# leggedrobotics/traversability_estimation

Hardware: AMD Instinct MI355X
Metric: map cells/s through full filter chain (higher is better)
Workload: dtype f64 moments and eigen-solve, f32 acos and score tail (step filter and combine: f32 compare/add, exact); 1 GPU; 1 x 4096x4096 elevation map per GPU, res 0.05 m, radius 9 cells (normals/roughness/step), slope+roughness+step+normals+combine + traversability_footprint pass; maps_per_gpu=1, map_cells=16777216, footprint=True

## Files before the change

### include/travgpu.h

```cpp
#ifndef TRAVGPU_H
#define TRAVGPU_H

#include <stddef.h>
#include <stdint.h>

#ifdef __cplusplus
extern "C" {
#endif

#define TE_ABI_VERSION 1

typedef enum te_status {
  TE_OK = 0,
  TE_ERR_INVALID_ARG = -1,
  TE_ERR_BAD_PARAM = -2,
  TE_ERR_NOT_READY = -3,
  TE_ERR_HIP = -4,
  TE_ERR_NO_DEVICE = -5,
  TE_ERR_UNSUPPORTED = -6
} te_status;

typedef enum te_layer {
  TE_LAYER_ELEVATION = 0,
  TE_LAYER_SLOPE = 1,
  TE_LAYER_STEP = 2,
  TE_LAYER_ROUGHNESS = 3,
  TE_LAYER_TRAVERSABILITY = 4,
  TE_LAYER_FOOTPRINT = 5,
  TE_LAYER_NORMAL_X = 6,
  TE_LAYER_NORMAL_Y = 7,
  TE_LAYER_NORMAL_Z = 8,
  TE_LAYER_SLOPE_FOOTPRINT = 9,
  TE_LAYER_STEP_FOOTPRINT = 10,
  TE_LAYER_ROUGHNESS_FOOTPRINT = 11,
  TE_LAYER_TRAVERSABILITY_X = 12,
  TE_LAYER_TRAVERSABILITY_ROT = 13,
  TE_LAYER_ROBOT_SLOPE = 14,
  TE_LAYER_COUNT = 15
} te_layer;

#define TE_RUN_KEEP_NORMALS 0x1u
#define TE_RUN_FOOTPRINT    0x2u
#define TE_RUN_FOOTPRINT_MEMO 0x8u
#define TE_RUN_SEQUENTIAL 0x10u
#define TE_RUN_NORMALS_ONLY 0x20u
#define TE_RUN_GENERIC_KERNELS 0x4u

typedef enum te_filter {
  TE_FILTER_SLOPE = 1,
  TE_FILTER_STEP = 2,
  TE_FILTER_ROUGHNESS = 3,
  TE_FILTER_COMBINE = 4,
  TE_FILTER_NORMALS = 5
} te_filter;

typedef struct te_params {
  uint32_t size;
  uint32_t abi_version;
  double normals_radius;
  int32_t normals_axis;
  int32_t _pad0;
  double slope_critical;
  double step_critical;
  double step_radius1;
  double step_radius2;
  int32_t step_ncrit;
  int32_t _pad1;
  double rough_critical;
  double rough_radius;
  float w_scale, w_slope, w_step, w_rough;
  double fp_radius;
  double fp_offset;
  double fp_default;
  double fp_max_gap;
  double fp_critical_step;
  int32_t fp_check_roughness;
  int32_t _pad2;
} te_params;

typedef struct te_ctx te_ctx;

int te_params_default(te_params* p);
int te_params_validate(const te_params* p);

int te_device_count(int* count);
int te_create(int device, te_ctx** out);
int te_destroy(te_ctx* ctx);

int te_set_params(te_ctx* ctx, const te_params* p);
int te_get_params(te_ctx* ctx, te_params* p);
#define TE_OPT_FP_BLOCKED_WALK 1
#define TE_OPT_FP_BLOCKED_BLOCKS_PER_CU 2
#define TE_OPT_GRAPH_REPLAY 4
#define TE_OPT_POLYGON_PER_CELL 3
#define TE_OPT_BCAST_RCCL 5
#define TE_OPT_FP_ANY_REACH 7
#define TE_OPT_NORMALS_RANK_RULE 6
#define TE_OPT_FILTER_ANY_RADIUS 8
#define TE_OPT_FACE_FLAGS 9
int te_set_option(te_ctx* ctx, int option, int value);
int te_download_face_flags(te_ctx* ctx, unsigned char* out, size_t bytes);
int te_set_geometry(te_ctx* ctx, int rows, int cols, int batch, double resolution, double pos_x, double pos_y);

int te_upload_elevation(te_ctx* ctx, const float* host, int map0, int nmaps);
int te_upload_tile(te_ctx* ctx, const float* host_tile, int map, int row0, int col0, int h, int w);
int te_device_ptr(te_ctx* ctx, int layer, void** dptr, size_t* bytes);
int te_set_layer_present(te_ctx* ctx, int layer, int present);

int te_upload_layer(te_ctx* ctx, int layer, const float* host, int map0, int nmaps);
int te_upload_layer_circular(te_ctx* ctx, int layer, const float* host, int map, int start_row, int start_col);
int te_download_layer_circular(te_ctx* ctx, int layer, float* host, int map, int start_row, int start_col);
int te_prefetch_layers(te_ctx* ctx, int n, const int* layers, const float* const* hosts);
int te_wait_prefetch(te_ctx* ctx);
int te_run_filter(te_ctx* ctx, int filter, unsigned flags);
int te_run_chain(te_ctx* ctx, unsigned flags);
int te_run_chain_region(te_ctx* ctx, unsigned flags, int map, int row0, int col0, int h, int w);
int te_download_tile(te_ctx* ctx, int layer, int map, int row0, int col0, int h, int w, float* host_tile);
int te_upload_tile_async(te_ctx* ctx, const float* host_tile, int map, int row0, int col0, int h, int w);
int te_download_tile_async(te_ctx* ctx, int layer, int map, int row0, int col0, int h, int w, float* host_tile);
int te_run_footprint(te_ctx* ctx);
int te_check_footprint_paths(te_ctx* ctx, int map, int n_paths, const int* pose_offset, const double* pose_xy,
                             unsigned char* is_safe, double* traversability, int* status);
typedef struct te_path_check_stats {
  int n_visits, n_discs, n_radius_classes;
} te_path_check_stats;
int te_check_footprint_paths_radius(te_ctx* ctx, int map, int n_paths, const int* pose_offset, const double* pose_xy,
                                    const double* radius, double offset, unsigned char* is_safe, double* traversability,
                                    int* status, te_path_check_stats* stats);
int te_set_check_robot_inclination(te_ctx* ctx, int enabled);
int te_check_inclination(te_ctx* ctx, int map, int n_segments, const double* start_end_xy, unsigned char* ok, int* status);
#define TE_MAX_POLYGON_VERTICES 32
int te_run_polygon_footprint(te_ctx* ctx, int n_points, const double* points_xy, double yaw);
int te_polygons_traversable(te_ctx* ctx, int map, int n_polygons, const int* vertex_offset, const double* vertex_xy,
                            unsigned char* is_traversable, double* traversability);
int te_polygon_untraversable_hull(te_ctx* ctx, int map, int n_vertices, const double* vertex_xy, unsigned char* is_traversable,
                                  double* traversability, int cap_vertices, int* n_hull, double* hull_xy);
int te_check_polygon_footprint_paths(te_ctx* ctx, int map, int n_paths, const int* pose_offset, const double* poses, int n_points,
                                     const double* points_xyz, const unsigned char* conservative, unsigned char* is_safe,
                                     double* traversability, double* area, int* status);
int te_path_polygons(int n_paths, const int* pose_offset, const double* poses, int n_points, const double* points_xyz,
                     const unsigned char* conservative, int cap_polygons, int cap_vertices, int* n_polygons, int* n_vertices,
                     int* polygon_first, int* vertex_offset, double* vertex_xy, double* area);
int te_sync(te_ctx* ctx);

int te_download_layer(te_ctx* ctx, int layer, float* host, int map0, int nmaps);
int te_pin_host(void* host, size_t bytes);
int te_unpin_host(void* host);

int te_shard_range(int batch, int n_shards, int k, int* first, int* count);
int te_bcast_params(te_ctx** ctxs, int n, int root);
int te_run_chain_multi(te_ctx** ctxs, int n, unsigned flags);
int te_sync_multi(te_ctx** ctxs, int n);

int te_time_chain(te_ctx* ctx, unsigned flags, int warmup, int iters, float* ms_per_iter);
int te_time_chain_samples(te_ctx* ctx, unsigned flags, int warmup, int iters, float* ms);

#define TE_MSG_MAX_NAME 64
typedef struct te_msg_info {
  uint32_t seq, stamp_sec, stamp_nsec;
  char frame_id[TE_MSG_MAX_NAME];
  double resolution, length_x, length_y;
  double pose[7];
  int32_t rows, cols;
  int32_t start_row, start_col;
  int32_t n_layers, n_basic_layers;
} te_msg_info;

int te_msg_parse(const void* msg, size_t len, te_msg_info* info);
int te_msg_layer(const void* msg, size_t len, int k, char* name, size_t* data_offset);
int te_msg_write(const te_msg_info* info, int n_layers, const char* const* names, const float* const* layer_data, int n_basic,
                 const char* const* basic_names, void* out, size_t cap, size_t* written);
int te_upload_msg(te_ctx* ctx, const void* msg, size_t len, const char* layer_name, int layer, te_msg_info* info);
int te_download_msg(te_ctx* ctx, const te_msg_info* info, int n_layers, const int* layers, const char* const* names, int n_basic,
                    const char* const* basic_names, void* out, size_t cap, size_t* written);
int te_bag_find_message(const void* bag, size_t len, const char* topic, size_t* msg_offset, size_t* msg_len);
int te_bag_write(const void* msg, size_t msg_len, const char* topic, uint32_t stamp_sec, uint32_t stamp_nsec, void* out,
                 size_t cap, size_t* written);

typedef struct te_image_info {
  uint32_t seq, stamp_sec, stamp_nsec;
  char frame_id[TE_MSG_MAX_NAME];
  int32_t height, width, step;
  int32_t channels, bytes_per_channel;
// ... 64 lines not shown
```

### traversability_estimation_amd/capi.py

```python
import ctypes as C
import os
import struct
import sys

import numpy as np

_HERE = os.path.dirname(os.path.abspath(__file__))
LIB_PATH = os.environ.get("TRAVGPU_LIB") or os.path.join(_HERE, "libtravgpu.so")

TE_OK = 0
TE_ERR_INVALID_ARG, TE_ERR_BAD_PARAM, TE_ERR_NOT_READY, TE_ERR_HIP, TE_ERR_NO_DEVICE, TE_ERR_UNSUPPORTED = \
    -1, -2, -3, -4, -5, -6

LAYERS = dict(elevation=0, traversability_slope=1, traversability_step=2, traversability_roughness=3,
              traversability=4, traversability_footprint=5, surface_normal_x=6, surface_normal_y=7,
              surface_normal_z=8, slope_footprint=9, step_footprint=10, roughness_footprint=11,
              traversability_x=12, traversability_rot=13, robot_slope=14)
FILTERS = dict(slope=1, step=2, roughness=3, combine=4, normals=5)
RUN_KEEP_NORMALS = 0x1
RUN_FOOTPRINT = 0x2
RUN_GENERIC_KERNELS = 0x4
RUN_FOOTPRINT_MEMO = 0x8
RUN_SEQUENTIAL = 0x10
RUN_NORMALS_ONLY = 0x20
OPT_FP_BLOCKED_WALK, OPT_FP_BLOCKED_BLOCKS_PER_CU, OPT_POLYGON_PER_CELL, OPT_GRAPH_REPLAY, OPT_BCAST_RCCL, OPT_NORMALS_RANK_RULE = 1, 2, 3, 4, 5, 6
OPT_FP_ANY_REACH = 7
OPT_FACE_FLAGS = 9
OPT_FILTER_ANY_RADIUS = 8

SYMBOLS = ["te_params_default", "te_params_validate", "te_device_count", "te_create", "te_destroy",
           "te_set_params", "te_get_params", "te_set_option", "te_download_face_flags", "te_set_geometry", "te_upload_elevation", "te_upload_tile", "te_download_tile",
           "te_upload_tile_async", "te_download_tile_async",
           "te_device_ptr", "te_set_layer_present", "te_upload_layer", "te_prefetch_layers", "te_wait_prefetch", "te_upload_layer_circular", "te_download_layer_circular", "te_run_filter", "te_run_chain", "te_run_chain_region", "te_run_footprint", "te_check_footprint_paths", "te_check_footprint_paths_radius",
           "te_sync",
           "te_download_layer", "te_time_chain", "te_time_chain_samples", "te_last_error", "te_version",
           "te_msg_parse", "te_msg_layer", "te_msg_write", "te_upload_msg", "te_download_msg", "te_bag_find_message",
           "te_bag_write", "te_run_polygon_footprint", "te_polygons_traversable",
           "te_check_polygon_footprint_paths", "te_pin_host", "te_unpin_host", "te_path_polygons",
           "te_shard_range", "te_bcast_params", "te_run_chain_multi", "te_sync_multi",
           "te_set_check_robot_inclination", "te_check_inclination", "te_polygon_untraversable_hull",
           "te_image_parse", "te_upload_image", "te_upload_image_msg",
           "te_download_occupancy", "te_download_occupancy_msg", "te_occupancy_msg_write", "te_occupancy_parse",
           "te_download_cloud", "te_download_cloud_msg", "te_cloud_msg_write", "te_cloud_parse", "te_cloud_field", "te_cloud_spans",
           "te_expr_check", "te_run_expression", "te_time_expression_samples"]
MSG_MAX_NAME = 64
OCCUPANCY_MAX_LAYERS = CLOUD_MAX_LAYERS = 16
POINTFIELD_FLOAT32 = 7


def shard_range(batch, n_shards, k):
    first, count = C.c_int(), C.c_int()
    _check(load().te_shard_range(int(batch), int(n_shards), int(k), C.byref(first), C.byref(count)))
    return first.value, count.value


def _handles(ctxs):
    return (C.c_void_p * len(ctxs))(*[c._h for c in ctxs])


def bcast_params(ctxs, root=0):
    _check(load().te_bcast_params(_handles(ctxs), len(ctxs), int(root)))


def run_chain_multi(ctxs, flags=0):
    _check(load().te_run_chain_multi(_handles(ctxs), len(ctxs), int(flags)))


def sync_multi(ctxs):
    _check(load().te_sync_multi(_handles(ctxs), len(ctxs)))


def pack_paths(paths):
    paths = [np.asarray(p, dtype=np.float64).reshape(-1, 2) for p in paths]
    n = len(paths)
    off = np.zeros(n + 1, np.int32)
    if n:
        off[1:] = np.cumsum([len(p) for p in paths])
    xy = np.ascontiguousarray(np.concatenate(paths) if n and off[-1] else np.zeros((1, 2)), dtype=np.float64)
    return off, xy


class TeMsgInfo(C.Structure):
    _fields_ = [("seq", C.c_uint32), ("stamp_sec", C.c_uint32), ("stamp_nsec", C.c_uint32),
                ("frame_id", C.c_char * MSG_MAX_NAME),
                ("resolution", C.c_double), ("length_x", C.c_double), ("length_y", C.c_double),
                ("pose", C.c_double * 7),
                ("rows", C.c_int32), ("cols", C.c_int32), ("start_row", C.c_int32), ("start_col", C.c_int32),
                ("n_layers", C.c_int32), ("n_basic_layers", C.c_int32)]


class TeImageInfo(C.Structure):
    _fields_ = [("seq", C.c_uint32), ("stamp_sec", C.c_uint32), ("stamp_nsec", C.c_uint32),
                ("frame_id", C.c_char * MSG_MAX_NAME),
                ("height", C.c_int32), ("width", C.c_int32), ("step", C.c_int32),
                ("channels", C.c_int32), ("bytes_per_channel", C.c_int32), ("is_bigendian", C.c_int32),
                ("encoding", C.c_char * MSG_MAX_NAME)]


class TeOccupancyInfo(C.Structure):
    _fields_ = [("seq", C.c_uint32), ("stamp_sec", C.c_uint32), ("stamp_nsec", C.c_uint32),
                ("frame_id", C.c_char * MSG_MAX_NAME),
                ("map_load_sec", C.c_uint32), ("map_load_nsec", C.c_uint32),
                ("resolution", C.c_float), ("width", C.c_uint32), ("height", C.c_uint32),
                ("origin", C.c_double * 7)]


class TeCloudInfo(C.Structure):
    _fields_ = [("seq", C.c_uint32), ("stamp_sec", C.c_uint32), ("stamp_nsec", C.c_uint32),
                ("frame_id", C.c_char * MSG_MAX_NAME),
                ("height", C.c_uint32), ("width", C.c_uint32),
                ("n_fields", C.c_uint32), ("point_step", C.c_uint32), ("row_step", C.c_uint32),
                ("is_bigendian", C.c_int32), ("is_dense", C.c_int32)]


IMAGE_ENCODINGS = {"mono8": (1, 1), "8UC1": (1, 1), "mono16": (1, 2), "16UC1": (1, 2),
                   "rgb8": (3, 1), "bgr8": (3, 1), "8UC3": (3, 1), "rgba8": (4, 1), "bgra8": (4, 1), "8UC4": (4, 1),
                   "rgb16": (3, 2), "bgr16": (3, 2), "16UC3": (3, 2), "rgba16": (4, 2), "bgra16": (4, 2), "16UC4": (4, 2)}


class TeExprInfo(C.Structure):
    _fields_ = [("n_instructions", C.c_int32), ("layer_mask", C.c_uint32), ("n_reductions", C.c_int32), ("stack_depth", C.c_int32)]


class TePathCheckStats(C.Structure):
    _fields_ = [("n_visits", C.c_int), ("n_discs", C.c_int), ("n_radius_classes", C.c_int)]


class TeParams(C.Structure):
    _fields_ = [("size", C.c_uint32), ("abi_version", C.c_uint32),
                ("normals_radius", C.c_double), ("normals_axis", C.c_int32), ("_pad0", C.c_int32),
                ("slope_critical", C.c_double),
                ("step_critical", C.c_double), ("step_radius1", C.c_double), ("step_radius2", C.c_double),
                ("step_ncrit", C.c_int32), ("_pad1", C.c_int32),
                ("rough_critical", C.c_double), ("rough_radius", C.c_double),
                ("w_scale", C.c_float), ("w_slope", C.c_float), ("w_step", C.c_float), ("w_rough", C.c_float),
                ("fp_radius", C.c_double), ("fp_offset", C.c_double), ("fp_default", C.c_double),
                ("fp_max_gap", C.c_double), ("fp_critical_step", C.c_double),
                ("fp_check_roughness", C.c_int32), ("_pad2", C.c_int32)]


class TeError(RuntimeError):
    def __init__(self, code, msg):
        super().__init__(f"travgpu error {code}: {msg}")
        self.code = code


_lib = None


def load():
    global _lib
    if _lib is None:
        if not os.path.exists(LIB_PATH):
            raise ImportError(f"{LIB_PATH} is missing: build it with `python -m traversability_estimation_amd.build` "
                              "(hipcc --offload-arch=gfx950); there is no CPU fallback")
        L = C.CDLL(LIB_PATH)
        vp, pp = C.c_void_p, C.POINTER(TeParams)
        fp = C.POINTER(C.c_float)
        L.te_params_default.argtypes = [pp]
        L.te_params_validate.argtypes = [pp]
        L.te_device_count.argtypes = [C.POINTER(C.c_int)]
        L.te_create.argtypes = [C.c_int, C.POINTER(vp)]
        L.te_destroy.argtypes = [vp]
        L.te_set_params.argtypes = [vp, pp]
        L.te_get_params.argtypes = [vp, pp]
        L.te_set_option.argtypes = [vp, C.c_int, C.c_int]
        if "TRAVGPU_LIB" not in os.environ or hasattr(L, "te_download_face_flags"):
            L.te_download_face_flags.argtypes = [vp, C.POINTER(C.c_ubyte), C.c_size_t]
        L.te_set_geometry.argtypes = [vp, C.c_int, C.c_int, C.c_int, C.c_double, C.c_double, C.c_double]
        L.te_upload_elevation.argtypes = [vp, fp, C.c_int, C.c_int]
        L.te_upload_tile.argtypes = [vp, fp, C.c_int, C.c_int, C.c_int, C.c_int, C.c_int]
        L.te_download_tile.argtypes = [vp, C.c_int, C.c_int, C.c_int, C.c_int, C.c_int, C.c_int, fp]
        L.te_upload_tile_async.argtypes = [vp, fp, C.c_int, C.c_int, C.c_int, C.c_int, C.c_int]
        L.te_download_tile_async.argtypes = [vp, C.c_int, C.c_int, C.c_int, C.c_int, C.c_int, C.c_int, fp]
        L.te_device_ptr.argtypes = [vp, C.c_int, C.POINTER(vp), C.POINTER(C.c_size_t)]
        L.te_set_layer_present.argtypes = [vp, C.c_int, C.c_int]
        L.te_upload_layer.argtypes = [vp, C.c_int, fp, C.c_int, C.c_int]
        L.te_upload_layer_circular.argtypes = [vp, C.c_int, fp, C.c_int, C.c_int, C.c_int]
        if "TRAVGPU_LIB" not in os.environ or hasattr(L, "te_prefetch_layers"):
            L.te_prefetch_layers.argtypes = [vp, C.c_int, C.POINTER(C.c_int), C.POINTER(fp)]
            L.te_wait_prefetch.argtypes = [vp]
        L.te_download_layer_circular.argtypes = [vp, C.c_int, fp, C.c_int, C.c_int, C.c_int]
        L.te_run_filter.argtypes = [vp, C.c_int, C.c_uint]
        L.te_run_chain.argtypes = [vp, C.c_uint]
        L.te_run_chain_region.argtypes = [vp, C.c_uint, C.c_int, C.c_int, C.c_int, C.c_int, C.c_int]
        L.te_run_footprint.argtypes = [vp]
        L.te_polygon_untraversable_hull.argtypes = [vp, C.c_int, C.c_int, C.POINTER(C.c_double), C.POINTER(C.c_ubyte),
                                                    C.POINTER(C.c_double), C.c_int, C.POINTER(C.c_int), C.POINTER(C.c_double)]
        L.te_set_check_robot_inclination.argtypes = [vp, C.c_int]
        L.te_check_inclination.argtypes = [vp, C.c_int, C.c_int, C.POINTER(C.c_double), C.POINTER(C.c_ubyte), C.POINTER(C.c_int)]
        L.te_check_footprint_paths.argtypes = [vp, C.c_int, C.c_int, C.POINTER(C.c_int), C.POINTER(C.c_double),
                                               C.POINTER(C.c_ubyte), C.POINTER(C.c_double), C.POINTER(C.c_int)]
        L.te_check_footprint_paths_radius.argtypes = [vp, C.c_int, C.c_int, C.POINTER(C.c_int), C.POINTER(C.c_double),
                                                      C.POINTER(C.c_double), C.c_double, C.POINTER(C.c_ubyte),
                                                      C.POINTER(C.c_double), C.POINTER(C.c_int), C.POINTER(TePathCheckStats)]
        L.te_run_polygon_footprint.argtypes = [vp, C.c_int, C.POINTER(C.c_double), C.c_double]
        L.te_polygons_traversable.argtypes = [vp, C.c_int, C.c_int, C.POINTER(C.c_int), C.POINTER(C.c_double),
                                              C.POINTER(C.c_ubyte), C.POINTER(C.c_double)]
        L.te_check_polygon_footprint_paths.argtypes = [vp, C.c_int, C.c_int, C.POINTER(C.c_int), C.POINTER(C.c_double), C.c_int,
                                                       C.POINTER(C.c_double), C.POINTER(C.c_ubyte), C.POINTER(C.c_ubyte),
                                                       C.POINTER(C.c_double), C.POINTER(C.c_double), C.POINTER(C.c_int)]
        L.te_pin_host.argtypes = [vp, C.c_size_t]
        L.te_unpin_host.argtypes = [vp]
        ip_, dp_ = C.POINTER(C.c_int), C.POINTER(C.c_double)
        L.te_path_polygons.argtypes = [C.c_int, ip_, dp_, C.c_int, dp_, C.POINTER(C.c_ubyte), C.c_int, C.c_int, ip_, ip_, ip_, ip_,
                                       dp_, dp_]
        L.te_sync.argtypes = [vp]
        L.te_download_layer.argtypes = [vp, C.c_int, fp, C.c_int, C.c_int]
        L.te_time_chain.argtypes = [vp, C.c_uint, C.c_int, C.c_int, C.POINTER(C.c_float)]
        L.te_time_chain_samples.argtypes = [vp, C.c_uint, C.c_int, C.c_int, C.POINTER(C.c_float)]
        L.te_shard_range.argtypes = [C.c_int, C.c_int, C.c_int, C.POINTER(C.c_int), C.POINTER(C.c_int)]
        L.te_bcast_params.argtypes = [C.POINTER(vp), C.c_int, C.c_int]
        L.te_run_chain_multi.argtypes = [C.POINTER(vp), C.c_int, C.c_uint]
        L.te_sync_multi.argtypes = [C.POINTER(vp), C.c_int]
        szp, cpp = C.POINTER(C.c_size_t), C.POINTER(C.c_char_p)
        L.te_msg_parse.argtypes = [C.c_char_p, C.c_size_t, C.POINTER(TeMsgInfo)]
        L.te_msg_layer.argtypes = [C.c_char_p, C.c_size_t, C.c_int, C.c_char_p, szp]
        L.te_msg_write.argtypes = [C.POINTER(TeMsgInfo), C.c_int, cpp, C.POINTER(fp), C.c_int, cpp, vp, C.c_size_t, szp]
        L.te_upload_msg.argtypes = [vp, C.c_char_p, C.c_size_t, C.c_char_p, C.c_int, C.POINTER(TeMsgInfo)]
        L.te_download_msg.argtypes = [vp, C.POINTER(TeMsgInfo), C.c_int, C.POINTER(C.c_int), cpp, C.c_int, cpp, vp,
                                      C.c_size_t, szp]
        L.te_bag_find_message.argtypes = [C.c_char_p, C.c_size_t, C.c_char_p, szp, szp]
        L.te_bag_write.argtypes = [C.c_char_p, C.c_size_t, C.c_char_p, C.c_uint32, C.c_uint32, vp, C.c_size_t, szp]
        L.te_image_parse.argtypes = [C.c_char_p, C.c_size_t, C.POINTER(TeImageInfo), szp]
        L.te_upload_image.argtypes = [vp, C.POINTER(TeImageInfo), vp, C.c_int, C.c_int, C.c_float, C.c_float, C.c_double]
        L.te_upload_image_msg.argtypes = [vp, C.c_char_p, C.c_size_t, C.c_int, C.c_float, C.c_float, C.c_double, C.c_double,
                                          C.c_double, C.c_double, C.POINTER(TeImageInfo)]
        ip, i8p, u32p = C.POINTER(C.c_int), C.POINTER(C.c_int8), C.POINTER(C.c_uint32)
        L.te_download_occupancy.argtypes = [vp, C.c_int, C.c_int, ip, fp, fp, vp]
        L.te_download_occupancy_msg.argtypes = [vp, C.POINTER(TeMsgInfo), C.c_int, C.c_float, C.c_float, vp, C.c_size_t, szp]
        L.te_occupancy_msg_write.argtypes = [C.POINTER(TeOccupancyInfo), i8p, vp, C.c_size_t, szp]
        L.te_occupancy_parse.argtypes = [C.c_char_p, C.c_size_t, C.POINTER(TeOccupancyInfo), szp]
        L.te_download_cloud.argtypes = [vp, C.c_int, C.c_int, ip, C.c_int, C.c_int, ip, vp, C.c_size_t, szp]
        L.te_download_cloud_msg.argtypes = [vp, C.POINTER(TeMsgInfo), C.c_int, ip, cpp, C.c_int, C.c_int, ip, vp, C.c_size_t, szp]
        L.te_cloud_msg_write.argtypes = [C.POINTER(TeCloudInfo), C.c_int, cpp, fp, vp, C.c_size_t, szp]
        L.te_cloud_parse.argtypes = [C.c_char_p, C.c_size_t, C.POINTER(TeCloudInfo), szp]
        L.te_cloud_field.argtypes = [C.c_char_p, C.c_size_t, C.c_int, C.c_char_p, u32p, u32p, u32p]
        L.te_cloud_spans.argtypes = [szp]
        L.te_expr_check.argtypes = [C.c_char_p, C.POINTER(TeExprInfo)]
        L.te_run_expression.argtypes = [vp, C.c_char_p, C.c_int]
        L.te_time_expression_samples.argtypes = [vp, C.c_char_p, C.c_int, C.c_int, C.POINTER(C.c_float)]
        L.te_last_error.restype = C.c_char_p
        L.te_version.restype = C.c_char_p
        _lib = L
    return _lib


def _check(rc):
    if rc != TE_OK:
        raise TeError(rc, load().te_last_error().decode())

# ... 155 lines not shown
            struct.pack("<BII", 1 if is_bigendian else 0, step, len(data)) + data)


def pin_host(array):
    _check(load().te_pin_host(array.ctypes.data_as(C.c_void_p), array.nbytes))


def unpin_host(array):
    _check(load().te_unpin_host(array.ctypes.data_as(C.c_void_p)))


def path_polygons(paths, points_xyz, conservative=None):
    paths = [np.asarray(p, dtype=np.float64).reshape(-1, 7) for p in paths]
    n = len(paths)
    off = np.zeros(n + 1, np.int32)
    if n:
        off[1:] = np.cumsum([len(p) for p in paths])
    poses = np.ascontiguousarray(np.concatenate(paths) if n and off[-1] else np.zeros((1, 7)), dtype=np.float64)
    pts = np.ascontiguousarray(points_xyz, dtype=np.float64).reshape(-1, 3)
    cons = None if conservative is None else np.ascontiguousarray(conservative, dtype=np.uint8)
    ip_, dp_ = C.POINTER(C.c_int), C.POINTER(C.c_double)
    args = (n, off.ctypes.data_as(ip_), poses.ctypes.data_as(dp_), len(pts), pts.ctypes.data_as(dp_),
            None if cons is None else cons.ctypes.data_as(C.POINTER(C.c_ubyte)))
    npoly, nvert = C.c_int(), C.c_int()
    L = load()
    L.te_path_polygons(*args, 0, 0, C.byref(npoly), C.byref(nvert), None, None, None, None)
    first = np.zeros(n + 1, np.int32)
    voff = np.zeros(npoly.value + 1, np.int32)
    xy = np.zeros((max(nvert.value, 1), 2), np.float64)
    area = np.zeros(max(npoly.value, 1), np.float64)
    _check(L.te_path_polygons(*args, npoly.value, nvert.value, C.byref(npoly), C.byref(nvert), first.ctypes.data_as(ip_),
                              voff.ctypes.data_as(ip_), xy.ctypes.data_as(dp_), area.ctypes.data_as(dp_)))
    return [[(xy[voff[q]:voff[q + 1]].copy(), float(area[q])) for q in range(first[k], first[k + 1])] for k in range(n)]


def expr_check(text):
    info = TeExprInfo()
    _check(load().te_expr_check(str(text).encode(), C.byref(info)))
    return {"n_instructions": int(info.n_instructions), "layers": [k for k, v in LAYERS.items() if info.layer_mask >> v & 1],
            "n_reductions": int(info.n_reductions), "stack_depth": int(info.stack_depth)}


def device_count():
    n = C.c_int(0)
    rc = load().te_device_count(C.byref(n))
    return n.value if rc == TE_OK else 0


class Context:

    def __init__(self, device=0):
        self._h = C.c_void_p()
        _check(load().te_create(int(device), C.byref(self._h)))
        self.rows = self.cols = self.batch = 0

    def close(self):
        if self._h:
            load().te_destroy(self._h)
            self._h = C.c_void_p()

    def __del__(self):
        try:
            self.close()
        except Exception:
            pass

    def __enter__(self):
        return self

    def __exit__(self, *a):
        self.close()

    def set_params(self, p):
        _check(load().te_set_params(self._h, C.byref(p)))

    def set_option(self, option, value):
        _check(load().te_set_option(self._h, int(option), int(value)))

    def download_face_flags(self):
        out = np.empty((self.batch, (self.cols + 3) // 4, (self.rows + 63) // 64), np.uint8)
        _check(load().te_download_face_flags(self._h, out.ctypes.data_as(C.POINTER(C.c_ubyte)), out.size))
        return out

    def get_params(self):
        p = TeParams()
        _check(load().te_get_params(self._h, C.byref(p)))
        return p

    def set_geometry(self, rows, cols, batch, res, pos=(0.0, 0.0)):
        _check(load().te_set_geometry(self._h, int(rows), int(cols), int(batch), float(res), float(pos[0]), float(pos[1])))
        self.rows, self.cols, self.batch = int(rows), int(cols), int(batch)

    def upload_elevation(self, elev, map0=0):
        a = np.ascontiguousarray(elev, dtype=np.float32).reshape(-1)
        per = self.rows * self.cols
        assert a.size % per == 0, (a.size, per)
        _check(load().te_upload_elevation(self._h, a.ctypes.data_as(C.POINTER(C.c_float)), int(map0), a.size // per))

    def upload_tile(self, tile, map_index, row0, col0):
        t = np.ascontiguousarray(tile, dtype=np.float32)
        w, h = t.shape
        _check(load().te_upload_tile(self._h, t.ctypes.data_as(C.POINTER(C.c_float)), int(map_index), int(row0),
                                     int(col0), int(h), int(w)))

    def download_tile(self, layer, map_index, row0, col0, h, w):
        t = np.empty((int(w), int(h)), np.float32)
        _check(load().te_download_tile(self._h, LAYERS[layer] if isinstance(layer, str) else int(layer), int(map_index), int(row0),
                                       int(col0), int(h), int(w), t.ctypes.data_as(C.POINTER(C.c_float))))
        return t

    def upload_tile_async(self, tile, map_index, row0, col0):
        assert tile.dtype == np.float32 and tile.flags["C_CONTIGUOUS"], "upload_tile_async: float32, C-contiguous (no hidden copy)"
        w, h = tile.shape
        _check(load().te_upload_tile_async(self._h, tile.ctypes.data_as(C.POINTER(C.c_float)), int(map_index), int(row0), int(col0),
                                           int(h), int(w)))

    def download_tile_async(self, layer, map_index, row0, col0, out):
        assert out.dtype == np.float32 and out.flags["C_CONTIGUOUS"]
        w, h = out.shape
        _check(load().te_download_tile_async(self._h, LAYERS[layer] if isinstance(layer, str) else int(layer), int(map_index),
                                             int(row0), int(col0), int(h), int(w), out.ctypes.data_as(C.POINTER(C.c_float))))

    def device_ptr(self, layer):
        p, n = C.c_void_p(), C.c_size_t()
        _check(load().te_device_ptr(self._h, LAYERS[layer] if isinstance(layer, str) else int(layer), C.byref(p),
                                    C.byref(n)))
        return p.value, n.value

    def set_layer_present(self, layer, present):
        _check(load().te_set_layer_present(self._h, LAYERS[layer] if isinstance(layer, str) else int(layer), 1 if present else 0))

    def upload_layer(self, layer, data, map0=0):
        a = np.ascontiguousarray(data, dtype=np.float32).reshape(-1)
        per = self.rows * self.cols
        assert a.size % per == 0, (a.size, per)
        _check(load().te_upload_layer(self._h, LAYERS[layer] if isinstance(layer, str) else int(layer),
                                      a.ctypes.data_as(C.POINTER(C.c_float)), int(map0), a.size // per))

    def prefetch_layers(self, layers):
        names = list(layers)
        arrs = [np.ascontiguousarray(layers[k], dtype=np.float32).reshape(-1) for k in names]
        for a in arrs:
            assert a.size == self.rows * self.cols * self.batch, (a.size, self.rows, self.cols, self.batch)
        ids = (C.c_int * len(names))(*[LAYERS[k] if isinstance(k, str) else int(k) for k in names])
        ptrs = (C.POINTER(C.c_float) * len(names))(*[a.ctypes.data_as(C.POINTER(C.c_float)) for a in arrs])
        self._prefetch_keep = arrs
        _check(load().te_prefetch_layers(self._h, len(names), ids, ptrs))

    def wait_prefetch(self):
        try:
            _check(load().te_wait_prefetch(self._h))
        finally:
            self._prefetch_keep = None

    def upload_layer_circular(self, layer, data, start_index, map_index=0):
        a = np.ascontiguousarray(data, dtype=np.float32).reshape(-1)
        assert a.size == self.rows * self.cols, (a.size, self.rows, self.cols)
        _check(load().te_upload_layer_circular(self._h, LAYERS[layer] if isinstance(layer, str) else int(layer),
                                               a.ctypes.data_as(C.POINTER(C.c_float)), int(map_index),
                                               int(start_index[0]), int(start_index[1])))

    def download_layer_circular(self, layer, start_index, map_index=0):
        out = np.empty((self.cols, self.rows), dtype=np.float32)
        _check(load().te_download_layer_circular(self._h, LAYERS[layer] if isinstance(layer, str) else int(layer),
                                                 out.ctypes.data_as(C.POINTER(C.c_float)), int(map_index),
                                                 int(start_index[0]), int(start_index[1])))
# ... 247 lines not shown
```

### traversability_estimation_amd/csrc/te_ctx.h

```cpp
#pragma once
#include <math.h>
#include <stdarg.h>
#include <stdio.h>
#include <string.h>

#include <algorithm>
#include <condition_variable>
#include <dlfcn.h>
#include <functional>
#include <chrono>
#include <mutex>
#include <new>
#include <thread>
#include <vector>

#include <cstdlib>
#include "te_devbuf.h"
#include "te_disc_table.h"
#include "te_internal.h"
#include "te_msg.h"

struct te_ctx;

namespace te {
namespace shim {
int fail(int code, const char* fmt, ...);
}
}

#define HIP_TRY(expr)                                                                            \
  do {                                                                                           \
    hipError_t e__ = (expr);                                                                     \
    if (e__ != hipSuccess) {                                                                     \
      (void)hipGetLastError();  \
      return ::te::shim::fail(TE_ERR_HIP, "%s: %s", #expr, hipGetErrorString(e__));                          \
    }                                                                                            \
  } while (0)

struct te_ctx {
  std::mutex mu;
  int device = 0;
  hipStream_t stream = nullptr;
  hipEvent_t ev0 = nullptr, ev1 = nullptr;
  hipStream_t aux_stream = nullptr;
  hipEvent_t ev_fork = nullptr, ev_join = nullptr;
  te_params params;
  bool have_params = false, have_geo = false, have_elev = false, chain_done = false, footprint_done = false;
  struct PdTable {
    double radius = 0.0, offset = 0.0, res = 0.0;
    int rows = 0, cols = 0;
    te::DevBuf dev;
    int n_spiral = 0;
    unsigned long long used = 0;
  };
  static constexpr int kPdTables = 16;
  struct LayerMem {
    te::DevBuf slab;
    te::DevBuf poly;
    te::DevBuf poly_stream;
    te::DevBuf robot_slope;
    te::DevBuf tie_scratch;
    te::DevBuf img_stage;
    te::DevBuf occ_out, cloud_counts, cloud_out;
    te::DevBuf expr_scratch;
    struct FpAny {
      te::DevBuf tab, prefix;
    } fpa;
    PdTable pd_tables[kPdTables];
    te::DevBuf pd_scratch;
  } lmem;
  struct CtxMem {
    te::DevBuf spiral;
    te::DevBuf count;
    te::DevBuf hole_queue;
    te::DevBuf clip_table, fp_clip_table;
    te::DevBuf fa_tab;
    te::DevBuf tile_in[2], tile_out[2];
  } cmem;
  float* poly_rot = nullptr;
  bool have_robot_slope = false, check_inclination = false;
  std::vector<unsigned> poly_stream_host;
  te::Geo geo;
  te::ChainParams cp;
  te::FootprintParams fp;
  te::Layers L;
  size_t layer_elems = 0;
  bool mask_done = false;
  unsigned long long pd_clock = 0;
  bool combine_deferred = false;
  bool trav_external = false;
  bool trav_ptr_out = false;
  int opt_fb_walk = 0, opt_fb_blocks_per_cu = 0, opt_polygon_per_cell = 0, opt_graph = 0, opt_bcast_rccl = 0, opt_rank_rule = 0,
      opt_fp_any = 0;
  int opt_filter_any = 0;
  te::DiscTable fa_host[4];
  long long invalid_cells = -1;
  long long invalid_runs = -1;
  uint8_t* face_flags = nullptr;
  double face_crit = __builtin_nan("");
  bool elev_ptr_out = false;
  int opt_face_flags = 1;
  bool tables_ready = false;
  bool fp_tables_ready = false;
  int fp_tables_rc = TE_OK;
  char fp_tables_err[256] = "";
  static constexpr int kGraphs = 4;
  hipGraphExec_t graph_exec[kGraphs] = {nullptr, nullptr, nullptr, nullptr};
  unsigned graph_flags[kGraphs] = {0, 0, 0, 0};
  int graph_next = 0;
  bool graph_ok = true;
  struct TileSlot {
    hipEvent_t ready = nullptr, freed = nullptr;
    bool used = false;
  };
  hipStream_t in_stream = nullptr, out_stream = nullptr;
  TileSlot in_slot[2], out_slot[2];
  int in_next = 0, out_next = 0;
  bool tiles_pending = false;
  te::HostStager stager;
  unsigned layers_written = 0;
  te::HostStager prefetcher;
  hipStream_t prefetch_order = nullptr;
  std::thread prefetch_thread;
  std::mutex pf_mu;
  std::condition_variable pf_cv;
  std::function<void()> pf_job;
  bool pf_quit = false;
  bool prefetch_running = false, prefetch_elev = false;
  unsigned prefetch_mask = 0;
  std::atomic<int> prefetch_rc{TE_OK};
};

namespace te {
namespace shim {
void finish_prefetch_locked(te_ctx* c);
struct CtxLock {
  std::lock_guard<std::mutex> lk;
  explicit CtxLock(te_ctx* c, bool beside_prefetch = false, unsigned touches = 0) : lk(c->mu) {
    if (!beside_prefetch || (touches & c->prefetch_mask)) finish_prefetch_locked(c);
  }
};
constexpr unsigned bit(int layer) { return (layer >= 0 && layer < 32) ? 1u << layer : 0u; }
int count_invalid_elevation(te_ctx* c);
const uint8_t* usable_face_flags(const te_ctx* c);
float* layer_ptr(te_ctx* c, int layer);
int ensure_input_layer(te_ctx* c, int layer);
int rebuild_tables(te_ctx* c);
void rebuild_footprint_tables(te_ctx* c);
int sync_tiles(te_ctx* c);
int run_whole_locked(te_ctx* c, unsigned flags);
}
}
```

### traversability_estimation_amd/csrc/te_face_flags.h

```cpp
#pragma once

#include <stddef.h>
#include <stdint.h>

#if defined(__HIPCC__)
#define TE_FF_HD __host__ __device__ __forceinline__
#else
#define TE_FF_HD inline
#endif

namespace te {

constexpr int kFaceGranI = 64, kFaceGranJ = 4;
constexpr int kFaceDilate = 2;

TE_FF_HD int face_flag_ntx(int rows) { return (rows + kFaceGranI - 1) / kFaceGranI; }
TE_FF_HD int face_flag_nfy(int cols) { return (cols + kFaceGranJ - 1) / kFaceGranJ; }
TE_FF_HD size_t face_flag_bytes(int rows, int cols, int batch) {
  return (size_t)face_flag_ntx(rows) * (size_t)face_flag_nfy(cols) * (size_t)batch;
}
TE_FF_HD size_t face_flag_index(int rows, int cols, int map, int i, int j) {
  return ((size_t)map * (size_t)face_flag_nfy(cols) + (size_t)(j / kFaceGranJ)) * (size_t)face_flag_ntx(rows) + (size_t)(i / kFaceGranI);
}

TE_FF_HD float face_min(float a, float b) { return (b < a || a != a) ? b : a; }
TE_FF_HD bool face_hit(float m, float e, double crit_step) { return (double)m < (double)e - crit_step; }

TE_FF_HD bool face_tile_near_failing_border(int rows, int cols, int edge_fail, int i0, int j0, int tw, int th) {
  return ((edge_fail & 1) && i0 <= 2) || ((edge_fail & 2) && i0 + tw - 1 >= rows - 3) || ((edge_fail & 4) && j0 <= 2) ||
         ((edge_fail & 8) && j0 + th - 1 >= cols - 3);
}

TE_FF_HD bool face_tile_clear(const uint8_t* flags, int rows, int cols, int map, int i0, int j0, int th) {
  const int ntx = face_flag_ntx(rows), nfy = face_flag_nfy(cols);
  const uint8_t* f = flags + ((size_t)map * (size_t)nfy) * (size_t)ntx + (size_t)(i0 / kFaceGranI);
  unsigned any = 0;
  for (int t = 0; t < th / kFaceGranJ; ++t) {
    const int fj = j0 / kFaceGranJ + t;
    if (fj < nfy) any |= f[(size_t)fj * (size_t)ntx];
  }
  return any == 0;
}

#if !defined(__HIP_DEVICE_COMPILE__)
inline void face_flags_host(const float* elev, int rows, int cols, int batch, double crit_step, uint8_t* flags, uint8_t* hit = nullptr) {
  const size_t nflags = face_flag_bytes(rows, cols, batch);
  for (size_t k = 0; k < nflags; ++k) flags[k] = 0;
  const float nan = __builtin_nanf("");
  for (int m = 0; m < batch; ++m) {
    const float* e = elev + (size_t)m * rows * cols;
    for (int j = 0; j < cols; ++j)
      for (int i = 0; i < rows; ++i) {
        float mn = nan;
        for (int dj = -1; dj <= 1; ++dj)
          for (int di = -1; di <= 1; ++di) {
            const int a = i + di, b = j + dj;
            if (a >= 0 && a < rows && b >= 0 && b < cols) mn = face_min(mn, e[(size_t)b * rows + a]);
          }
        const bool h = face_hit(mn, e[(size_t)j * rows + i], crit_step);
        if (hit) hit[(size_t)m * rows * cols + (size_t)j * rows + i] = h ? 1 : 0;
        if (!h) continue;
        const int a0 = i - kFaceDilate < 0 ? 0 : i - kFaceDilate, a1 = i + kFaceDilate > rows - 1 ? rows - 1 : i + kFaceDilate;
        const int b0 = j - kFaceDilate < 0 ? 0 : j - kFaceDilate, b1 = j + kFaceDilate > cols - 1 ? cols - 1 : j + kFaceDilate;
        for (int gj = b0 / kFaceGranJ; gj <= b1 / kFaceGranJ; ++gj)
          for (int gi = a0 / kFaceGranI; gi <= a1 / kFaceGranI; ++gi) flags[face_flag_index(rows, cols, m, gi * kFaceGranI, gj * kFaceGranJ)] = 1;
      }
  }
}
#endif

}
```

### traversability_estimation_amd/csrc/te_footprint.hip

```cpp
#include "te_internal.h"

#include <cstdlib>
#include "te_geom.h"
#include "te_march.h"

namespace te {

namespace {

constexpr int kLanes = 64;

__device__ __forceinline__ float qnanf() { return __builtin_nanf(""); }
inline int submap_edge_failures(const Geo& g) {
  auto bound = [](double position, double len, double mappos) {
    double shifted = position - mappos + 0.5 * len;
    double eps = 10.0 * 2.220446049250313e-16;
    if (fabs(position) > 1.0) eps *= fabs(position);
    if (shifted <= 0)
      shifted = eps;
    else if (shifted >= len)
      shifted = len - eps;
    return shifted + mappos - 0.5 * len;
  };
  auto ok = [](double x, double len, double mappos, double res, int n) {
// ... 189 lines not shown
    const double lowest = height - crit_step;
    const double tcx = cx - cell_x(g, ii), tcy = cy - cell_y(g, ij);
    for (int lin = 0; lin < sm.sr * sm.sc; ++lin) {
      const int a = lin % sm.sr, b = lin / sm.sr;
      if (!(step.at(sm.ti + a, sm.tj + b) == 0.0f && (double)elev.at(sm.ti + a, sm.tj + b) < lowest)) continue;
      double vx, vy;
      pair_vector(g, ii, ij, sm, a, b, vx, vy);
      if (sqrt(vx * vx + vy * vy) < 0.025) continue;
      if (sqrt(tcx * tcx + tcy * tcy) > 0.025) {
        if (tcx * vx + tcy * vy < 0.0) continue;
      }
      if (pair_blocks(g, elev, ii, ij, vx, vy, height, crit_step, max_gap)) return false;
    }
  }
  return true;
}

__device__ bool pair_bit(const Geo& g, const TileView& elev, const float* __restrict__ t_elev, const float* __restrict__ t_key, int idx,
                         int ii, int ij, int lin, double crit_step, double max_gap) {
  const Submap sm = submap_of(g, ii, ij);
  if (lin >= sm.sr * sm.sc) return false;
  const double height = (double)t_elev[idx];
  const double lowest = height - crit_step;
  const int a = lin % sm.sr, b = lin / sm.sr;
  const int m = idx + (sm.tj + b - ij) * MTW + (sm.ti + a - ii);
  const float km = t_key[m];
  if (!((double)km < lowest)) return false;
  double vx, vy;
  pair_vector(g, ii, ij, sm, a, b, vx, vy);
  if (sqrt(vx * vx + vy * vy) < 0.025) return false;
  return pair_blocks(g, elev, ii, ij, vx, vy, height, crit_step, max_gap);
}
__device__ bool check_step_memo(const Geo& g, const float* __restrict__ t_elev, const float* __restrict__ t_key,
                                const unsigned short* __restrict__ fmask, int ctr, int ci, int cj, double crit_step, int edge_fail) {
  const double cx = cell_x(g, ci), cy = cell_y(g, cj);
  const double thr = crit_step + (double)t_elev[ctr];
  int ncand = 0;
  for (int dj = -2; dj <= 2; ++dj) {
    const int hw = (dj == -2 || dj == 2) ? 1 : 2;
    for (int di = -hw; di <= hw; ++di) {
      const int idx = ctr + dj * MTW + di;
      if (!((double)t_key[idx] > thr)) continue;
      ++ncand;
      const int ii = ci + di, ij = cj + dj;
      if (submap_fails(g, edge_fail, ii, ij)) return false;
      unsigned f = fmask[idx];
      if (f == 0u) continue;
      const Submap sm = submap_of(g, ii, ij);
      const double tcx = cx - cell_x(g, ii), tcy = cy - cell_y(g, ij);
      const bool filter = sqrt(tcx * tcx + tcy * tcy) > 0.025;
      while (f) {
        const int lin = __ffs((int)f) - 1;
        f &= f - 1u;
        if (filter) {
          double vx, vy;
          pair_vector(g, ii, ij, sm, lin % sm.sr, lin / sm.sr, vx, vy);
          if (tcx * vx + tcy * vy < 0.0) continue;
        }
        return false;
      }
    }
  }
  if (ncand == 0) {
    if (submap_fails(g, edge_fail, ci, cj)) return false;
    if (fmask[ctr] != 0) return false;
  }
  return true;
}

struct MaskArgs {
  Disc slope_disc;
  Disc step_disc;
  int ncrit_slope, ncrit_rough, check_rough, write_memo;
  double crit_step, max_gap;
  int edge_fail;
  int combine;
  float w_scale, w_slope, w_step, w_rough;
  int ti0, tj0, map;
  unsigned* blocked_count;
  uint8_t* untrav_flags;
  int flag_ntx, flag_nfy;
  const uint8_t* face_flags;
  int whatif;
};

template <int MY>
__global__ __launch_bounds__(MX* MBY) __attribute__((amdgpu_waves_per_eu(4, 4))) void k_fp_mask(Geo g, MaskArgs a, const float* __restrict__ elev,
                                                     const float* __restrict__ slope, const float* __restrict__ step,
                                                     const float* __restrict__ rough, uint8_t* __restrict__ untrav,
                                                     float* __restrict__ slope_fp, float* __restrict__ step_fp,
                                                     float* __restrict__ rough_fp, float* __restrict__ trav) {
  constexpr int MTH = MY + 2 * MH;
  __shared__ float t_elev[MTW * MTH], t_key[MTW * MTH], t_kl[MTW * MTH];
  __shared__ int ntodo, arrived, members, compacted, nkl;
  if (threadIdx.x == 0 && threadIdx.y == 0) ntodo = arrived = members = compacted = nkl = 0;
  const size_t mo = (size_t)(a.map >= 0 ? a.map : (int)blockIdx.z) * g.rows * g.cols;
  const int i0 = ((int)blockIdx.x + a.ti0) * MX, j0 = ((int)blockIdx.y + a.tj0) * MY;
  if (a.blocked_count && threadIdx.x == 0 && threadIdx.y == 0 && blockIdx.x == 0 && blockIdx.y == 0 && blockIdx.z == 0)
    a.blocked_count[0] = a.blocked_count[1] = a.blocked_count[4] = 0u;
  const bool q5 = a.step_disc.Q == 5 && a.step_disc.n_ties == 0;
  bool flat = false;
  if (a.face_flags != nullptr && q5 && a.whatif == 0)
    flat = face_tile_clear(a.face_flags, g.rows, g.cols, a.map >= 0 ? a.map : (int)blockIdx.z, i0, j0, MY) &&
           !(a.edge_fail != 0 && face_tile_near_failing_border(g.rows, g.cols, a.edge_fail, i0, j0, MX, MY));
  flat = __builtin_amdgcn_readfirstlane(flat ? 1 : 0) != 0;
  uint8_t* const my_flags = a.untrav_flags + ((size_t)(a.map >= 0 ? a.map : (int)blockIdx.z) * a.flag_nfy) * a.flag_ntx + (i0 >> 6);
  {
    constexpr int NF = MY / 4;
    const int t = threadIdx.y * MX + threadIdx.x;
    if (t < NF && (j0 >> 2) + t < a.flag_nfy) my_flags[(size_t)((j0 >> 2) + t) * a.flag_ntx] = 0;
  }
  constexpr int NC = MY / MBY;
  const int i = i0 + threadIdx.x;
  const int ic = i < g.rows ? i : g.rows - 1;
  const int jb = threadIdx.y * NC;
  float s_slope[NC], s_step[NC], s_rough[NC];
  fast::static_for<NC>([&](auto cc) __attribute__((always_inline)) {
    constexpr int c = decltype(cc)::value;
    int j = j0 + jb + c;
    j = j < g.cols ? j : g.cols - 1;
    const size_t o = mo + (size_t)j * g.rows + ic;
    s_slope[c] = slope[o];
    s_step[c] = step[o];
    s_rough[c] = (a.check_rough || a.combine) ? rough[o] : 1.0f;
  });
  if (!flat) {
    constexpr int KM = (MTH + MBY - 1) / MBY;
    const int tid = threadIdx.y * MX + threadIdx.x;
    const int ac = i0 + (int)threadIdx.x;
    const bool col_in = ac < g.rows;
    const float* const pe = elev + mo + (col_in ? ac : g.rows - 1);
    const float* const ps = step + mo + (col_in ? ac : g.rows - 1);
    float le[KM], ls[KM];
#pragma unroll
    for (int k = 0; k < KM; ++k) {
      int bb = j0 - MH + (int)threadIdx.y + k * MBY;
      bb = bb < 0 ? 0 : (bb >= g.cols ? g.cols - 1 : bb);
      const size_t o = (size_t)bb * g.rows;
      le[k] = pe[o];
      ls[k] = ps[o];
    }
    constexpr int NH = 2 * MH * MTH;
    static_assert(NH <= MX * MBY, "one halo cell per thread");
    const int hj = tid / (2 * MH), hc = tid - hj * (2 * MH);
    const int hti = hc < MH ? hc : MX + hc;
    const int ha = i0 - MH + hti, hb = j0 - MH + hj;
    float he = 0.0f, hs = 0.0f;
    if (tid < NH) {
      const int aa = ha < 0 ? 0 : (ha >= g.rows ? g.rows - 1 : ha), bb = hb < 0 ? 0 : (hb >= g.cols ? g.cols - 1 : hb);
      const size_t o = mo + (size_t)bb * g.rows + aa;
      he = elev[o];
      hs = step[o];
    }
#pragma unroll
    for (int k = 0; k < KM; ++k) {
      const int tj = (int)threadIdx.y + k * MBY, bb = j0 - MH + tj;
      const bool in = col_in && bb >= 0 && bb < g.cols;
      if (tj < MTH) {
        const int idx = tj * MTW + (int)threadIdx.x + MH;
        t_elev[idx] = in ? le[k] : qnanf();
        t_key[idx] = (in && ls[k] == 0.0f) ? le[k] : qnanf();
      }
    }
    if (tid < NH) {
      const bool in = ha >= 0 && ha < g.rows && hb >= 0 && hb < g.cols;
      const int idx = hj * MTW + hti;
      t_elev[idx] = in ? he : qnanf();
      t_key[idx] = (in && hs == 0.0f) ? he : qnanf();
    }
  }
  __syncthreads();
  bool any_kl = false;
  if (!flat) {
    static_assert((MTH - 2) % MBY == 0, "row segments");
    constexpr int SEG = (MTH - 2) / MBY;
    const int la = threadIdx.x + 2, r0 = 1 + threadIdx.y * SEG;
    float rm[3];
    auto row_min = [&](int r) {
      const float* k = t_key + r * MTW + la;
      return fast::vmin3(k[-1], k[0], k[1]);
    };
    rm[0] = row_min(r0 - 1);
    rm[1] = row_min(r0);
    fast::static_for<SEG>([&](auto rc) __attribute__((always_inline)) {
      constexpr int q = decltype(rc)::value;
      const int r = r0 + q;
      const float next = row_min(r + 1);
      const float m = fast::vmin3(rm[q % 3], rm[(q + 1) % 3], next);
      rm[(q + 2) % 3] = next;
      const int idx = r * MTW + la;
      const bool hit = (double)m < (double)t_elev[idx] - a.crit_step;
      t_kl[idx] = hit ? t_key[idx] : qnanf();
      any_kl |= hit;
    });
    const int tid = threadIdx.y * MX + threadIdx.x;
    if (tid < 4 * (MTH - 2)) {
      const int col = (tid & 3) == 0 ? 1 : MTW - 5 + (tid & 3);
      const int idx = (1 + (tid >> 2)) * MTW + col;
      const float* k = t_key + idx;
      const float m = fast::vmin3(fast::vmin3(k[-MTW - 1], k[-MTW], k[-MTW + 1]), fast::vmin3(k[-1], k[0], k[1]),
                                  fast::vmin3(k[MTW - 1], k[MTW], k[MTW + 1]));
      const bool hit = (double)m < (double)t_elev[idx] - a.crit_step;
      t_kl[idx] = hit ? t_key[idx] : qnanf();
      any_kl |= hit;
    }
  }
  const bool tile_has_kl = flat ? false : __syncthreads_or(any_kl ? 1 : 0) != 0;
  const TileView ve = {t_elev, elev + mo, i0, j0, g.rows, MTH}, vs = {nullptr, step + mo, i0, j0, g.rows, MTH},
                 vl = {nullptr, slope + mo, i0, j0, g.rows, MTH}, vr = {nullptr, rough + mo, i0, j0, g.rows, MTH};
  const bool in_map = i < g.rows;
  float h1k[5], h2k[5], h1l[5], h2l[5];
  auto reduce_row = [&](int row, int slot) {
    const int base = (jb + row + MH) * MTW + (threadIdx.x + MH);
    const float* k = t_key + base;
    const float* l = t_kl + base;
    h1k[slot] = fast::vmax3(k[-1], k[0], k[1]);
    h2k[slot] = fast::vmax3(h1k[slot], k[-2], k[2]);
    h1l[slot] = fast::vmax3(l[-1], l[0], l[1]);
    h2l[slot] = fast::vmax3(h1l[slot], l[-2], l[2]);
  };
  unsigned screen_mask = 0;
  if (q5 && in_map && !tile_has_kl) screen_mask = (1u << NC) - 1u;
  if (q5 && in_map && tile_has_kl) {
    fast::static_for<4>([&](auto rc) __attribute__((always_inline)) {
      constexpr int r = decltype(rc)::value;
      reduce_row(r - 2, r);
    });
    fast::static_for<NC>([&](auto cc) __attribute__((always_inline)) {
      constexpr int c = decltype(cc)::value;
      constexpr int s2 = (c + 4) % 5;
      reduce_row(c + 2, s2);
      constexpr int sm2 = c % 5, sm1 = (c + 1) % 5, s0 = (c + 2) % 5, s1 = (c + 3) % 5;
      const float mk = fast::vmax3(fast::vmax3(h1k[sm2], h2k[sm1], h2k[s0]), h2k[s1], h1k[s2]);
      const float ml = fast::vmax3(fast::vmax3(h1l[sm2], h2l[sm1], h2l[s0]), h2l[s1], h1l[s2]);
      const int ctr = (jb + c + MH) * MTW + (threadIdx.x + MH);
      const double thr = a.crit_step + (double)t_elev[ctr];
      const float lc = t_kl[ctr];
      const bool hit = ((double)mk > thr) ? ((double)ml > thr) : (lc == lc);
      screen_mask |= hit ? 0u : (1u << c);
    });
  }
  unsigned slow_mask = 0;
  fast::static_for<NC>([&](auto cc) __attribute__((always_inline)) {
    constexpr int c = decltype(cc)::value;
    const int j = j0 + jb + c;
    const float c_slope = s_slope[c], c_step = s_step[c], c_rough = s_rough[c];
    bool near_bad_edge = false;
    if (__builtin_expect(a.edge_fail != 0, 0))
      near_bad_edge = ((a.edge_fail & 1) && i <= 2) || ((a.edge_fail & 2) && i >= g.rows - 3) || ((a.edge_fail & 4) && j <= 2) ||
                      ((a.edge_fail & 8) && j >= g.cols - 3);
    const bool step_fast = !(c_step == 0.0f) || (q5 && ((screen_mask >> c) & 1u) != 0 && !near_bad_edge);
    const bool slow = (c_slope == 0.0f) || !step_fast || (a.check_rough && c_rough == 0.0f);
    slow_mask |= (slow && j < g.cols && in_map) ? (1u << c) : 0u;
    if (j < g.cols && in_map) {
      const size_t o = mo + (size_t)j * g.rows + i;
      if (!slow) untrav[o] = 0;
      if (a.combine) {
        const float ta = a.w_slope * c_slope, tb = a.w_step * c_step, tc = a.w_rough * c_rough;
        const float tab = ta + tb;
        const float tabc = tab + tc;
        trav[o] = a.w_scale * tabc;
      }
      if (a.write_memo && !slow) {
        slope_fp[o] = qnanf();
        step_fp[o] = (c_step == 0.0f) ? 1.0f : qnanf();
        rough_fp[o] = qnanf();
      }
    }
  });
  static_assert(sizeof(t_kl) >= MX * MY * sizeof(unsigned short), "the list fits the tile it replaces");
  unsigned short* const todo = reinterpret_cast<unsigned short*>(t_kl);
  if (!q5) {
#pragma unroll 1
    while (slow_mask) {
      const int c = __ffs((int)slow_mask) - 1;
      slow_mask &= slow_mask - 1;
      const int j = j0 + jb + c;
      const size_t o = mo + (size_t)j * g.rows + i;
      const float c_slope = slope[o], c_step = step[o], c_rough = (a.check_rough || a.combine) ? rough[o] : 1.0f;
      float m_slope = qnanf(), m_step = qnanf(), m_rough = qnanf();
      bool ok = true;
      const int ctr = (jb + c + MH) * MTW + (threadIdx.x + MH);
      if (c_slope == 0.0f) {
        ok = count_zero_ok(g, a.slope_disc, vl, i, j, a.ncrit_slope);
        m_slope = ok ? 1.0f : 0.0f;
      }
      if (ok && c_step == 0.0f) {
        const bool screen_ok = check_step_screen(a.step_disc, t_elev, t_key, t_kl, ctr, a.crit_step);
        const bool near_bad_edge = a.edge_fail && (((a.edge_fail & 1) && i <= 2) || ((a.edge_fail & 2) && i >= g.rows - 3) ||
                                                    ((a.edge_fail & 4) && j <= 2) || ((a.edge_fail & 8) && j >= g.cols - 3));
        ok = (screen_ok && !near_bad_edge) || check_step(g, a.step_disc, ve, vs, i, j, a.crit_step, a.max_gap, a.edge_fail);
        m_step = ok ? 1.0f : 0.0f;
      }
      if (ok && a.check_rough && c_rough == 0.0f) {
        ok = count_zero_ok(g, a.slope_disc, vr, i, j, a.ncrit_rough);
        m_rough = ok ? 1.0f : 0.0f;
      }
      untrav[o] = ok ? 0 : 1;
      if (!ok) my_flags[(size_t)(j >> 2) * a.flag_ntx] = 1;
      if (a.write_memo) {
        slope_fp[o] = m_slope;
        step_fp[o] = m_step;
        rough_fp[o] = m_rough;
      }
    }
    return;
  }
  if (tile_has_kl) {
    constexpr int NCELL = MTW * MTH;
    static_assert(sizeof(t_kl) >= 2 * NCELL * sizeof(unsigned short), "candidate list + pair masks fit the tile they replace");
    static_assert(NCELL % 2 == 0, "pair masks are cleared word by word");
    unsigned short* const klist = reinterpret_cast<unsigned short*>(t_kl);
    unsigned short* const fmask = klist + NCELL;
    const int tid = threadIdx.y * MX + threadIdx.x;
    constexpr int SEG = (MTH - 2) / MBY;
    unsigned klbits = 0;
    {
      const int la = threadIdx.x + 2, r0 = 1 + threadIdx.y * SEG;
#pragma unroll
      for (int q = 0; q < SEG; ++q) {
        const float v = t_kl[(r0 + q) * MTW + la];
        klbits |= (v == v) ? (1u << q) : 0u;
      }
      if (tid < 4 * (MTH - 2)) {
        const int col = (tid & 3) == 0 ? 1 : MTW - 5 + (tid & 3);
        const float v = t_kl[(1 + (tid >> 2)) * MTW + col];
        klbits |= (v == v) ? 0x80000000u : 0u;
      }
    }
    __syncthreads();
    for (int k = tid; k < NCELL / 2; k += MX * MBY) reinterpret_cast<unsigned*>(fmask)[k] = 0u;
    if (klbits != 0u) {
      int at = atomicAdd(&nkl, __popc(klbits));
      const int la = threadIdx.x + 2, r0 = 1 + threadIdx.y * SEG;
      unsigned bits = klbits & 0x7fffffffu;
      while (bits) {
        const int q = __ffs((int)bits) - 1;
        bits &= bits - 1u;
        klist[at++] = (unsigned short)((r0 + q) * MTW + la);
      }
      if (klbits & 0x80000000u) klist[at++] = (unsigned short)((1 + (tid >> 2)) * MTW + ((tid & 3) == 0 ? 1 : MTW - 5 + (tid & 3)));
    }
    __syncthreads();
    {
      const int n_jobs = (a.whatif & 1) ? 0 : nkl * 9;
#pragma unroll 1
      for (int k = tid; k < n_jobs; k += MX * MBY) {
        const int idx = klist[k / 9], lin = k - (k / 9) * 9;
// ... 12 lines not shown
        int base = 0;
        if (threadIdx.x == 0) base = atomicAdd(&ntodo, __popcll(bm));
        base = __shfl(base, 0);
        if (need)
          todo2[base + __popcll(bm & ((1ull << threadIdx.x) - 1ull))] =
              (unsigned short)(((jb + c) << 7) | ((((screen_mask >> c) & 1u) != 0 ? 1 : 0) << 6) | (int)threadIdx.x);
      }
    });
    __syncthreads();
    const int n_todo2 = (a.whatif & 2) ? 0 : ntodo;
#pragma unroll 1
    for (int k = tid; k < n_todo2; k += MX * MBY) {
      const int e = todo2[k];
      const int li = e & 63, lj = e >> 7;
      const bool screened = ((e >> 6) & 1) != 0;
      const int ci = i0 + li, j = j0 + lj;
      const size_t o = mo + (size_t)j * g.rows + ci;
      const float c_slope = slope[o], c_step = step[o], c_rough = (a.check_rough || a.combine) ? rough[o] : 1.0f;
      float m_slope = qnanf(), m_step = qnanf(), m_rough = qnanf();
      bool ok = true;
      if (c_slope == 0.0f) {
        ok = count_zero_ok(g, a.slope_disc, vl, ci, j, a.ncrit_slope);
        m_slope = ok ? 1.0f : 0.0f;
      }
      if (ok && c_step == 0.0f) {
        const bool near_bad_edge = a.edge_fail && (((a.edge_fail & 1) && ci <= 2) || ((a.edge_fail & 2) && ci >= g.rows - 3) ||
                                                    ((a.edge_fail & 4) && j <= 2) || ((a.edge_fail & 8) && j >= g.cols - 3));
        ok = (screened && !near_bad_edge) ||
             check_step_memo(g, t_elev, t_key, fmask, (lj + MH) * MTW + (li + MH), ci, j, a.crit_step, a.edge_fail);
        m_step = ok ? 1.0f : 0.0f;
      }
      if (ok && a.check_rough && c_rough == 0.0f) {
        ok = count_zero_ok(g, a.slope_disc, vr, ci, j, a.ncrit_rough);
        m_rough = ok ? 1.0f : 0.0f;
      }
      untrav[o] = ok ? 0 : 1;
      if (!ok) my_flags[(size_t)(j >> 2) * a.flag_ntx] = 1;
      if (a.write_memo) {
        slope_fp[o] = m_slope;
        step_fp[o] = m_step;
        rough_fp[o] = m_rough;
      }
    }
    return;
  }
  const bool mine = __ballot(slow_mask != 0u) != 0ull;
  int rank = 0;
  __builtin_amdgcn_fence(__ATOMIC_RELEASE, "workgroup");
  if (threadIdx.x == 0) {
    if (mine) rank = atomicAdd(&members, 1);
    atomicAdd(&arrived, 1);
  }
  if (!mine) return;
  rank = __builtin_amdgcn_readfirstlane(rank);
  while (*(volatile int*)&arrived < MBY) __builtin_amdgcn_s_sleep(1);
  __builtin_amdgcn_fence(__ATOMIC_ACQUIRE, "workgroup");
  const int n_members = *(volatile int*)&members;
  fast::static_for<NC>([&](auto cc) __attribute__((always_inline)) {
    constexpr int c = decltype(cc)::value;
    const bool need = ((slow_mask >> c) & 1u) != 0;
    const unsigned long long bm = __ballot(need);
    if (bm != 0ull) {
      int base = 0;
      if (threadIdx.x == 0) base = atomicAdd(&ntodo, __popcll(bm));
      base = __shfl(base, 0);
      if (need)
        todo[base + __popcll(bm & ((1ull << threadIdx.x) - 1ull))] =
            (unsigned short)(((jb + c) << 7) | ((((screen_mask >> c) & 1u) != 0 ? 1 : 0) << 6) | (int)threadIdx.x);
    }
  });
  __builtin_amdgcn_fence(__ATOMIC_RELEASE, "workgroup");
  if (threadIdx.x == 0) atomicAdd(&compacted, 1);
  while (*(volatile int*)&compacted < n_members) __builtin_amdgcn_s_sleep(1);
  __builtin_amdgcn_fence(__ATOMIC_ACQUIRE, "workgroup");
  const int n_todo = *(volatile int*)&ntodo;
#pragma unroll 1
  for (int k = rank * MX + (int)threadIdx.x; k < n_todo; k += n_members * MX) {
    const int e = todo[k];
    const int li = e & 63, lj = e >> 7;
    const bool screened = ((e >> 6) & 1) != 0;
    const int ci = i0 + li, j = j0 + lj;
    const size_t o = mo + (size_t)j * g.rows + ci;
    const float c_slope = slope[o], c_step = step[o], c_rough = (a.check_rough || a.combine) ? rough[o] : 1.0f;
    float m_slope = qnanf(), m_step = qnanf(), m_rough = qnanf();
    bool ok = true;
    if (c_slope == 0.0f) {
      ok = count_zero_ok(g, a.slope_disc, vl, ci, j, a.ncrit_slope);
      m_slope = ok ? 1.0f : 0.0f;
    }
    if (ok && c_step == 0.0f) {
      const bool screen_ok = screened;
      const bool near_bad_edge = a.edge_fail && (((a.edge_fail & 1) && ci <= 2) || ((a.edge_fail & 2) && ci >= g.rows - 3) ||
                                                  ((a.edge_fail & 4) && j <= 2) || ((a.edge_fail & 8) && j >= g.cols - 3));
      ok = flat || (screen_ok && !near_bad_edge) || check_step(g, a.step_disc, ve, vs, ci, j, a.crit_step, a.max_gap, a.edge_fail);
      m_step = ok ? 1.0f : 0.0f;
    }
    if (ok && a.check_rough && c_rough == 0.0f) {
      ok = count_zero_ok(g, a.slope_disc, vr, ci, j, a.ncrit_rough);
      m_rough = ok ? 1.0f : 0.0f;
    }
    untrav[o] = ok ? 0 : 1;
    if (!ok) my_flags[(size_t)(j >> 2) * a.flag_ntx] = 1;
    if (a.write_memo) {
      slope_fp[o] = m_slope;
      step_fp[o] = m_step;
      rough_fp[o] = m_rough;
    }
  }
}

struct SpiralArgs {
  int h[kMaxRadiusCells + 1];
  int n_ties;
  int8_t tie_di[kMaxTies], tie_dj[kMaxTies];
  double r2;
  int n_spiral;
  const unsigned* ptab;
  const int* gtab;
  double rmin, rmax, def;
  int out_rows;
  int inner_q;
  int map0;
};

constexpr double kUOff = 4096.0;
constexpr int kFpHead = 24;
constexpr int kFpWaves = 2;

template <int R>
__global__ __launch_bounds__(kLanes, kFpWaves) void k_fp_slide(Geo g, SpiralArgs a, const float* __restrict__ trav,
                                                     const uint8_t* __restrict__ untrav,
                                                     float* __restrict__ footprint) {
  constexpr int W = kLanes + 2 * R;
  constexpr int NR = 2 * R + 3;
  constexpr int NX = (W + kLanes - 1) / kLanes;
  constexpr int kAhead = 4;
  constexpr bool kPipe = R <= 10;
  __shared__ double ring[NR * W];
  const int lane = threadIdx.x;
  const size_t mo = (size_t)(a.map0 + (int)blockIdx.z) * g.rows * g.cols;
  const int i0 = blockIdx.x * kLanes;
  const int js = blockIdx.y * a.out_rows;
  const int jend = js + a.out_rows < g.cols ? js + a.out_rows : g.cols;
  const int i = i0 + lane;
  const int c = lane + R;
  const int kx = (i >= g.rows) ? 0 : (i < R) ? (R - i) : ((g.rows - 1 - i < R) ? -(R - (g.rows - 1 - i)) : 0);

  for (int idx = lane; idx < NR * W; idx += kLanes) ring[idx] = 0.0;
  __syncthreads();
  auto load_row = [&](int r, float (&pt)[NX], int (&pu)[NX]) {
    const int rc = r < 0 ? 0 : (r >= g.cols ? g.cols - 1 : r);
    const size_t base = mo + (size_t)rc * g.rows;
#pragma unroll
    for (int x = 0; x < NX; ++x) {
      int ci = i0 - R + lane + x * kLanes;
      ci = ci < 0 ? 0 : (ci >= g.rows ? g.rows - 1 : ci);
      pt[x] = trav[base + ci];
      pu[x] = untrav[base + ci];
    }
  };
  auto store_row = [&](int r, int slot, const float (&pt)[NX], const int (&pu)[NX]) {
    const bool rin = r >= 0 && r < g.cols;
    double* dst = ring + slot * W;
    double v0 = 0.0;
#pragma unroll
    for (int x = 0; x < NX; ++x) {
      const int cc = lane + x * kLanes;
      const int ci = i0 - R + cc;
      const bool inmap = rin && cc < W && ci >= 0 && ci < g.rows;
      const double t = __builtin_isfinite(pt[x]) ? (double)pt[x] : a.def;
      const double v = inmap ? t + (pu[x] ? kUOff : 0.0) : 0.0;
      if (x == 0) v0 = v;
      dst[cc < W ? cc : lane] = cc < W ? v : v0;
    }
  };

  constexpr bool kRegTab = R <= 16;
  constexpr int NTAB = kRegTab ? (int)(3.2 * (R + 1) * (R + 1) / kLanes) + 1 : 1;
  unsigned tabreg[NTAB];
  if (kRegTab) {
    const unsigned* __restrict__ ptab0 = a.ptab;
#pragma unroll
    for (int ch = 0; ch < NTAB; ++ch) tabreg[ch] = ch * kLanes + lane < a.n_spiral ? ptab0[ch * kLanes + lane] : 0u;
  }

  double S = 0.0;
  const int jstart = js;
  int slot_j = 0;
  int lead[R + 1], trail[R + 1];
// ... 219 lines not shown
            done = true;
            if (a.rmin == 0.0 || (double)ring_first * g.res <= a.rmin) {
              oc = 0.0f;
              return;
            }
            const bool before = in && lane < first;
            acc += before ? v : 0.0;
            cnt += __popcll(__ballot(before));
#pragma unroll
            for (int d = 32; d >= 1; d >>= 1) acc += __shfl_xor(acc, d);
            oc = value_at(ring_first, acc, cnt);
            return;
          }
          acc += in ? v : 0.0;
          cnt += __popcll(__ballot(in));
        };
        if (kRegTab && a.n_spiral <= NTAB * kLanes) {
          fast::static_for<NTAB>([&](auto chc) __attribute__((always_inline)) {
            constexpr int ch = decltype(chc)::value;
            if (done || ch * kLanes >= a.n_spiral) return;
            chunk(tabreg[ch], ch * kLanes);
          });
        } else {
          for (int k0 = 0; k0 < a.n_spiral && !done; k0 += kLanes) chunk(ptab[k0 + lane < a.n_spiral ? k0 + lane : 0], k0);
        }
        if (lane == l) out = oc;
      }
    }
    if (qs % 2 == 0)
      advance(j, ptq[qs], puq[qs], vb, va);
    else
      advance(j, ptq[qs], puq[qs], va, vb);
    if (i < g.rows) footprint[mo + (size_t)j * g.rows + i] = out;
  });
  }
}

bool footprint_slide_general(const Geo& g, const FootprintParams& p, const Layers& L, const unsigned* ptab, const int* clip_table,
                             hipStream_t stream, const Region* region) {
  SpiralArgs a;
  const Disc& d = p.fp_disc;
  for (int k = 0; k <= kMaxRadiusCells; ++k) a.h[k] = (k <= d.R) ? d.hw[k] : -1;
  a.n_ties = d.n_ties;
  for (int t = 0; t < kMaxTies; ++t) {
    a.tie_di[t] = d.tie_di[t];
    a.tie_dj[t] = d.tie_dj[t];
  }
  a.r2 = d.r2;
  a.n_spiral = p.n_spiral;
  a.ptab = ptab;
  a.gtab = clip_table;
  a.rmin = p.rmin;
  a.rmax = p.rmax;
  a.def = p.def;
  a.inner_q = fast::footprint_inner_q(g.res, p.rmin, p.rmax);
  {
    const int nbx = (g.rows + kLanes - 1) / kLanes;
    const int Rk = p.reach;
    const long ring_bytes = (long)(2 * Rk + 3) * (kLanes + 2 * Rk) * 8;
    long per_cu = 160 * 1024 / ring_bytes;
    if (per_cu > kFpWaves * 4) per_cu = kFpWaves * 4;
    int strips = (int)((per_cu * 256) / (nbx * (region ? 1 : (g.batch > 0 ? g.batch : 1))));
    strips = strips < 1 ? 1 : strips;
    int rows_per = (g.cols + strips - 1) / strips;
    static const int min_rows = lab_int("TE_FP_MIN_STRIP", 1);
    a.out_rows = rows_per < min_rows ? min_rows : (rows_per > 512 ? 512 : rows_per);
    a.out_rows = a.out_rows < 1 ? 1 : a.out_rows;
  }
  a.map0 = region ? region->map : 0;
  const dim3 grid((unsigned)((g.rows + kLanes - 1) / kLanes), (unsigned)((g.cols + a.out_rows - 1) / a.out_rows),
                  (unsigned)(region ? 1 : g.batch));
  switch (p.reach) {
#define X(q) \
  case q:    \
    hipLaunchKernelGGL((k_fp_slide<q>), grid, dim3(kLanes), 0, stream, g, a, L.trav, L.untrav, L.footprint); \
    return true;
    X(1) X(2) X(3) X(4) X(5) X(6) X(7) X(8) X(9) X(10) X(11) X(12) X(13) X(14) X(15) X(16) X(17) X(18) X(19) X(20)
#undef X
    default:
      return false;
  }
}

void launch_mask_pass(const Geo& g, const FootprintParams& p, const Layers& L, const uint8_t* face_flags, bool write_memo, const ChainParams* combine,
                      hipStream_t stream, const Region* region, Region* rf_out) {
  MaskArgs m;
  m.slope_disc = p.slope_disc;
  m.step_disc = p.step_disc;
  m.ncrit_slope = p.ncrit_slope;
  m.ncrit_rough = p.ncrit_rough;
  m.check_rough = p.check_rough;
  m.write_memo = write_memo ? 1 : 0;
  m.crit_step = p.crit_step;
  m.max_gap = p.max_gap;
  m.combine = combine ? 1 : 0;
  m.edge_fail = submap_edge_failures(g);
  m.w_scale = combine ? combine->w_scale : 0.0f;
  m.w_slope = combine ? combine->w_slope : 0.0f;
  m.w_step = combine ? combine->w_step : 0.0f;
  m.w_rough = combine ? combine->w_rough : 0.0f;
  m.ti0 = m.tj0 = 0;
  m.map = -1;
  m.blocked_count = L.fp_blocked_count;
  m.untrav_flags = L.untrav_flags;
  m.face_flags = face_flags;
  m.flag_ntx = untrav_flag_ntx(g.rows);
  m.flag_nfy = untrav_flag_nfy(g.cols);
  static const int mask_whatif = lab_int("TE_MASK_WHATIF", 0);
  m.whatif = mask_whatif;
  Region rm = {-1, 0, 0, g.rows, g.cols}, rf = rm;
  if (region) {
    auto grow = [&](const Region& r, int k) {
      Region o = r;
      o.i0 = r.i0 - k < 0 ? 0 : r.i0 - k;
      o.j0 = r.j0 - k < 0 ? 0 : r.j0 - k;
      o.i1 = r.i1 + k > g.rows ? g.rows : r.i1 + k;
      o.j1 = r.j1 + k > g.cols ? g.cols : r.j1 + k;
      return o;
    };
    rm = grow(*region, MH);
    rf = grow(rm, p.reach);
    m.map = region->map;
  }
  const long tiles32 = (long)((rm.i1 - rm.i0 + MX - 1) / MX) * ((rm.j1 - rm.j0 + 31) / 32) * (region ? 1 : (g.batch > 0 ? g.batch : 1));
  static const int small_env = lab_int("TE_MASK_SMALL_TILES", -1);
  const bool small = small_env >= 0 ? small_env != 0 : tiles32 < 1024;
  static const int tile_env = lab_int("TE_MASK_TILE", 0);
  const int my = (small && tiles32 < 128 && small_env != 8) ? 4 : (small ? 8 : (tile_env == 16 ? 16 : 32));
  auto launch_mask = [&](int t0, int t1, hipStream_t st) {
    if (t1 <= t0) return;
    m.ti0 = rm.i0 / MX;
    m.tj0 = t0;
    const dim3 grid((unsigned)((rm.i1 - 1) / MX - m.ti0 + 1), (unsigned)(t1 - t0), (unsigned)(region ? 1 : g.batch));
    if (my == 4)
      hipLaunchKernelGGL(k_fp_mask<4>, grid, dim3(MX, MBY), 0, st, g, m, L.elev, L.slope, L.step, L.rough, L.untrav, L.slope_fp, L.step_fp, L.rough_fp, L.trav);
    else if (my == 8)
      hipLaunchKernelGGL(k_fp_mask<8>, grid, dim3(MX, MBY), 0, st, g, m, L.elev, L.slope, L.step, L.rough, L.untrav, L.slope_fp, L.step_fp, L.rough_fp, L.trav);
#ifdef TE_LAB
    else if (my == 16)
      hipLaunchKernelGGL(k_fp_mask<16>, grid, dim3(MX, MBY), 0, st, g, m, L.elev, L.slope, L.step, L.rough, L.untrav, L.slope_fp, L.step_fp, L.rough_fp, L.trav);
#endif
    else
      hipLaunchKernelGGL(k_fp_mask<32>, grid, dim3(MX, MBY), 0, st, g, m, L.elev, L.slope, L.step, L.rough, L.untrav, L.slope_fp, L.step_fp, L.rough_fp, L.trav);
  };
  const int t_lo = rm.j0 / my, t_hi = (rm.j1 - 1) / my + 1;
  {
    TraceRange tr(combine ? "footprint: isTraversableForFilters mask + weighted combine" : "footprint: isTraversableForFilters mask");
    launch_mask(t_lo, t_hi, stream);
  }
  *rf_out = rf;
}

}

hipError_t launch_footprint_mask(const Geo& g, const FootprintParams& p, const Layers& L, const uint8_t* face_flags, const ChainParams* combine,
                                 hipStream_t stream) {
  Region rf;
  launch_mask_pass(g, p, L, face_flags, false, combine, stream, nullptr, &rf);
  return hipGetLastError();
}

hipError_t launch_footprint(const Geo& g, const FootprintParams& p, const Layers& L, const uint8_t* face_flags, const unsigned* ptab,
                            const int* clip_table, bool write_memo, const ChainParams* combine, double trav_cap, hipStream_t stream,
                            const Region* region) {
  Region rf;
  launch_mask_pass(g, p, L, face_flags, write_memo, combine, stream, region, &rf);
  TraceRange tr_sum("footprint: disc sums (+ blocked discs)");
  const Region* rfp = region ? &rf : nullptr;
  const Disc& d = p.fp_disc;
  fast::FpRouteIn in;
  in.R = d.R;
  in.Q = d.Q;
  in.npoints = d.npoints;
  in.n_ties = d.n_ties;
  in.ties_on_circle = true;
  in.n_gen = 0;
  for (int t = 0; t < d.n_ties; ++t) {
    in.ties_on_circle = in.ties_on_circle && (int)d.tie_di[t] * d.tie_di[t] + (int)d.tie_dj[t] * d.tie_dj[t] == p.reach * p.reach;
    in.n_gen += (d.tie_di[t] != 0 && d.tie_dj[t] != 0) ? 1 : 0;
  }
  in.reach = p.reach;
  in.n_spiral = p.n_spiral;
  in.rmin = p.rmin;
  in.def = p.def;
  in.tcap = trav_cap;
  in.rows = g.rows;
  in.cols = g.cols;
  in.batch = g.batch;
  in.region = rfp != nullptr;
  in.i0 = rf.i0;
  in.i1 = rf.i1;
  in.j0 = rf.j0;
  in.j1 = rf.j1;
  in.guard_rows = layer_has_guard_rows(L.trav, g, sizeof(float)) && layer_has_guard_rows(L.untrav, g, sizeof(uint8_t));
  in.has_list = L.fp_blocked && L.fp_blocked_count;
  in.has_scratch = L.fp_scratch != nullptr;
  in.list_cap = L.fp_blocked_cap;
  in.cus = device_cus();
  in.any = p.any != 0;
  in.no_f3 = lab_flag("TE_NO_F3");
  in.no_f4 = lab_flag("TE_NO_F4");
  in.no_f5 = lab_flag("TE_NO_F5");
  in.f4_no_ties = lab_flag("TE_F4_NO_TIES");
  in.f5_waves = lab_int("TE_F5_WAVES", 0);
  in.f5_max_strip = lab_int("TE_F5_MAX_STRIP", 512);
  in.f4_blocks_per_cu = lab_int("TE_F4_BLOCKS_PER_CU", 0);
  in.f4_min_strip = lab_int("TE_F4_MIN_STRIP", 1);
  const fast::FpRoute r = fast::plan_fp_route(in);
  bool launched = true;
  switch (r.route) {
    case fast::kFpAny:
      return launch_footprint_any(g, p, L, rfp, stream);
    case fast::kFpSlide5:
      launched = fast::footprint_slide5(g, p, L, clip_table, r, stream, rfp);
      break;
    case fast::kFpSlide4:
      launched = fast::footprint_slide4(g, p, L, clip_table, r, stream, rfp);
      break;
    case fast::kFpSlide3:
      launched = fast::footprint_slide3(g, p, L, ptab, clip_table, stream, rfp);
      break;
    case fast::kFpGeneral:
      launched = footprint_slide_general(g, p, L, ptab, clip_table, stream, region);
      break;
  }
  if (!launched) return hipErrorNoBinaryForGpu;
  if (r.blocked) fast::footprint_blocked4(g, p, L, ptab, stream);
  return hipGetLastError();
}

}
```

### traversability_estimation_amd/csrc/te_internal.h

```cpp
#pragma once
#include <atomic>
#include <hip/hip_runtime.h>
#include <math.h>
#include <stdint.h>
#include <stdlib.h>

#include <vector>

#include "te_face_flags.h"
#include "te_fp_route.h"
#include "te_slab.h"
#include "travgpu.h"

namespace te {

#ifdef TE_LAB
inline int lab_int(const char* name, int dflt) {
  const char* v = getenv(name);
  return v ? atoi(v) : dflt;
}
inline bool lab_flag(const char* name) { return getenv(name) != nullptr; }
#else
constexpr int lab_int(const char*, int dflt) { return dflt; }
constexpr bool lab_flag(const char*) { return false; }
// ... 147 lines not shown
struct PathPolygons {
  std::vector<int> vertex_offset;
  std::vector<double> vertex_xy;
  std::vector<double> area;
  std::vector<double> area_previous;
  std::vector<int> first, count, status;
};
void build_path_polygons(int n_paths, const int* pose_offset, const double* poses, int n_points, const double* points_xyz,
                         const unsigned char* conservative, PathPolygons& out);

constexpr int kFixTiles = 8;
inline int fix_groups(int ntiles) { return ntiles <= 2048 ? ntiles : (ntiles + kFixTiles - 1) / kFixTiles; }

struct FastGrid {
  int ntx, nty, nbz;
  int frame;
};

struct HostStager {
  static constexpr size_t kChunk = (size_t)8 << 20, kMinBytes = (size_t)4 << 20;
  static constexpr int kSlots = 4;
  char* slot[kSlots] = {nullptr, nullptr, nullptr, nullptr};
  hipEvent_t ev[kSlots] = {nullptr, nullptr, nullptr, nullptr};
  hipEvent_t ev_order = nullptr;
  hipStream_t stream = nullptr;
  int pool = 0;
  ~HostStager();
  void release();
  hipError_t ensure();
  hipError_t upload(void* dev, const void* host, size_t bytes, hipStream_t compute);
  hipError_t download(void* host, const void* dev, size_t bytes, hipStream_t compute);
};

inline std::atomic<unsigned>& guard_cache_generation() {
  static std::atomic<unsigned> g{0};
  return g;
}
inline bool layer_has_guard_rows(const void* p, const Geo& g, size_t elem_bytes) {
  struct Entry {
    const void* p;
    int rows, cols, batch;
    unsigned gen;
    bool ok;
  };
  static thread_local Entry cache[8] = {};
  static thread_local int next = 0;
  const unsigned gen = guard_cache_generation().load(std::memory_order_acquire);
  for (const Entry& e : cache)
    if (e.p == p && e.rows == g.rows && e.cols == g.cols && e.batch == g.batch && e.gen == gen && p) return e.ok;
  bool ok = false;
  hipDeviceptr_t base = nullptr;
  size_t size = 0;
  if (p && hipMemGetAddressRange(&base, &size, (hipDeviceptr_t)p) == hipSuccess) {
    const size_t guard = (size_t)kSlabGuardRows * (size_t)g.rows * elem_bytes;
    const size_t layer = (size_t)g.rows * (size_t)g.cols * (size_t)(g.batch > 0 ? g.batch : 1) * elem_bytes;
    const char* lo = (const char*)base;
    const char* hi = lo + size;
    ok = (size_t)((const char*)p - lo) >= guard && (const char*)p + layer <= hi && (size_t)(hi - ((const char*)p + layer)) >= guard;
  } else {
    (void)hipGetLastError();
  }
  cache[next] = Entry{p, g.rows, g.cols, g.batch, gen, ok};
  next = (next + 1) & 7;
  return ok;
}

inline int device_cus() {
  static std::atomic<int> cache[64];
  int dev = 0, cus = 256;
  if (hipGetDevice(&dev) != hipSuccess) return cus;
  if (dev >= 0 && dev < 64) {
    const int v = cache[dev].load(std::memory_order_relaxed);
    if (v > 0) return v;
  }
  if (hipDeviceGetAttribute(&cus, hipDeviceAttributeMultiprocessorCount, dev) != hipSuccess || cus <= 0) cus = 256;
  if (dev >= 0 && dev < 64) cache[dev].store(cus, std::memory_order_relaxed);
  return cus;
}

hipError_t launch_filter(const Geo& g, const ChainParams& p, const Layers& L, int filter, unsigned flags,
                         hipStream_t stream);
hipError_t launch_chain(const Geo& g, const ChainParams& p, const Layers& L, const Region& r, unsigned flags,
                        hipStream_t stream);
hipError_t launch_footprint(const Geo& g, const FootprintParams& p, const Layers& L, const uint8_t* face_flags, const unsigned* ptab,
                            const int* clip_table, bool write_memo, const ChainParams* combine, double trav_cap, hipStream_t stream,
                            const Region* region = nullptr);
hipError_t launch_footprint_any(const Geo& g, const FootprintParams& p, const Layers& L, const Region* rf, hipStream_t s);
int chain_max_reach(const ChainParams& p);
inline int untrav_flag_ntx(int rows) { return (rows + 63) / 64; }
inline int untrav_flag_nfy(int cols) { return (cols + 3) / 4; }
inline size_t untrav_flag_bytes(int rows, int cols, int batch) { return (size_t)untrav_flag_ntx(rows) * (size_t)untrav_flag_nfy(cols) * (size_t)batch; }
hipError_t launch_check_circular_paths(const Geo& g, const float* footprint, double fp_default, const float* robot_slope,
                                       int n_paths, const int* pose_offset, const double* pose_xy, unsigned char* is_safe,
                                       double* traversability, int* status, hipStream_t stream);
hipError_t launch_check_inclination(const Geo& g, const float* robot_slope, int n, const double* start_end_xy,
                                    unsigned char* ok, int* status, hipStream_t stream);

struct PathDiscClass {
  const int4* spiral;
  int n_spiral, pad;
  double rmin, rmax, r2;
};
enum { kPdDiscs = 0, kPdOverflow = 1, kPdVisits = 2, kPdCounters = 4 };
struct PathDiscScratch {
  uint64_t* keys;
  float* vals;
  unsigned* list;
  unsigned* counters;
  uint64_t mask;
  unsigned list_cap;
};
hipError_t launch_path_discs(const Geo& g, const PathDiscScratch& s, const PathDiscClass* classes, const float* trav, const uint8_t* untrav,
                             double fp_default, const float* robot_slope, int n_paths, const int* pose_offset, const double* pose_xy,
                             const int* path_class, unsigned char* is_safe, double* traversability, int* status, hipStream_t stream);
hipError_t launch_footprint_mask(const Geo& g, const FootprintParams& p, const Layers& L, const uint8_t* face_flags, const ChainParams* combine,
                                 hipStream_t stream);

namespace any {
struct NormalsJob {
  Disc dn, dr;
  int same_disc, axis, rank_rule;
  int combine;
  int given_normals;
  double slope_crit, rough_crit;
  float w_scale, w_slope, w_step, w_rough;
};
hipError_t step_height(const Geo& g, const Disc& d, const float* elev, float* sh, const Region& r, hipStream_t s);
hipError_t step_score(const Geo& g, const Disc& d, double crit, int ncrit, const float* sh, float* out, const Region& r, hipStream_t s);
hipError_t normals(const Geo& g, const NormalsJob& a, const Layers& L, float* nx, float* ny, float* nz, const Region& r, hipStream_t s);
}

namespace fast {
bool step_height_fast(int Q, const Geo& g, const float* elev, float* sh, const Region& r, hipStream_t s);
bool step_score_fast(int Q, const Geo& g, double crit, int ncrit, const float* sh, float* out, const Region& r,
                     hipStream_t s);
bool step_height5(int Q, const Geo& g, const float* elev, float* sh, float* sh_min, const Region& r, hipStream_t s);
bool step_score5(int Q, const Geo& g, double crit, int ncrit, const float* sh, float* out, float* out_count, const Region& r, hipStream_t s);
bool step_height_ties(const Disc& d, const Geo& g, const float* elev, float* sh, float* scratch, const Region& r, hipStream_t s);
bool step_score_ties(const Disc& d, const Geo& g, double crit, int ncrit, const float* sh, float* out, float* scratch, const Region& r,
                     hipStream_t s);
bool normals_fast(const Geo& g, const ChainParams& p, const Layers& L, bool keep_normals, bool combine,
                  const Region& r, int* block_flags, const int* clip_table, FastGrid* fg, hipStream_t s, bool* combined);
bool roughness_given_fast(const Geo& g, const ChainParams& p, const Layers& L, const Region& r, int* block_flags, FastGrid* fg, hipStream_t s);
int footprint_inner_q(double res, double rmin, double rmax);
bool normals_fast3(const Geo& g, const ChainParams& p, const Layers& L, bool keep_normals, const Region& r, int* block_flags,
                   FastGrid* fg, hipStream_t s);
bool normals_small(const Geo& g, const ChainParams& p, const Layers& L, bool keep_normals, const Region& r, int* block_flags, FastGrid* fg,
                   hipStream_t s, bool write_step = false, bool combine = false);
bool chain_window(const Geo& g, const ChainParams& p, const Layers& L, bool keep_normals, const Region& r, bool combine, hipStream_t s);
int normals_fast_max_blocks(const Geo& g);
size_t normals_hole_queue_bytes();
bool footprint_slide5(const Geo& g, const FootprintParams& p, const Layers& L, const int* clip_table, const FpRoute& r, hipStream_t s,
                      const Region* region);
bool footprint_slide4(const Geo& g, const FootprintParams& p, const Layers& L, const int* clip_table, const FpRoute& r, hipStream_t s,
                      const Region* region);
bool footprint_slide3(const Geo& g, const FootprintParams& p, const Layers& L, const unsigned* ptab, const int* clip_table, hipStream_t s,
                      const Region* region);
constexpr int kClipInts = 6 * (2 * kMaxRadiusCells + 1) * (2 * kMaxRadiusCells + 1);
constexpr int kFpClipInts = 6 * 41 * 41;
void footprint_blocked4(const Geo& g, const FootprintParams& p, const Layers& L, const unsigned* ptab, hipStream_t s);
void build_clip_table(const Disc& d, int Rk, int* out);
}

}
```

### traversability_estimation_amd/csrc/te_paths_api.hip

```cpp
#include "te_ctx.h"
#include "te_fp_table.h"
#include "te_path_visit.h"

using namespace te;
using namespace te::shim;

namespace {
int path_disc_table(te_ctx* c, double radius, double offset, unsigned long long first_clock, std::vector<DevBuf>& temps,
                    PathDiscClass* out) {
  const Geo& g = c->geo;
  out->rmin = radius;
  out->rmax = radius + offset;
  out->r2 = out->rmax * out->rmax;
  out->pad = 0;
  te_ctx::PdTable* victim = nullptr;
  for (te_ctx::PdTable& t : c->lmem.pd_tables) {
    if (t.dev.p && t.radius == radius && t.offset == offset && t.res == g.res && t.rows == g.rows && t.cols == g.cols) {
      t.used = ++c->pd_clock;
      out->spiral = t.dev.as<const int4>();
      out->n_spiral = t.n_spiral;
      return TE_OK;
    }
    if ((!t.dev.p || t.used <= first_clock) && (!victim || (victim->dev.p && (!t.dev.p || t.used < victim->used)))) victim = &t;
  }
// ... 27 lines not shown
}
}

extern "C" {

int te_check_footprint_paths_radius(te_ctx* c, int map, int n_paths, const int* pose_offset, const double* pose_xy, const double* radius,
                                    double offset, unsigned char* is_safe, double* traversability, int* status,
                                    te_path_check_stats* stats) {
  if (!c || n_paths < 0 || (n_paths > 0 && (!pose_offset || !pose_xy || !radius || !is_safe || !traversability || !status)))
    return fail(TE_ERR_INVALID_ARG, "te_check_footprint_paths_radius: NULL argument");
  if (!isfinite(offset) || offset < 0.0) return fail(TE_ERR_INVALID_ARG, "te_check_footprint_paths_radius: offset %g", offset);
  for (int k = 0; k < n_paths; ++k)
    if (!isfinite(radius[k]) || radius[k] < 0.0)
      return fail(TE_ERR_INVALID_ARG, "te_check_footprint_paths_radius: radius[%d] = %g (a footprint radius is finite and not negative)", k, radius[k]);
  CtxLock lk(c);
  if (!c->have_geo || !c->chain_done || !c->tables_ready)
    return fail(TE_ERR_NOT_READY, "te_check_footprint_paths_radius: run the filter chain first (it produces the layers the discs read)");
  if (map < 0 || map >= c->geo.batch) return fail(TE_ERR_INVALID_ARG, "te_check_footprint_paths_radius: map %d of %d", map, c->geo.batch);
  if (c->check_inclination && !c->have_robot_slope)
    return fail(TE_ERR_NOT_READY, "te_check_footprint_paths_radius: check_robot_inclination is set but the layer robot_slope was never uploaded");
  if (stats) stats->n_visits = stats->n_discs = stats->n_radius_classes = 0;
  if (n_paths == 0) return TE_OK;
  const int n_poses = pose_offset[n_paths];
  if (pose_offset[0] != 0 || n_poses < 0) return fail(TE_ERR_INVALID_ARG, "te_check_footprint_paths_radius: bad pose offsets");
  for (int k = 0; k < n_paths; ++k)
    if (pose_offset[k + 1] < pose_offset[k]) return fail(TE_ERR_INVALID_ARG, "te_check_footprint_paths_radius: bad pose offsets");
  if (!c->fp_tables_ready) return fail(c->fp_tables_rc ? c->fp_tables_rc : TE_ERR_NOT_READY, "%s", c->fp_tables_err);
  const Geo& g = c->geo;
  std::vector<double> uniq;
  std::vector<int> cls;
  pv::class_radii(n_paths, radius, &uniq, &cls);
  if (uniq.size() > (size_t)pv::kMaxClasses)
    return fail(TE_ERR_UNSUPPORTED, "te_check_footprint_paths_radius: %zu distinct radii in one call (at most %d)", uniq.size(), pv::kMaxClasses);
  const pv::Geom hg = {g.rows, g.cols, g.res, g.len_x, g.len_y, g.pos_x, g.pos_y};
  unsigned long long n_visits = 0;
  for (int k = 0; k < n_paths; ++k)
    n_visits += (unsigned long long)pv::count_path_visits(hg, pose_offset[k + 1] - pose_offset[k], pose_xy + 2 * (size_t)pose_offset[k]);
  const uint64_t entries = pv::table_entries(n_visits);
  if (entries > ((uint64_t)1 << 31)) return fail(TE_ERR_UNSUPPORTED, "te_check_footprint_paths_radius: %llu centres in one call", n_visits);
  HIP_TRY(hipSetDevice(c->device));
  const unsigned long long first_clock = c->pd_clock;
  std::vector<PathDiscClass> classes(uniq.size());
  std::vector<DevBuf> temps;
  for (size_t q = 0; q < uniq.size(); ++q)
    if (const int rc = path_disc_table(c, uniq[q], offset, first_clock, temps, &classes[q])) return rc;
  const size_t list_cap = n_visits > 0 ? (size_t)n_visits : 1;
  Carve cv;
  const auto p_keys = cv.add<uint64_t>((size_t)entries);
  const auto p_xy = cv.add<double>((size_t)2 * (n_poses > 0 ? n_poses : 1));
  const auto p_trav = cv.add<double>(n_paths);
  const auto p_classes = cv.add<PathDiscClass>(classes.size());
  const auto p_off = cv.add<int>((size_t)n_paths + 1);
  const auto p_cls = cv.add<int>(n_paths);
  const auto p_st = cv.add<int>(n_paths);
  const auto p_vals = cv.add<float>((size_t)entries);
  const auto p_list = cv.add<unsigned>(list_cap);
  const auto p_cnt = cv.add<unsigned>(kPdCounters);
  const auto p_safe = cv.add<unsigned char>(n_paths);
  DevBuf& scratch = c->lmem.pd_scratch;
  if (const hipError_t e = scratch.reserve(cv.total, c->stream))
    return fail(TE_ERR_HIP, "te_check_footprint_paths_radius: hipMalloc(%zu bytes) for %llu centres: %s", cv.total, n_visits, hipGetErrorString(e));
  PathDiscScratch s;
  s.keys = p_keys.in(scratch);
  double* d_xy = p_xy.in(scratch);
  double* d_trav = p_trav.in(scratch);
  PathDiscClass* d_classes = p_classes.in(scratch);
  int* d_off = p_off.in(scratch);
  int* d_cls = p_cls.in(scratch);
  int* d_st = p_st.in(scratch);
  s.vals = p_vals.in(scratch);
  s.list = p_list.in(scratch);
  s.counters = p_cnt.in(scratch);
  unsigned char* d_safe = p_safe.in(scratch);
  s.mask = entries - 1;
  s.list_cap = (unsigned)list_cap;
  unsigned counters[kPdCounters] = {0, 0, 0, 0};
  hipError_t e = hipMemcpyAsync(d_off, pose_offset, p_off.bytes(), hipMemcpyHostToDevice, c->stream);
  if (e == hipSuccess && n_poses > 0) e = hipMemcpyAsync(d_xy, pose_xy, (size_t)2 * n_poses * sizeof(double), hipMemcpyHostToDevice, c->stream);
  if (e == hipSuccess) e = hipMemcpyAsync(d_cls, cls.data(), p_cls.bytes(), hipMemcpyHostToDevice, c->stream);
  if (e == hipSuccess) e = hipMemcpyAsync(d_classes, classes.data(), p_classes.bytes(), hipMemcpyHostToDevice, c->stream);
  if (e == hipSuccess) e = hipMemsetAsync(s.keys, 0xFF, p_keys.bytes(), c->stream);
  if (e == hipSuccess) e = hipMemsetAsync(s.counters, 0, p_cnt.bytes(), c->stream);
  if (e == hipSuccess && !c->mask_done) {
    e = launch_footprint_mask(g, c->fp, c->L, usable_face_flags(c), c->combine_deferred ? &c->cp : nullptr, c->stream);
    if (e == hipSuccess) {
      c->combine_deferred = false;
      c->mask_done = true;
    }
  }
  const size_t per = (size_t)g.rows * g.cols;
  if (e == hipSuccess)
    e = launch_path_discs(g, s, d_classes, c->L.trav + per * map, c->L.untrav + per * map, c->params.fp_default,
                          c->check_inclination ? c->lmem.robot_slope.as<float>() + per * map : nullptr, n_paths, d_off, d_xy, d_cls, d_safe, d_trav, d_st,
                          c->stream);
  if (e == hipSuccess) e = hipMemcpyAsync(is_safe, d_safe, p_safe.bytes(), hipMemcpyDeviceToHost, c->stream);
  if (e == hipSuccess) e = hipMemcpyAsync(traversability, d_trav, p_trav.bytes(), hipMemcpyDeviceToHost, c->stream);
  if (e == hipSuccess) e = hipMemcpyAsync(status, d_st, p_st.bytes(), hipMemcpyDeviceToHost, c->stream);
  if (e == hipSuccess) e = hipMemcpyAsync(counters, s.counters, p_cnt.bytes(), hipMemcpyDeviceToHost, c->stream);
  const hipError_t e_sync = hipStreamSynchronize(c->stream);
  if (e == hipSuccess) e = e_sync;
  if (e != hipSuccess) {
    (void)hipGetLastError();
    return fail(TE_ERR_HIP, "te_check_footprint_paths_radius: %s", hipGetErrorString(e));
  }
  if (counters[kPdOverflow])
    return fail(TE_ERR_UNSUPPORTED, "te_check_footprint_paths_radius: internal error: the memo of %llu entries (work list %zu) overflowed", (unsigned long long)entries, list_cap);
  if (counters[kPdVisits] != n_visits)
    return fail(TE_ERR_UNSUPPORTED, "te_check_footprint_paths_radius: internal error: the kernels visited %u centres, the plan counted %llu", counters[kPdVisits], n_visits);
  if (stats) {
    stats->n_visits = (int)counters[kPdVisits];
    stats->n_discs = (int)counters[kPdDiscs];
    stats->n_radius_classes = (int)uniq.size();
  }
  return TE_OK;
}

int te_check_footprint_paths(te_ctx* c, int map, int n_paths, const int* pose_offset, const double* pose_xy,
                             unsigned char* is_safe, double* traversability, int* status) {
  if (!c || n_paths < 0 || (n_paths > 0 && (!pose_offset || !pose_xy || !is_safe || !traversability || !status)))
    return fail(TE_ERR_INVALID_ARG, "te_check_footprint_paths: NULL argument");
  CtxLock lk(c);
  if (!c->have_geo || !c->footprint_done)
    return fail(TE_ERR_NOT_READY, "te_check_footprint_paths: run the chain with the footprint pass first");
  if (map < 0 || map >= c->geo.batch) return fail(TE_ERR_INVALID_ARG, "te_check_footprint_paths: map %d of %d", map, c->geo.batch);
  if (c->check_inclination && !c->have_robot_slope)
    return fail(TE_ERR_NOT_READY, "te_check_footprint_paths: check_robot_inclination is set but the layer robot_slope was never uploaded");
  if (n_paths == 0) return TE_OK;
  const int n_poses = pose_offset[n_paths];
  if (pose_offset[0] != 0 || n_poses < 0) return fail(TE_ERR_INVALID_ARG, "te_check_footprint_paths: bad pose offsets");
  for (int k = 0; k < n_paths; ++k)
    if (pose_offset[k + 1] < pose_offset[k]) return fail(TE_ERR_INVALID_ARG, "te_check_footprint_paths: bad pose offsets");
  HIP_TRY(hipSetDevice(c->device));
  Carve cv;
  const auto p_off = cv.add<int>((size_t)n_paths + 1);
  const auto p_xy = cv.add<double>((size_t)2 * (n_poses > 0 ? n_poses : 1));
  const auto p_trav = cv.add<double>(n_paths);
  const auto p_st = cv.add<int>(n_paths);
  const auto p_safe = cv.add<unsigned char>(n_paths);
  DevBuf tmp;
  HIP_TRY(tmp.once(cv.total));
  int* d_off = p_off.in(tmp);
  double* d_xy = p_xy.in(tmp);
  double* d_trav = p_trav.in(tmp);
  int* d_st = p_st.in(tmp);
  unsigned char* d_safe = p_safe.in(tmp);
  hipError_t e = hipMemcpyAsync(d_off, pose_offset, p_off.bytes(), hipMemcpyHostToDevice, c->stream);
  if (e == hipSuccess && n_poses > 0) e = hipMemcpyAsync(d_xy, pose_xy, (size_t)2 * n_poses * sizeof(double), hipMemcpyHostToDevice, c->stream);
  const size_t per = (size_t)c->geo.rows * c->geo.cols;
  if (e == hipSuccess)
    e = launch_check_circular_paths(c->geo, c->L.footprint + per * map, c->params.fp_default,
                                    c->check_inclination ? c->lmem.robot_slope.as<float>() + per * map : nullptr, n_paths, d_off, d_xy, d_safe,
                                    d_trav, d_st, c->stream);
  if (e == hipSuccess) e = hipMemcpyAsync(is_safe, d_safe, p_safe.bytes(), hipMemcpyDeviceToHost, c->stream);
  if (e == hipSuccess) e = hipMemcpyAsync(traversability, d_trav, p_trav.bytes(), hipMemcpyDeviceToHost, c->stream);
  if (e == hipSuccess) e = hipMemcpyAsync(status, d_st, p_st.bytes(), hipMemcpyDeviceToHost, c->stream);
  if (e == hipSuccess) e = hipStreamSynchronize(c->stream);
  if (e != hipSuccess) return fail(TE_ERR_HIP, "te_check_footprint_paths: %s", hipGetErrorString(e));
  return TE_OK;
}

int te_set_check_robot_inclination(te_ctx* c, int enabled) {
  if (!c) return fail(TE_ERR_INVALID_ARG, "te_set_check_robot_inclination: NULL");
  CtxLock lk(c);
  c->check_inclination = enabled != 0;
  return TE_OK;
}

// ... 303 lines not shown
```

### traversability_estimation_amd/csrc/te_shim.hip

```cpp
#include "te_ctx.h"
#include "te_fp_table.h"
#include "te_hole_routing.h"

using namespace te;
using namespace te::shim;

namespace te {
namespace shim {

thread_local char g_err[512] = "";

int fail(int code, const char* fmt, ...) {
  va_list ap;
  va_start(ap, fmt);
  vsnprintf(g_err, sizeof(g_err), fmt, ap);
  va_end(ap);
  return code;
}

int build_disc(double radius, double res, Disc* d, const char* what) {
  memset(d, 0, sizeof(*d));
  d->r2 = radius * radius;
  const double q = (radius / res) * (radius / res);
  const double tol = 1e-9 * (q > 1.0 ? q : 1.0);
// ... 30 lines not shown
      d->R = b;
      d->npoints += (b == 0 ? 1 : 2) * (2 * hw + 1);
    }
  }
  if (d->R > d->reach) d->reach = d->R;
  if (d->hw[0] > d->reach) d->reach = d->hw[0];
  d->Q = -1;
  if (d->n_ties == 0) {
    int best = -1;
    for (int a = 0; a <= lim; ++a)
      for (int b = 0; b <= lim; ++b) {
        const int m = a * a + b * b;
        if ((double)m < q && m > best) best = m;
      }
    d->Q = best;
  }
  return TE_OK;
}

int filter_disc(te_ctx* c, double radius, Disc* d, DiscTable* t, const char* what) {
  *t = DiscTable();
  if (c->opt_filter_any != 2) {
    char before[sizeof(g_err)];
    memcpy(before, g_err, sizeof(before));
    const int rc = build_disc(radius, c->geo.res, d, what);
    if (rc == TE_OK || c->opt_filter_any == 0) return rc;
    memcpy(g_err, before, sizeof(before));
  }
  build_disc_table(radius, c->geo.res, t);
  memset(d, 0, sizeof(*d));
  d->R = t->R;
  for (int b = 0; b <= kMaxRadiusCells; ++b) d->hw[b] = -1;
  d->n_ties = t->n_ties();
  d->r2 = t->r2;
  d->reach = t->reach;
  d->npoints = t->npoints < 0x7fffffff ? (int)t->npoints : 0x7fffffff;
  d->Q = -1;
  d->any = 1;
  d->any_hw0 = t->R >= 0 ? t->hw[0] : -1;
  d->tab = nullptr;
  return TE_OK;
}

int upload_any_discs(te_ctx* c) {
  Disc* ds[4] = {&c->cp.normals, &c->cp.rough, &c->cp.step1, &c->cp.step2};
  std::vector<int32_t> ints;
  size_t off[4] = {0, 0, 0, 0};
  for (int k = 0; k < 4; ++k) {
    if (!ds[k]->any) continue;
    off[k] = ints.size();
    ints.insert(ints.end(), c->fa_host[k].hw.begin(), c->fa_host[k].hw.end());
    ints.insert(ints.end(), c->fa_host[k].ties.begin(), c->fa_host[k].ties.end());
    ints.push_back(0);
  }
  if (ints.empty()) return TE_OK;
  const size_t bytes = ints.size() * sizeof(int32_t);
  HIP_TRY(hipSetDevice(c->device));
  if (c->cmem.fa_tab.reserve(bytes, c->stream) != hipSuccess)
    return fail(TE_ERR_UNSUPPORTED, "filter discs of any radius: their tables (%zu bytes) do not fit in device memory", bytes);
  HIP_TRY(hipMemcpyAsync(c->cmem.fa_tab.p, ints.data(), bytes, hipMemcpyHostToDevice, c->stream));
  HIP_TRY(hipStreamSynchronize(c->stream));
  for (int k = 0; k < 4; ++k)
    if (ds[k]->any) ds[k]->tab = c->cmem.fa_tab.as<const int>() + off[k];
  return TE_OK;
}

bool same_disc(const Disc& a, const Disc& b) {
  if (a.R != b.R || a.n_ties != b.n_ties) return false;
  for (int k = 0; k <= kMaxRadiusCells; ++k)
    if (a.hw[k] != b.hw[k]) return false;
  if (a.n_ties && a.r2 != b.r2) return false;
  return true;
}

}
}


namespace {
constexpr int kCfX = 64, kCfY = 32, kCfH = te::kFaceDilate + 1, kCfT = kCfY + 2 * kCfH, kCfWaves = 4, kCfG = 10;
static_assert(kCfX == te::kFaceGranI && kCfY % te::kFaceGranJ == 0 && kCfT <= 64 && kCfY / te::kFaceGranJ <= 64, "k_count_invalid: tile shape");
}
__global__ __launch_bounds__(64 * kCfWaves) void k_count_invalid(const float* __restrict__ v, int rows, int cols, double crit_step,
                                                                 uint8_t* __restrict__ flags, unsigned long long* __restrict__ out) {
  const int lane = threadIdx.x & 63, wave = threadIdx.x >> 6;
  const int ti = (int)blockIdx.x * kCfWaves + wave;
  if (ti >= te::face_flag_ntx(rows)) return;
  const int map = blockIdx.z, i0 = ti * kCfX, j0 = (int)blockIdx.y * kCfY;
  const size_t mo = (size_t)map * (size_t)rows * (size_t)cols;
  const float nan = __builtin_nanf("");
  const int i = i0 + lane, ic = i < rows ? i : rows - 1;
  const bool own = i < rows, has_up = i > 0;
  const int o_prev = ic - 1, o_prev0 = ic > 0 ? ic - 1 : 0, o_next = ic + 1 < rows ? ic + 1 : ic;
  const int xl = lane & 3;
  const int ix = xl < te::kFaceDilate ? i0 - te::kFaceDilate + xl : i0 + kCfX + xl - te::kFaceDilate;
  const bool xin = ix >= 0 && ix < rows;
  const int ixc = ix < 0 ? 0 : (ix < rows ? ix : rows - 1);
  const int ox_prev = ixc > 0 ? ixc - 1 : 0, ox_next = ixc + 1 < rows ? ixc + 1 : ixc;
  auto mn = [](float a, float b) { return __builtin_fminf(a, b); };
  unsigned cnt = 0, runs = 0;
  unsigned long long step_any = 0ull;
  float a0 = nan, a1 = nan, e1 = nan, x0 = nan, x1 = nan, ex1 = nan;
#pragma unroll
  for (int rb = 0; rb < kCfT; rb += kCfG) {
    float prev[kCfG], mid[kCfG], next[kCfG], xprev[kCfG], xmid[kCfG], xnext[kCfG];
#pragma unroll
    for (int q = 0; q < kCfG; ++q) {
      if (rb + q >= kCfT) continue;
      const int j = j0 - kCfH + rb + q;
      const size_t col = mo + (size_t)(j < 0 ? 0 : (j < cols ? j : cols - 1)) * rows;
      const float* __restrict__ cp = v + col;
      prev[q] = cp[col == 0 ? o_prev0 : o_prev], mid[q] = cp[ic], next[q] = cp[o_next];
      xprev[q] = cp[ox_prev], xmid[q] = cp[ixc], xnext[q] = cp[ox_next];
    }
#pragma unroll
    for (int q = 0; q < kCfG; ++q) {
      const int r = rb + q;
      if (r >= kCfT) continue;
      const int j = j0 - kCfH + r;
      const bool jin = j >= 0 && j < cols;
      const bool in = jin && own, inx = jin && xin;
      const float e2 = in ? mid[q] : nan, ex2 = inx ? xmid[q] : nan;
      const float a2 = in ? mn(mn(has_up ? prev[q] : mid[q], mid[q]), next[q]) : nan;
      const float x2 = inx ? mn(mn(xprev[q], xmid[q]), xnext[q]) : nan;
      if (r >= kCfH && r < kCfH + kCfY) {
        const bool bad = in && !__builtin_isfinite(mid[q]);
        const bool first = map == 0 && j == 0 && i == 0;
        cnt += bad ? 1u : 0u;
        runs += (bad && (first || __builtin_isfinite(prev[q]))) ? 1u : 0u;
      }
      if (r >= 2) {
        const bool hit = te::face_hit(mn(mn(a0, a1), a2), e1, crit_step) || te::face_hit(mn(mn(x0, x1), x2), ex1, crit_step);
        if (__ballot(hit) != 0ull) step_any |= 1ull << (r - 1);
      }
      a0 = a1, a1 = a2, e1 = e2;
      x0 = x1, x1 = x2, ex1 = ex2;
    }
  }
  for (int d = 32; d >= 1; d >>= 1) {
    cnt += __shfl_xor((int)cnt, d);
    runs += __shfl_xor((int)runs, d);
  }
  if (lane == 0 && cnt) {
    atomicAdd(out, (unsigned long long)cnt);
    if (runs) atomicAdd(out + 1, (unsigned long long)runs);
  }
  if (flags != nullptr && lane < kCfY / te::kFaceGranJ) {
    const int fj = j0 / te::kFaceGranJ + lane;
    if (fj < te::face_flag_nfy(cols)) {
      const unsigned long long span = (1ull << (te::kFaceGranJ + 2 * te::kFaceDilate)) - 1ull;
      const bool any = ((step_any >> (kCfH - te::kFaceDilate + te::kFaceGranJ * lane)) & span) != 0ull;
      flags[((size_t)map * (size_t)te::face_flag_nfy(cols) + (size_t)fj) * (size_t)te::face_flag_ntx(rows) + (size_t)ti] = any ? 1 : 0;
    }
  }
}


namespace te {
namespace shim {
void finish_prefetch_locked(te_ctx* c) {
  {
    std::unique_lock<std::mutex> pl(c->pf_mu);
    if (!c->prefetch_running && !c->prefetch_mask) return;
    c->pf_cv.wait(pl, [c] { return !c->prefetch_running; });
  }
  const unsigned mask = c->prefetch_mask;
  c->prefetch_mask = 0;
  c->prefetch_elev = false;
  const bool ok = c->prefetch_rc.load() == TE_OK;
  if (mask & (1u << TE_LAYER_ELEVATION)) {
    c->chain_done = false;
    c->footprint_done = false;
    c->mask_done = false;
    c->invalid_cells = -1;
    c->invalid_runs = -1;
    c->face_crit = __builtin_nan("");
    if (ok) {
      c->have_elev = true;
      if (hipSetDevice(c->device) != hipSuccess || count_invalid_elevation(c) != TE_OK) {
        (void)hipGetLastError();
        c->invalid_cells = -1;
        c->face_crit = __builtin_nan("");
      }
    } else {
      c->have_elev = false;
    }
  }
  if (ok) {
    if (mask & (1u << TE_LAYER_ROBOT_SLOPE)) c->have_robot_slope = true;
    if (mask & (1u << TE_LAYER_TRAVERSABILITY)) c->trav_external = c->trav_ptr_out = true;
  }
  if (mask & (bit(TE_LAYER_SLOPE) | bit(TE_LAYER_STEP) | bit(TE_LAYER_ROUGHNESS))) c->mask_done = false;
}
unsigned filter_layers(int filter) {
  const unsigned normals = bit(TE_LAYER_NORMAL_X) | bit(TE_LAYER_NORMAL_Y) | bit(TE_LAYER_NORMAL_Z);
  switch (filter) {
    case TE_FILTER_SLOPE: return bit(TE_LAYER_NORMAL_Z) | bit(TE_LAYER_SLOPE);
    case TE_FILTER_STEP: return bit(TE_LAYER_ELEVATION) | bit(TE_LAYER_STEP);
    case TE_FILTER_ROUGHNESS: return bit(TE_LAYER_ELEVATION) | normals | bit(TE_LAYER_ROUGHNESS);
    case TE_FILTER_COMBINE: return bit(TE_LAYER_SLOPE) | bit(TE_LAYER_STEP) | bit(TE_LAYER_ROUGHNESS) | bit(TE_LAYER_TRAVERSABILITY);
    case TE_FILTER_NORMALS: return bit(TE_LAYER_ELEVATION) | normals | bit(TE_LAYER_SLOPE) | bit(TE_LAYER_ROUGHNESS);
    default: return ~0u;
  }
}
}
}

namespace te {
namespace shim {

int count_invalid_elevation(te_ctx* c) {
  c->invalid_cells = -1;
  c->face_crit = __builtin_nan("");
  HIP_TRY(c->cmem.count.once(2 * sizeof(unsigned long long)));
  unsigned long long* const d_count = c->cmem.count.as<unsigned long long>();
  HIP_TRY(hipMemsetAsync(d_count, 0, 2 * sizeof(unsigned long long), c->stream));
  const bool with_flags = c->face_flags != nullptr;
  const double crit = c->params.fp_critical_step;
  const dim3 grid((unsigned)((face_flag_ntx(c->geo.rows) + kCfWaves - 1) / kCfWaves), (unsigned)((c->geo.cols + kCfY - 1) / kCfY), (unsigned)c->geo.batch);
  if (grid.y > 65535u || grid.z > 65535u) return fail(TE_ERR_UNSUPPORTED, "elevation layer of %d columns x %d maps: too many for one pass", c->geo.cols, c->geo.batch);
  hipLaunchKernelGGL(k_count_invalid, grid, dim3(64 * kCfWaves), 0, c->stream, c->L.elev, c->geo.rows, c->geo.cols, crit, c->face_flags, d_count);
  HIP_TRY(hipGetLastError());
  unsigned long long h[2] = {0, 0};
  HIP_TRY(hipMemcpyAsync(h, d_count, sizeof(h), hipMemcpyDeviceToHost, c->stream));
  HIP_TRY(hipStreamSynchronize(c->stream));
  c->invalid_cells = (long long)h[0];
  c->invalid_runs = (long long)h[1];
  if (with_flags) c->face_crit = crit;
  return TE_OK;
}

const uint8_t* usable_face_flags(const te_ctx* c) {
  return (c->opt_face_flags && c->face_flags && !c->elev_ptr_out && c->face_crit == c->fp.crit_step && c->face_crit == c->params.fp_critical_step)
             ? c->face_flags
             : nullptr;
}

HoleCounts hole_counts(const te_ctx* c) { return HoleCounts{(long long)c->layer_elems, c->invalid_cells, c->invalid_runs}; }
bool clustered_holes(const te_ctx* c) { return holes_clustered(hole_counts(c)); }
bool sparse_holes(const te_ctx* c) {
  static const int force = lab_int("TE_N3_HOLES", 0);
  if (force == 1 || force == 2) return force == 1;
  return holes_sparse(hole_counts(c));
}
bool skip_clean_march(const te_ctx* c) {
#ifdef TE_NO_SKIP_CLEAN
  return false;
#endif
  return sparse_holes(c) && holes_skip_clean_march(hole_counts(c));
}
bool short_strips(const te_ctx* c) {
  static const int force = lab_int("TE_N3_SHORT_STRIPS", -1);
  if (force >= 0) return force == 1 && c->invalid_cells > 0 && !sparse_holes(c);
  return clustered_holes(c) && !sparse_holes(c);
}

bool ensure_hole_queue(te_ctx* c) {
  if (c->cmem.hole_queue.p) return true;
  return hipSetDevice(c->device) == hipSuccess && c->cmem.hole_queue.once(fast::normals_hole_queue_bytes()) == hipSuccess;
}

void ensure_tie_scratch(te_ctx* c) {
  if (c->lmem.tie_scratch.p || !c->tables_ready || c->layer_elems == 0) return;
  if ((c->cp.step1.n_ties == 0 || c->cp.step1.any) && (c->cp.step2.n_ties == 0 || c->cp.step2.any)) return;
  if (hipSetDevice(c->device) == hipSuccess) (void)c->lmem.tie_scratch.once(c->layer_elems * sizeof(float));
}

void set_launch_hints(te_ctx* c) {
  c->L.sparse_holes = sparse_holes(c) && ensure_hole_queue(c) ? 1 : 0;
  c->L.no_holes = c->invalid_cells == 0 ? 1 : 0;
  c->L.skip_clean = c->L.sparse_holes && skip_clean_march(c) ? 1 : 0;
  c->L.short_strips = short_strips(c) ? 1 : 0;
  c->L.hole_queue = c->cmem.hole_queue.as<char>();
  ensure_tie_scratch(c);
  c->L.tie_scratch = c->lmem.tie_scratch.as<float>();
  c->cp.rank_rule = c->opt_rank_rule;
}

int refuse_rank_rule(te_ctx* c) {
  if (c->opt_rank_rule && c->cp.normals.any)
    return fail(TE_ERR_UNSUPPORTED, "TE_OPT_NORMALS_RANK_RULE is not supported with a normals disc of the route of any radius (%d cells)",
                c->cp.normals.R);
  return TE_OK;
}

void drop_graph(te_ctx* c) {
  for (int k = 0; k < te_ctx::kGraphs; ++k) {
    if (c->graph_exec[k]) (void)hipGraphExecDestroy(c->graph_exec[k]);
    c->graph_exec[k] = nullptr;
  }
}

void clear_fp_any_ptrs(te_ctx* c) {
  c->fp.any_spiral = nullptr;
  c->fp.any_ints = nullptr;
  c->fp.any_psum = nullptr;
  c->fp.any_pcnt = nullptr;
}
void release_fp_any(te_ctx* c) {
  c->lmem.fpa = te_ctx::LayerMem::FpAny();
  clear_fp_any_ptrs(c);
}

static int fp_any_alloc(te_ctx* c, DevBuf& buf, size_t bytes, const char* what) {
  if (buf.reserve(bytes, c->stream) == hipSuccess) return TE_OK;
  return fail(TE_ERR_UNSUPPORTED, "footprint radius %.3g m is %d cells: its %s (%zu bytes) do not fit in device memory", c->fp.rmax,
              c->fp.reach, what, bytes);
}

int build_fp_any_tables(te_ctx* c, const FpTable& t) {
  FootprintParams& f = c->fp;
  const Geo& g = c->geo;
  std::vector<int32_t> ints(t.hw.begin(), t.hw.end());
  f.any_R = t.R;
  f.any_inner_R = -1;
  f.any_k_inner = 0;
  const int inner_q = fast::footprint_inner_q(g.res, f.rmin, f.rmax);
  if (inner_q >= 0) {
// ... 110 lines not shown

void rebuild_footprint_tables(te_ctx* c) {
  c->fp_tables_ready = false;
  const int rc = rebuild_footprint_tables_impl(c);
  c->fp_tables_rc = rc;
  if (rc) {
    snprintf(c->fp_tables_err, sizeof(c->fp_tables_err), "%s", g_err);
    (void)hipGetLastError();
  } else {
    c->fp_tables_ready = true;
  }
}

int rebuild_tables(te_ctx* c) {
  c->tables_ready = false;
  c->fp_tables_ready = false;
  drop_graph(c);
  if (!c->have_params || !c->have_geo) return TE_OK;
  const te_params& p = c->params;
  const double res = c->geo.res;
  int rc;
  if ((rc = filter_disc(c, p.normals_radius, &c->cp.normals, &c->fa_host[0], "normals"))) return rc;
  if ((rc = filter_disc(c, p.rough_radius, &c->cp.rough, &c->fa_host[1], "roughness estimation"))) return rc;
  if ((rc = filter_disc(c, p.step_radius1, &c->cp.step1, &c->fa_host[2], "step first window"))) return rc;
  if ((rc = filter_disc(c, p.step_radius2, &c->cp.step2, &c->fa_host[3], "step second window"))) return rc;
  if ((rc = upload_any_discs(c))) return rc;
  if (c->cp.normals.any || c->cp.rough.any)
    c->cp.same_rough_disc = c->cp.normals.any && c->cp.rough.any && same_disc_table(c->fa_host[0], c->fa_host[1]) ? 1 : 0;
  else
    c->cp.same_rough_disc = same_disc(c->cp.normals, c->cp.rough) ? 1 : 0;
  c->cp.axis = p.normals_axis;
  c->cp.slope_crit = p.slope_critical;
  c->cp.step_crit = p.step_critical;
  c->cp.rough_crit = p.rough_critical;
  c->cp.step_ncrit = p.step_ncrit;
  c->cp.w_scale = p.w_scale;
  c->cp.w_slope = p.w_slope;
  c->cp.w_step = p.w_step;
  c->cp.w_rough = p.w_rough;
  if (!c->cp.normals.any && (c->cp.normals.R >= 1 || c->cp.normals.n_ties != 0)) {
    const Disc& dn = c->cp.normals;
    HIP_TRY(hipSetDevice(c->device));
    HIP_TRY(c->cmem.clip_table.once(sizeof(int) * (2 * fast::kClipInts + kMaxTies)));
    int* const clip_table = c->cmem.clip_table.as<int>();
    std::vector<int> tab, tab_full;
    int gen_tab[kMaxTies];
    if (dn.n_ties == 0) {
      const int R = dn.R;
      tab.resize((size_t)(2 * R + 1) * (2 * R + 1) * 6);
      fast::build_clip_table(dn, R, tab.data());
      HIP_TRY(hipMemcpyAsync(clip_table, tab.data(), tab.size() * sizeof(int), hipMemcpyHostToDevice, c->stream));
    } else {
      Disc full = dn;
      int n_gen = 0;
      for (int t = 0; t < dn.n_ties; ++t) {
        const int ai = abs((int)dn.tie_di[t]), aj = abs((int)dn.tie_dj[t]);
        if (full.hw[aj] < ai) full.hw[aj] = ai;
        if (full.R < aj) full.R = aj;
        if (dn.tie_di[t] != 0 && dn.tie_dj[t] != 0) gen_tab[n_gen++] = ((int)dn.tie_di[t] & 0xff) | (((int)dn.tie_dj[t] & 0xff) << 8);
      }
      const int R = dn.reach;
      tab_full.resize((size_t)(2 * R + 1) * (2 * R + 1) * 6);
      fast::build_clip_table(full, R, tab_full.data());
      HIP_TRY(hipMemcpyAsync(clip_table + fast::kClipInts, tab_full.data(), tab_full.size() * sizeof(int), hipMemcpyHostToDevice, c->stream));
      if (n_gen) HIP_TRY(hipMemcpyAsync(clip_table + 2 * fast::kClipInts, gen_tab, n_gen * sizeof(int), hipMemcpyHostToDevice, c->stream));
    }
    HIP_TRY(hipStreamSynchronize(c->stream));
  }
  c->L.clip_table = c->cmem.clip_table.as<int>();

  c->tables_ready = true;
  rebuild_footprint_tables(c);
  return TE_OK;
}

void free_layers(te_ctx* c) {
  drop_graph(c);
  c->lmem = te_ctx::LayerMem();
  memset(&c->L, 0, sizeof(c->L));
  c->face_flags = nullptr;
  c->poly_rot = nullptr;
  clear_fp_any_ptrs(c);
  c->face_crit = __builtin_nan("");
  c->elev_ptr_out = false;
  guard_cache_generation().fetch_add(1, std::memory_order_acq_rel);
  c->layers_written = 0;
  c->have_robot_slope = false;
  c->layer_elems = 0;
  c->trav_ptr_out = false;
  c->have_elev = false;
  c->chain_done = false;
  c->footprint_done = false;
  c->mask_done = false;
}

float* layer_ptr(te_ctx* c, int layer) {
  switch (layer) {
    case TE_LAYER_ELEVATION: return c->L.elev;
    case TE_LAYER_SLOPE: return c->L.slope;
    case TE_LAYER_STEP: return c->L.step;
    case TE_LAYER_ROUGHNESS: return c->L.rough;
    case TE_LAYER_TRAVERSABILITY: return c->L.trav;
    case TE_LAYER_FOOTPRINT: return c->L.footprint;
    case TE_LAYER_NORMAL_X: return c->L.nx;
    case TE_LAYER_NORMAL_Y: return c->L.ny;
    case TE_LAYER_NORMAL_Z: return c->L.nz;
    case TE_LAYER_SLOPE_FOOTPRINT: return c->L.slope_fp;
    case TE_LAYER_STEP_FOOTPRINT: return c->L.step_fp;
    case TE_LAYER_ROUGHNESS_FOOTPRINT: return c->L.rough_fp;
    case TE_LAYER_TRAVERSABILITY_X: return c->lmem.poly.as<float>();
    case TE_LAYER_TRAVERSABILITY_ROT: return c->poly_rot;
    case TE_LAYER_ROBOT_SLOPE: return c->lmem.robot_slope.as<float>();
    default: return nullptr;
  }
}

int ensure_input_layer(te_ctx* c, int layer) {
  c->layers_written |= bit(layer);
  DevBuf& rs = c->lmem.robot_slope;
  if (layer != TE_LAYER_ROBOT_SLOPE || rs.p) return TE_OK;
  HIP_TRY(hipSetDevice(c->device));
  HIP_TRY(rs.once(c->layer_elems * sizeof(float)));
  const hipError_t e = hipMemsetD32Async((hipDeviceptr_t)rs.p, 0x7fc00000, c->layer_elems, c->stream);
  if (e != hipSuccess) {
    rs.release();
    return fail(TE_ERR_HIP, "robot_slope layer: %s", hipGetErrorString(e));
  }
  return TE_OK;
}

constexpr unsigned kNormalLayers = bit(TE_LAYER_NORMAL_X) | bit(TE_LAYER_NORMAL_Y) | bit(TE_LAYER_NORMAL_Z);
constexpr unsigned kMemoLayers = bit(TE_LAYER_SLOPE_FOOTPRINT) | bit(TE_LAYER_STEP_FOOTPRINT) | bit(TE_LAYER_ROUGHNESS_FOOTPRINT);
static void note_normals_kept(te_ctx* c, unsigned flags) {
  if (flags & (TE_RUN_KEEP_NORMALS | TE_RUN_NORMALS_ONLY))
    c->layers_written |= kNormalLayers;
  else
    c->layers_written &= ~kNormalLayers;
}

int run_chain_locked(te_ctx* c, unsigned flags, const Region& r) {
  if (!c->have_params || !c->have_geo) return fail(TE_ERR_NOT_READY, "te_run_chain: set params and geometry first");
  if (!c->tables_ready) {
    int rc = rebuild_tables(c);
    if (rc) return rc;
  }
  if (!c->have_elev) return fail(TE_ERR_NOT_READY, "te_run_chain: no elevation uploaded");
  if (int rc = refuse_rank_rule(c)) return rc;
  HIP_TRY(hipSetDevice(c->device));
  static const bool force_two = lab_flag("TE_TWO_STREAMS");
  const bool small = !force_two && (size_t)c->geo.rows * c->geo.cols * c->geo.batch < ((size_t)1 << 21);
  c->L.aux_stream = ((flags & TE_RUN_SEQUENTIAL) || small) ? nullptr : c->aux_stream;
  if (flags & TE_RUN_NORMALS_ONLY) flags &= ~(TE_RUN_FOOTPRINT | TE_RUN_FOOTPRINT_MEMO);
  if ((flags & TE_RUN_FOOTPRINT) && !c->fp_tables_ready)
    return fail(c->fp_tables_rc ? c->fp_tables_rc : TE_ERR_NOT_READY, "%s", c->fp_tables_err[0] ? c->fp_tables_err : "footprint tables not built");
  c->combine_deferred = (r.map < 0) && !(flags & TE_RUN_SEQUENTIAL) && (flags & TE_RUN_FOOTPRINT);
  if (c->combine_deferred) flags |= kDeferCombine;
  c->L.ev_fork = c->ev_fork;
  c->L.ev_join = c->ev_join;
  c->L.fb_walk = c->opt_fb_walk;
  c->L.fb_blocks_per_cu = c->opt_fb_blocks_per_cu;
  set_launch_hints(c);
  if (c->opt_rank_rule) flags |= TE_RUN_GENERIC_KERNELS;
  HIP_TRY(launch_chain(c->geo, c->cp, c->L, r, flags, c->stream));
  c->chain_done = true;
  c->footprint_done = false;
  c->mask_done = false;
  if (r.map < 0) c->trav_external = false;
  if (r.map < 0) note_normals_kept(c, flags);
  return TE_OK;
}

int run_footprint_locked(te_ctx* c, unsigned flags, bool fresh = false) {
  if (!c->chain_done || !c->tables_ready)
    return fail(TE_ERR_NOT_READY, "te_run_footprint: run the filter chain first (it produces the layers the footprint reads)");
  if (!c->fp_tables_ready) return fail(c->fp_tables_rc ? c->fp_tables_rc : TE_ERR_NOT_READY, "%s", c->fp_tables_err);
  HIP_TRY(hipSetDevice(c->device));
  const ChainParams& q = c->cp;
  const bool bounded = !c->trav_external && (fresh || !c->trav_ptr_out) && q.w_scale >= 0.0f && q.w_slope >= 0.0f && q.w_step >= 0.0f && q.w_rough >= 0.0f;
  const double trav_cap = bounded ? (double)q.w_scale * ((double)q.w_slope + (double)q.w_step + (double)q.w_rough) : -1.0;
  HIP_TRY(launch_footprint(c->geo, c->fp, c->L, usable_face_flags(c), c->cmem.spiral.as<unsigned>(), c->cmem.fp_clip_table.as<int>(), (flags & TE_RUN_FOOTPRINT_MEMO) != 0,
                           c->combine_deferred ? &c->cp : nullptr, trav_cap, c->stream));
  c->combine_deferred = false;
  c->footprint_done = true;
  c->mask_done = true;
  if (flags & TE_RUN_FOOTPRINT_MEMO) c->layers_written |= kMemoLayers;
  return TE_OK;
}

int run_whole_locked(te_ctx* c, unsigned flags) {
  const Region r = {-1, 0, 0, c->geo.rows, c->geo.cols};
  static const bool no_graph = lab_flag("TE_NO_GRAPH");
  const bool large = c->opt_graph == 1 || (c->opt_graph == 0 && (size_t)c->geo.rows * c->geo.cols * c->geo.batch >= ((size_t)1 << 22));
  flags &= TE_RUN_KEEP_NORMALS | TE_RUN_FOOTPRINT | TE_RUN_GENERIC_KERNELS | TE_RUN_FOOTPRINT_MEMO | TE_RUN_SEQUENTIAL | TE_RUN_NORMALS_ONLY;
  if (c->opt_rank_rule) flags |= TE_RUN_GENERIC_KERNELS;
  if (flags & TE_RUN_NORMALS_ONLY) flags &= ~(TE_RUN_FOOTPRINT | TE_RUN_FOOTPRINT_MEMO);
  if (!no_graph && large && !(flags & TE_RUN_NORMALS_ONLY) && c->graph_ok && c->have_params && c->have_geo && c->have_elev) {
    if (!c->tables_ready) {
      int rc = rebuild_tables(c);
      if (rc) return rc;
    }
    if (int rc = refuse_rank_rule(c)) return rc;
    HIP_TRY(hipSetDevice(c->device));
    int slot = -1;
    ensure_tie_scratch(c);
    const unsigned key = flags | (((flags & TE_RUN_FOOTPRINT) && usable_face_flags(c)) ? 0x08000000u : 0u) | (sparse_holes(c) && ensure_hole_queue(c) ? 0x80000000u : 0u) | (c->invalid_cells == 0 ? 0x40000000u : 0u) | (skip_clean_march(c) ? 0x20000000u : 0u) | (short_strips(c) ? 0x10000000u : 0u);
    for (int k = 0; k < te_ctx::kGraphs; ++k)
      if (c->graph_exec[k] && c->graph_flags[k] == key) slot = k;
    if (slot < 0) {
      slot = c->graph_next;
      c->graph_next = (c->graph_next + 1) % te_ctx::kGraphs;
      if (c->graph_exec[slot]) (void)hipGraphExecDestroy(c->graph_exec[slot]);
      c->graph_exec[slot] = nullptr;
      hipGraph_t graph = nullptr;
      int rc = TE_OK;
      hipError_t e = hipStreamBeginCapture(c->stream, hipStreamCaptureModeRelaxed);
      if (e == hipSuccess) {
        rc = run_chain_locked(c, flags, r);
        if (!rc && (flags & TE_RUN_FOOTPRINT)) rc = run_footprint_locked(c, flags, true);
        e = hipStreamEndCapture(c->stream, &graph);
      }
      if (e == hipSuccess && rc == TE_OK && graph) e = hipGraphInstantiate(&c->graph_exec[slot], graph, nullptr, nullptr, 0);
      if (graph) (void)hipGraphDestroy(graph);
      if (e != hipSuccess || rc != TE_OK || !c->graph_exec[slot]) {
        (void)hipGetLastError();
        drop_graph(c);
        c->graph_ok = false;
        slot = -1;
      } else {
        c->graph_flags[slot] = key;
      }
    }
    if (slot >= 0) {
      TraceRange tr("te_run_chain: graph replay (chain + footprint kernels)");
      HIP_TRY(hipGraphLaunch(c->graph_exec[slot], c->stream));
      c->trav_external = false;
      c->chain_done = true;
      c->footprint_done = (flags & TE_RUN_FOOTPRINT) != 0;
      c->mask_done = c->footprint_done;
      c->combine_deferred = false;
      note_normals_kept(c, flags);
      if ((flags & TE_RUN_FOOTPRINT) && (flags & TE_RUN_FOOTPRINT_MEMO)) c->layers_written |= kMemoLayers;
      return TE_OK;
    }
  }
  int rc = run_chain_locked(c, flags, r);
  if (!rc && (flags & TE_RUN_FOOTPRINT)) rc = run_footprint_locked(c, flags, true);
  return rc;
}

int sync_tiles(te_ctx* c) {
  if (!c->tiles_pending) return TE_OK;
  if (c->in_stream) HIP_TRY(hipStreamSynchronize(c->in_stream));
  if (c->out_stream) HIP_TRY(hipStreamSynchronize(c->out_stream));
  c->tiles_pending = false;
  return TE_OK;
}

}
}

extern "C" {

const char* te_last_error(void) { return g_err; }
const char* te_version(void) { return "travgpu 0.1 (gfx950)"; }

int te_params_default(te_params* p) {
  if (!p) return fail(TE_ERR_INVALID_ARG, "te_params_default: NULL");
  memset(p, 0, sizeof(*p));
  p->size = (uint32_t)sizeof(te_params);
  p->abi_version = TE_ABI_VERSION;
  p->normals_radius = 0.05;
  p->normals_axis = 2;
  p->slope_critical = 1.0;
  p->step_critical = 0.12;
  p->step_radius1 = 0.04;
  p->step_radius2 = 0.04;
  p->step_ncrit = 4;
  p->rough_critical = 0.05;
  p->rough_radius = 0.05;
  p->w_scale = 1.0f / 3.0f;
  p->w_slope = p->w_step = p->w_rough = 1.0f;
  p->fp_radius = 0.30;
  p->fp_offset = 0.15;
  p->fp_default = 0.3;
  p->fp_max_gap = 0.3;
  p->fp_critical_step = 0.12;
  p->fp_check_roughness = 0;
  return TE_OK;
}

int te_params_validate(const te_params* p) {
  if (!p) return fail(TE_ERR_INVALID_ARG, "te_params: NULL");
  if (p->size != sizeof(te_params) || p->abi_version != TE_ABI_VERSION)
    return fail(TE_ERR_INVALID_ARG, "te_params: size/abi mismatch (got %u/%u, want %zu/%d)", p->size, p->abi_version,
                sizeof(te_params), TE_ABI_VERSION);
  if (!(p->slope_critical <= M_PI_2 && p->slope_critical >= 0.0))
    return fail(TE_ERR_BAD_PARAM, "Critical slope must be in the interval [0, PI/2]");
  if (!(p->step_critical >= 0.0))
    return fail(TE_ERR_BAD_PARAM, "Critical step height must be greater than zero.");
  if (!(p->step_radius1 >= 0.0))
    return fail(TE_ERR_BAD_PARAM, "'first_window_radius' must be greater than zero.");
  if (!(p->step_radius2 >= 0.0))
    return fail(TE_ERR_BAD_PARAM, "'second_window_radius' must be greater than zero.");
  if (p->step_ncrit <= 0)
    return fail(TE_ERR_BAD_PARAM, "'critical_cell_number' must be greater than zero.");
  if (!(p->rough_critical >= 0.0))
    return fail(TE_ERR_BAD_PARAM, "Critical roughness must be greater than zero");
  if (!(p->rough_radius >= 0.0))
    return fail(TE_ERR_BAD_PARAM, "Roughness estimation radius must be greater than zero");
  if (!(p->normals_radius >= 0.0)) return fail(TE_ERR_BAD_PARAM, "normals radius must not be negative");
  if (p->normals_axis < 0 || p->normals_axis > 2)
    return fail(TE_ERR_BAD_PARAM, "normal_vector_positive_axis must be x, y or z");
// ... 90 lines not shown
      if (sl->freed) (void)hipEventDestroy(sl->freed);
    }
    if (c->stream) (void)hipStreamDestroy(c->stream);
  }
  delete c;
  return TE_OK;
}

int te_set_params(te_ctx* c, const te_params* p) {
  if (!c) return fail(TE_ERR_INVALID_ARG, "te_set_params: NULL ctx");
  int rc = te_params_validate(p);
  if (rc) return rc;
  CtxLock lk(c,  true);
  te_params old = c->params;
  c->params = *p;
  c->have_params = true;
  rc = rebuild_tables(c);
  if (rc) {
    c->params = old;
    (void)rebuild_tables(c);
    return rc;
  }
  if (memcmp(&old, p, offsetof(te_params, fp_radius)) != 0) c->chain_done = false;
  c->mask_done = c->mask_done && c->chain_done && old.fp_max_gap == p->fp_max_gap &&
                      old.fp_critical_step == p->fp_critical_step && old.fp_check_roughness == p->fp_check_roughness;
  c->footprint_done = false;
  if (!(old.fp_critical_step == p->fp_critical_step)) c->face_crit = __builtin_nan("");
  return TE_OK;
}

int te_set_option(te_ctx* c, int option, int value) {
  if (!c) return fail(TE_ERR_INVALID_ARG, "te_set_option: NULL ctx");
  CtxLock lk(c);
  switch (option) {
    case TE_OPT_FP_BLOCKED_WALK:
      if (value < 0 || value > 2) return fail(TE_ERR_INVALID_ARG, "te_set_option: TE_OPT_FP_BLOCKED_WALK takes 0 (by list length), 1 (per wavefront), 2 (per lane)");
      c->opt_fb_walk = value;
      break;
    case TE_OPT_FP_BLOCKED_BLOCKS_PER_CU:
      if (value < 0 || value > 32) return fail(TE_ERR_INVALID_ARG, "te_set_option: TE_OPT_FP_BLOCKED_BLOCKS_PER_CU takes 0 (default) .. 32");
      c->opt_fb_blocks_per_cu = value;
      break;
    case TE_OPT_POLYGON_PER_CELL:
      c->opt_polygon_per_cell = value != 0;
      break;
    case TE_OPT_GRAPH_REPLAY:
      if (value < 0 || value > 2) return fail(TE_ERR_INVALID_ARG, "te_set_option: TE_OPT_GRAPH_REPLAY takes 0 (by size), 1 (always), 2 (never)");
      c->opt_graph = value;
      break;
    case TE_OPT_BCAST_RCCL:
      c->opt_bcast_rccl = value != 0;
      return TE_OK;
    case TE_OPT_FP_ANY_REACH:
      if (value < 0 || value > 1) return fail(TE_ERR_INVALID_ARG, "te_set_option: TE_OPT_FP_ANY_REACH takes 0 (by reach) or 1 (every reach)");
      if (c->opt_fp_any != value) {
        c->opt_fp_any = value;
        c->footprint_done = false;
        if (c->tables_ready) rebuild_footprint_tables(c);
      }
      break;
    case TE_OPT_FILTER_ANY_RADIUS:
      if (value < 0 || value > 2)
        return fail(TE_ERR_INVALID_ARG, "te_set_option: TE_OPT_FILTER_ANY_RADIUS takes 0 (up to 32 cells), 1 (any radius), 2 (the route of any radius for every disc)");
      if (c->opt_filter_any != value) {
        const int old = c->opt_filter_any;
        c->opt_filter_any = value;
        if (c->have_params && c->have_geo) {
          const int rc = rebuild_tables(c);
          if (rc) {
            c->opt_filter_any = old;
            (void)rebuild_tables(c);
            return rc;
          }
        }
        c->chain_done = false;
        c->footprint_done = false;
        c->mask_done = false;
      }
      break;
    case TE_OPT_FACE_FLAGS:
      if (value < 0 || value > 1) return fail(TE_ERR_INVALID_ARG, "te_set_option: TE_OPT_FACE_FLAGS takes 0 (never passed to the mask kernel) or 1 (passed when known)");
      c->opt_face_flags = value;
      break;
    case TE_OPT_NORMALS_RANK_RULE:
      c->opt_rank_rule = value != 0;
      c->chain_done = false;
      c->footprint_done = false;
      c->mask_done = false;
      break;
    default:
      return fail(TE_ERR_INVALID_ARG, "te_set_option: unknown option %d", option);
  }
  drop_graph(c);
  return TE_OK;
}

int te_download_face_flags(te_ctx* c, unsigned char* out, size_t bytes) {
  if (!c || !out) return fail(TE_ERR_INVALID_ARG, "te_download_face_flags: NULL");
  CtxLock lk(c);
  const uint8_t* f = c->have_geo && c->have_elev ? usable_face_flags(c) : nullptr;
  if (!f) return fail(TE_ERR_NOT_READY, "te_download_face_flags: the face flags of the elevation layer are unknown or switched off");
  const size_t n = face_flag_bytes(c->geo.rows, c->geo.cols, c->geo.batch);
  if (bytes != n) return fail(TE_ERR_INVALID_ARG, "te_download_face_flags: %zu bytes given, the flags are %zu", bytes, n);
  HIP_TRY(hipSetDevice(c->device));
  HIP_TRY(hipMemcpyAsync(out, f, n, hipMemcpyDeviceToHost, c->stream));
  HIP_TRY(hipStreamSynchronize(c->stream));
  return TE_OK;
}

int te_get_params(te_ctx* c, te_params* p) {
  if (!c || !p) return fail(TE_ERR_INVALID_ARG, "te_get_params: NULL");
  CtxLock lk(c,  true);
  *p = c->params;
  return TE_OK;
}

int te_set_geometry(te_ctx* c, int rows, int cols, int batch, double res, double pos_x, double pos_y) {
  if (!c) return fail(TE_ERR_INVALID_ARG, "te_set_geometry: NULL ctx");
  if (rows <= 0 || cols <= 0 || batch <= 0 || !(res > 0.0) || !isfinite(res) || !isfinite(pos_x) || !isfinite(pos_y))
    return fail(TE_ERR_INVALID_ARG, "te_set_geometry: rows=%d cols=%d batch=%d res=%g", rows, cols, batch, res);
  CtxLock lk(c);
  HIP_TRY(hipSetDevice(c->device));
  HIP_TRY(hipStreamSynchronize(c->stream));
  const size_t elems = (size_t)rows * cols * batch;
  if (elems != c->layer_elems || rows != c->geo.rows || cols != c->geo.cols || batch != c->geo.batch) {
    free_layers(c);
    Geo gtmp;
    gtmp.rows = rows;
    gtmp.cols = cols;
    gtmp.batch = batch;
    const SlabPlan sp = plan_slab(rows, cols, batch, (size_t)fast::normals_fast_max_blocks(gtmp), fast::fp_list_slack(rows, cols, batch, device_cus()),
                                  untrav_flag_bytes(rows, cols, batch), face_flag_bytes(rows, cols, batch));
    const hipError_t e = c->lmem.slab.once(sp.total);
    if (e != hipSuccess) return fail(TE_ERR_HIP, "te_set_geometry: hipMalloc(%zu bytes): %s", sp.total, hipGetErrorString(e));
    char* const slab = c->lmem.slab.as<char>();
    float** ptrs[kSlabFloatLayers] = {&c->L.elev, &c->L.slope, &c->L.step,     &c->L.rough,   &c->L.trav,     &c->L.footprint, &c->L.nx,
                                      &c->L.ny,   &c->L.nz,    &c->L.slope_fp, &c->L.step_fp, &c->L.rough_fp, &c->L.step_height};
    for (int k = 0; k < kSlabFloatLayers; ++k) *ptrs[k] = (float*)(slab + sp.layer_off(k));
    const bool have_list = sp.list_cap < ((size_t)1 << 32);
    c->L.untrav = (uint8_t*)(slab + sp.mask.off);
    c->L.block_flags = (int*)(slab + sp.fix_flags.off);
    c->L.fp_blocked = have_list ? (unsigned*)(slab + sp.list.off) : nullptr;
    c->L.fp_blocked_count = (unsigned*)(slab + sp.list_count.off);
    c->L.fp_blocked_cap = sp.list_cap;
    c->L.untrav_flags = (uint8_t*)(slab + sp.untrav_flags.off);
    c->L.fp_scratch = have_list ? (unsigned*)(slab + sp.sum_scratch.off) : nullptr;
    c->face_flags = (uint8_t*)(slab + sp.face_flags.off);
    c->face_crit = __builtin_nan("");
    c->layer_elems = elems;
    HIP_TRY(hipMemsetAsync(slab, 0xFF, sp.list.off, c->stream));
    HIP_TRY(hipMemsetAsync(slab + sp.back_guard.off, 0xFF, sp.back_guard.bytes, c->stream));
    HIP_TRY(hipMemsetAsync(c->face_flags, 0x01, sp.face_flags.bytes, c->stream));
    HIP_TRY(hipMemsetAsync(c->L.untrav_flags, 0x01, sp.untrav_flags.bytes, c->stream));
    HIP_TRY(hipMemsetAsync(c->L.untrav, 0x01, sp.mask.bytes, c->stream));
    HIP_TRY(hipMemsetAsync(c->L.fp_blocked_count, 0, sp.list_count.bytes, c->stream));
    HIP_TRY(hipMemsetAsync(c->L.block_flags, 0, sp.fix_flags.bytes, c->stream));
  }
  c->geo.rows = rows;
  c->geo.cols = cols;
  c->geo.batch = batch;
  c->geo.res = res;
  c->geo.len_x = (double)rows * res;
  c->geo.len_y = (double)cols * res;
  c->geo.pos_x = pos_x;
  c->geo.pos_y = pos_y;
  c->geo.ax = pos_x + (0.5 * c->geo.len_x - 0.5 * res);
  c->geo.ay = pos_y + (0.5 * c->geo.len_y - 0.5 * res);
  c->have_geo = true;
  c->chain_done = false;
  c->footprint_done = false;
  c->mask_done = false;
  return rebuild_tables(c);
}

int te_run_filter(te_ctx* c, int filter, unsigned flags) {
  if (!c) return fail(TE_ERR_INVALID_ARG, "te_run_filter: NULL ctx");
  static const char* const kFilterRange[] = {"te_run_filter", "te_run_filter: slope", "te_run_filter: step", "te_run_filter: roughness",
                                             "te_run_filter: combine", "te_run_filter: normals"};
  TraceRange tr(kFilterRange[(filter >= 0 && filter < 6) ? filter : 0]);
  CtxLock lk(c,  true, filter_layers(filter));
  if (!c->have_geo || !c->have_params) return fail(TE_ERR_NOT_READY, "te_run_filter: set params and geometry first");
  if (!c->tables_ready) {
    int rc = rebuild_tables(c);
    if (rc) return rc;
  }
  if (filter < TE_FILTER_SLOPE || filter > TE_FILTER_NORMALS) return fail(TE_ERR_INVALID_ARG, "te_run_filter: bad filter %d", filter);
  if ((filter == TE_FILTER_STEP || filter == TE_FILTER_ROUGHNESS || filter == TE_FILTER_NORMALS) && !c->have_elev)
    return fail(TE_ERR_NOT_READY, "te_run_filter: no elevation uploaded");
  if (filter == TE_FILTER_NORMALS)
    if (int rc = refuse_rank_rule(c)) return rc;
  HIP_TRY(hipSetDevice(c->device));
  set_launch_hints(c);
  if (c->opt_rank_rule) flags |= TE_RUN_GENERIC_KERNELS;
  HIP_TRY(launch_filter(c->geo, c->cp, c->L, filter, flags, c->stream));
  c->chain_done = false;
  c->footprint_done = false;
  c->mask_done = false;
  c->trav_external = true;
  if (filter == TE_FILTER_NORMALS) c->layers_written |= kNormalLayers;
  return TE_OK;
}

int te_run_chain(te_ctx* c, unsigned flags) {
  if (!c) return fail(TE_ERR_INVALID_ARG, "te_run_chain: NULL ctx");
  TraceRange tr("te_run_chain");
  CtxLock lk(c);
  if (!c->have_geo) return fail(TE_ERR_NOT_READY, "te_run_chain: geometry not set");
  return run_whole_locked(c, flags);
}

int te_run_chain_region(te_ctx* c, unsigned flags, int map, int row0, int col0, int h, int w) {
  if (!c) return fail(TE_ERR_INVALID_ARG, "te_run_chain_region: NULL ctx");
  TraceRange tr("te_run_chain_region");
  CtxLock lk(c);
  if (!c->have_geo) return fail(TE_ERR_NOT_READY, "te_run_chain_region: geometry not set");
  if (map < 0 || map >= c->geo.batch || row0 < 0 || col0 < 0 || h <= 0 || w <= 0 || row0 + h > c->geo.rows ||
      col0 + w > c->geo.cols)
    return fail(TE_ERR_INVALID_ARG, "te_run_chain_region: rectangle outside the map");
  if (!c->chain_done) return fail(TE_ERR_NOT_READY, "te_run_chain_region: run the full chain once first");
  const Region r = {map, row0, col0, row0 + h, col0 + w};
  const bool want_fp = (flags & (TE_RUN_FOOTPRINT | TE_RUN_FOOTPRINT_MEMO)) != 0;
  const bool fp_was_done = c->footprint_done, mask_was_done = c->mask_done;
  if (want_fp && !fp_was_done)
    return fail(TE_ERR_NOT_READY, "te_run_chain_region: the footprint flag refreshes a complete traversability_footprint layer; run the "
                                  "whole-map footprint pass once first (te_run_chain with TE_RUN_FOOTPRINT, or te_run_footprint)");
  int rc = run_chain_locked(c, flags & ~(TE_RUN_FOOTPRINT | TE_RUN_FOOTPRINT_MEMO), r);
  if (rc || !want_fp) return rc;
  const int gap_cells = (int)ceil(c->params.fp_max_gap / c->geo.res) + 5;
  const int reach = chain_max_reach(c->cp);
  const int grow = reach > gap_cells - 3 ? reach : gap_cells - 3;
  Region changed = r;
  changed.i0 = r.i0 - grow < 0 ? 0 : r.i0 - grow;
  changed.j0 = r.j0 - grow < 0 ? 0 : r.j0 - grow;
  changed.i1 = r.i1 + grow > c->geo.rows ? c->geo.rows : r.i1 + grow;
  changed.j1 = r.j1 + grow > c->geo.cols ? c->geo.cols : r.j1 + grow;
  const ChainParams& q = c->cp;
  const bool bounded = !c->trav_external && !c->trav_ptr_out && q.w_scale >= 0.0f && q.w_slope >= 0.0f && q.w_step >= 0.0f && q.w_rough >= 0.0f;
  const double trav_cap = bounded ? (double)q.w_scale * ((double)q.w_slope + (double)q.w_step + (double)q.w_rough) : -1.0;
  HIP_TRY(launch_footprint(c->geo, c->fp, c->L, usable_face_flags(c), c->cmem.spiral.as<unsigned>(), c->cmem.fp_clip_table.as<int>(), (flags & TE_RUN_FOOTPRINT_MEMO) != 0, nullptr, trav_cap,
                           c->stream, &changed));
  c->footprint_done = true;
  c->mask_done = mask_was_done;
  return TE_OK;
}

int te_run_footprint(te_ctx* c) {
  if (!c) return fail(TE_ERR_INVALID_ARG, "te_run_footprint: NULL ctx");
  TraceRange tr("te_run_footprint");
  CtxLock lk(c);
  return run_footprint_locked(c, TE_RUN_FOOTPRINT_MEMO);
}

int te_sync(te_ctx* c) {
  if (!c) return fail(TE_ERR_INVALID_ARG, "te_sync: NULL ctx");
  CtxLock lk(c);
  HIP_TRY(hipSetDevice(c->device));
  static const long spin_us = lab_int("TE_SYNC_SPIN_US", 2000);
  if (spin_us > 0) {
    const auto t0 = std::chrono::steady_clock::now();
    for (;;) {
      const hipError_t e = hipStreamQuery(c->stream);
      if (e == hipSuccess) return sync_tiles(c);
      if (e != hipErrorNotReady) return fail(TE_ERR_HIP, "te_sync: %s", hipGetErrorString(e));
      if (std::chrono::duration_cast<std::chrono::microseconds>(std::chrono::steady_clock::now() - t0).count() > spin_us) break;
    }
  }
  HIP_TRY(hipStreamSynchronize(c->stream));
  return sync_tiles(c);
}

int te_time_chain(te_ctx* c, unsigned flags, int warmup, int iters, float* ms_per_iter) {
  if (!c || !ms_per_iter || iters <= 0 || warmup < 0) return fail(TE_ERR_INVALID_ARG, "te_time_chain: bad argument");
  CtxLock lk(c);
  if (!c->have_geo) return fail(TE_ERR_NOT_READY, "te_time_chain: geometry not set");
  for (int k = 0; k < warmup; ++k) {
    int rc = run_whole_locked(c, flags);
    if (rc) return rc;
  }
  HIP_TRY(hipEventRecord(c->ev0, c->stream));
  for (int k = 0; k < iters; ++k) {
    int rc = run_whole_locked(c, flags);
    if (rc) return rc;
  }
  HIP_TRY(hipEventRecord(c->ev1, c->stream));
  HIP_TRY(hipEventSynchronize(c->ev1));
  float ms = 0.f;
  HIP_TRY(hipEventElapsedTime(&ms, c->ev0, c->ev1));
  *ms_per_iter = ms / (float)iters;
  return TE_OK;
}

int te_time_chain_samples(te_ctx* c, unsigned flags, int warmup, int iters, float* ms) {
  if (!c || !ms || iters <= 0 || warmup < 0) return fail(TE_ERR_INVALID_ARG, "te_time_chain_samples: bad argument");
  CtxLock lk(c);
  if (!c->have_geo) return fail(TE_ERR_NOT_READY, "te_time_chain_samples: geometry not set");
  for (int k = 0; k < warmup; ++k) {
    int rc = run_whole_locked(c, flags);
    if (rc) return rc;
  }
  for (int k = 0; k < iters; ++k) {
    HIP_TRY(hipEventRecord(c->ev0, c->stream));
    int rc = run_whole_locked(c, flags);
    if (rc) return rc;
    HIP_TRY(hipEventRecord(c->ev1, c->stream));
    HIP_TRY(hipEventSynchronize(c->ev1));
    HIP_TRY(hipEventElapsedTime(&ms[k], c->ev0, c->ev1));
  }
  return TE_OK;
}

}
```

Baseline: 50.12 billion cells/s.

## Split footprint mask into lean flat-tile kernel plus listed non-flat tiles

Adds a 'lean' route for the footprint mask. The invalid-elevation count kernel now also emits a compacted list of non-flat 64x32 face tiles. The full mask kernel then launches only over that list, and a separate lightweight vectorised kernel handles tiles that face flags prove flat. The aim is to avoid running the heavy shared-memory tile machinery on flat tiles. The cost is extra list bookkeeping, a graph-cache key on the tile count, and new code paths that could diverge from the original.

```diff
diff --git a/include/travgpu.h b/include/travgpu.h
--- a/include/travgpu.h
+++ b/include/travgpu.h
@@ -98,7 +98,10 @@
 #define TE_OPT_NORMALS_RANK_RULE 6
 #define TE_OPT_FILTER_ANY_RADIUS 8
 #define TE_OPT_FACE_FLAGS 9
+#define TE_OPT_MASK_LEAN 10
 int te_set_option(te_ctx* ctx, int option, int value);
+int te_download_mask_state(te_ctx* ctx, unsigned char* mask, size_t mask_bytes, unsigned char* tile_flags, size_t flag_bytes, unsigned* face_tiles,
+                           size_t tile_capacity, long long* n_face_tiles, int* lean_route);
 int te_download_face_flags(te_ctx* ctx, unsigned char* out, size_t bytes);
 int te_set_geometry(te_ctx* ctx, int rows, int cols, int batch, double resolution, double pos_x, double pos_y);
 
diff --git a/traversability_estimation_amd/capi.py b/traversability_estimation_amd/capi.py
--- a/traversability_estimation_amd/capi.py
+++ b/traversability_estimation_amd/capi.py
@@ -26,10 +26,11 @@
 OPT_FP_BLOCKED_WALK, OPT_FP_BLOCKED_BLOCKS_PER_CU, OPT_POLYGON_PER_CELL, OPT_GRAPH_REPLAY, OPT_BCAST_RCCL, OPT_NORMALS_RANK_RULE = 1, 2, 3, 4, 5, 6
 OPT_FP_ANY_REACH = 7
 OPT_FACE_FLAGS = 9
+OPT_MASK_LEAN = 10
 OPT_FILTER_ANY_RADIUS = 8
 
 SYMBOLS = ["te_params_default", "te_params_validate", "te_device_count", "te_create", "te_destroy",
-           "te_set_params", "te_get_params", "te_set_option", "te_download_face_flags", "te_set_geometry", "te_upload_elevation", "te_upload_tile", "te_download_tile",
+           "te_set_params", "te_get_params", "te_set_option", "te_download_face_flags", "te_download_mask_state", "te_set_geometry", "te_upload_elevation", "te_upload_tile", "te_download_tile",
            "te_upload_tile_async", "te_download_tile_async",
            "te_device_ptr", "te_set_layer_present", "te_upload_layer", "te_prefetch_layers", "te_wait_prefetch", "te_upload_layer_circular", "te_download_layer_circular", "te_run_filter", "te_run_chain", "te_run_chain_region", "te_run_footprint", "te_check_footprint_paths", "te_check_footprint_paths_radius",
            "te_sync",
@@ -167,6 +168,9 @@
         L.te_set_option.argtypes = [vp, C.c_int, C.c_int]
         if "TRAVGPU_LIB" not in os.environ or hasattr(L, "te_download_face_flags"):
             L.te_download_face_flags.argtypes = [vp, C.POINTER(C.c_ubyte), C.c_size_t]
+        if "TRAVGPU_LIB" not in os.environ or hasattr(L, "te_download_mask_state"):
+            L.te_download_mask_state.argtypes = [vp, C.POINTER(C.c_ubyte), C.c_size_t, C.POINTER(C.c_ubyte), C.c_size_t, C.POINTER(C.c_uint), C.c_size_t,
+                                                 C.POINTER(C.c_longlong), C.POINTER(C.c_int)]
         L.te_set_geometry.argtypes = [vp, C.c_int, C.c_int, C.c_int, C.c_double, C.c_double, C.c_double]
         L.te_upload_elevation.argtypes = [vp, fp, C.c_int, C.c_int]
         L.te_upload_tile.argtypes = [vp, fp, C.c_int, C.c_int, C.c_int, C.c_int, C.c_int]
@@ -488,6 +492,18 @@
         _check(load().te_download_face_flags(self._h, out.ctypes.data_as(C.POINTER(C.c_ubyte)), out.size))
         return out
 
+    def download_mask_state(self, mask=True):
+        m = np.empty((self.batch, self.cols, self.rows), np.uint8) if mask else None
+        f = np.empty((self.batch, (self.cols + 3) // 4, (self.rows + 63) // 64), np.uint8) if mask else None
+        cap = self.batch * ((self.cols + 31) // 32) * ((self.rows + 63) // 64)
+        t = np.zeros(cap, np.uint32)
+        n, lean = C.c_longlong(-1), C.c_int(0)
+        ub = C.POINTER(C.c_ubyte)
+        _check(load().te_download_mask_state(self._h, m.ctypes.data_as(ub) if mask else None, m.size if mask else 0,
+                                             f.ctypes.data_as(ub) if mask else None, f.size if mask else 0,
+                                             t.ctypes.data_as(C.POINTER(C.c_uint)), cap, C.byref(n), C.byref(lean)))
+        return dict(mask=m, tile_flags=f, face_tiles=None if n.value < 0 else np.sort(t[:n.value]), lean=bool(lean.value))
+
     def get_params(self):
         p = TeParams()
         _check(load().te_get_params(self._h, C.byref(p)))
diff --git a/traversability_estimation_amd/csrc/te_ctx.h b/traversability_estimation_amd/csrc/te_ctx.h
--- a/traversability_estimation_amd/csrc/te_ctx.h
+++ b/traversability_estimation_amd/csrc/te_ctx.h
@@ -55,6 +55,7 @@
   };
   static constexpr int kPdTables = 16;
   struct LayerMem {
+    te::DevBuf face_tiles;
     te::DevBuf slab;
     te::DevBuf poly;
     te::DevBuf poly_stream;
@@ -100,6 +101,10 @@
   double face_crit = __builtin_nan("");
   bool elev_ptr_out = false;
   int opt_face_flags = 1;
+  bool face_tiles_known = false;
+  unsigned face_tile_count = 0;
+  int face_tiles_edge_fail = 0;
+  int opt_mask_lean = 1;
   bool tables_ready = false;
   bool fp_tables_ready = false;
   int fp_tables_rc = TE_OK;
@@ -107,6 +112,7 @@
   static constexpr int kGraphs = 4;
   hipGraphExec_t graph_exec[kGraphs] = {nullptr, nullptr, nullptr, nullptr};
   unsigned graph_flags[kGraphs] = {0, 0, 0, 0};
+  unsigned graph_tiles[kGraphs] = {0, 0, 0, 0};
   int graph_next = 0;
   bool graph_ok = true;
   struct TileSlot {
@@ -143,6 +149,7 @@
 constexpr unsigned bit(int layer) { return (layer >= 0 && layer < 32) ? 1u << layer : 0u; }
 int count_invalid_elevation(te_ctx* c);
 const uint8_t* usable_face_flags(const te_ctx* c);
+te::FaceInfo usable_face_info(const te_ctx* c);
 float* layer_ptr(te_ctx* c, int layer);
 int ensure_input_layer(te_ctx* c, int layer);
 int rebuild_tables(te_ctx* c);
diff --git a/traversability_estimation_amd/csrc/te_face_flags.h b/traversability_estimation_amd/csrc/te_face_flags.h
--- a/traversability_estimation_amd/csrc/te_face_flags.h
+++ b/traversability_estimation_amd/csrc/te_face_flags.h
@@ -42,7 +42,34 @@
   return any == 0;
 }
 
+constexpr int kFaceTileRows = 32;
+TE_FF_HD int face_tile_nty(int cols) { return (cols + kFaceTileRows - 1) / kFaceTileRows; }
+TE_FF_HD size_t face_tile_total(int rows, int cols, int batch) {
+  return (size_t)face_flag_ntx(rows) * (size_t)face_tile_nty(cols) * (size_t)batch;
+}
+TE_FF_HD bool face_tile_flat(const uint8_t* flags, int rows, int cols, int edge_fail, int map, int i0, int j0, int tw, int th) {
+  return face_tile_clear(flags, rows, cols, map, i0, j0, th) &&
+         !(edge_fail != 0 && face_tile_near_failing_border(rows, cols, edge_fail, i0, j0, tw, th));
+}
+
+constexpr long kMaskLeanTiles = 1024;
+inline bool mask_route_lean(bool flags_known, bool list_known, bool region, bool q5, int opt, int rows, int cols, int batch) {
+  if (!flags_known || !list_known || region || !q5 || opt <= 0) return false;
+  return opt >= 2 || (long)face_tile_total(rows, cols, batch > 0 ? batch : 1) >= kMaskLeanTiles;
+}
+
 #if !defined(__HIP_DEVICE_COMPILE__)
+inline size_t face_tile_list_host(const uint8_t* flags, int rows, int cols, int batch, int edge_fail, unsigned* out) {
+  const int ntx = face_flag_ntx(rows), nty = face_tile_nty(cols);
+  size_t n = 0;
+  for (int m = 0; m < batch; ++m)
+    for (int tj = 0; tj < nty; ++tj)
+      for (int ti = 0; ti < ntx; ++ti)
+        if (!face_tile_flat(flags, rows, cols, edge_fail, m, ti * kFaceGranI, tj * kFaceTileRows, kFaceGranI, kFaceTileRows))
+          out[n++] = (unsigned)(((size_t)m * nty + tj) * ntx + ti);
+  return n;
+}
+
 inline void face_flags_host(const float* elev, int rows, int cols, int batch, double crit_step, uint8_t* flags, uint8_t* hit = nullptr) {
   const size_t nflags = face_flag_bytes(rows, cols, batch);
   for (size_t k = 0; k < nflags; ++k) flags[k] = 0;
diff --git a/traversability_estimation_amd/csrc/te_footprint.hip b/traversability_estimation_amd/csrc/te_footprint.hip
--- a/traversability_estimation_amd/csrc/te_footprint.hip
+++ b/traversability_estimation_amd/csrc/te_footprint.hip
@@ -295,7 +295,47 @@
   int flag_ntx, flag_nfy;
   const uint8_t* face_flags;
   int whatif;
+  const unsigned* tile_list;
+  int tile_ntx, tile_nty;
 };
+
+__device__ __forceinline__ bool mask_tile_flat(const Geo& g, const MaskArgs& a, int map, int i0, int j0, int my) {
+  const bool q5 = a.step_disc.Q == 5 && a.step_disc.n_ties == 0;
+  if (!(a.face_flags != nullptr && q5 && a.whatif == 0)) return false;
+  return face_tile_flat(a.face_flags, g.rows, g.cols, a.edge_fail, map, i0, j0, MX, my);
+}
+__device__ __forceinline__ float mask_combine(const MaskArgs& a, float c_slope, float c_step, float c_rough) {
+  const float ta = a.w_slope * c_slope, tb = a.w_step * c_step, tc = a.w_rough * c_rough;
+  const float tab = ta + tb;
+  const float tabc = tab + tc;
+  return a.w_scale * tabc;
+}
+__device__ __forceinline__ bool mask_cell_slow(const MaskArgs& a, float c_slope, float c_rough, bool step_fast) {
+  return (c_slope == 0.0f) || !step_fast || (a.check_rough && c_rough == 0.0f);
+}
+__device__ __forceinline__ float mask_fast_step_memo(float c_step) { return (c_step == 0.0f) ? 1.0f : qnanf(); }
+struct SlowVerdict {
+  bool ok;
+  float m_slope, m_step, m_rough;
+};
+template <typename StepOk>
+__device__ __forceinline__ SlowVerdict mask_slow_cell(const Geo& g, const MaskArgs& a, const TileView& vl, const TileView& vr, int ci, int j,
+                                                      float c_slope, float c_step, float c_rough, StepOk&& step_ok) {
+  SlowVerdict v = {true, qnanf(), qnanf(), qnanf()};
+  if (c_slope == 0.0f) {
+    v.ok = count_zero_ok(g, a.slope_disc, vl, ci, j, a.ncrit_slope);
+    v.m_slope = v.ok ? 1.0f : 0.0f;
+  }
+  if (v.ok && c_step == 0.0f) {
+    v.ok = step_ok();
+    v.m_step = v.ok ? 1.0f : 0.0f;
+  }
+  if (v.ok && a.check_rough && c_rough == 0.0f) {
+    v.ok = count_zero_ok(g, a.slope_disc, vr, ci, j, a.ncrit_rough);
+    v.m_rough = v.ok ? 1.0f : 0.0f;
+  }
+  return v;
+}
 
 template <int MY>
 __global__ __launch_bounds__(MX* MBY) __attribute__((amdgpu_waves_per_eu(4, 4))) void k_fp_mask(Geo g, MaskArgs a, const float* __restrict__ elev,
@@ -307,17 +347,21 @@
   __shared__ float t_elev[MTW * MTH], t_key[MTW * MTH], t_kl[MTW * MTH];
   __shared__ int ntodo, arrived, members, compacted, nkl;
   if (threadIdx.x == 0 && threadIdx.y == 0) ntodo = arrived = members = compacted = nkl = 0;
-  const size_t mo = (size_t)(a.map >= 0 ? a.map : (int)blockIdx.z) * g.rows * g.cols;
-  const int i0 = ((int)blockIdx.x + a.ti0) * MX, j0 = ((int)blockIdx.y + a.tj0) * MY;
+  int bx = (int)blockIdx.x + a.ti0, by = (int)blockIdx.y + a.tj0, map = a.map >= 0 ? a.map : (int)blockIdx.z;
+  if (a.tile_list != nullptr) {
+    const unsigned e = a.tile_list[blockIdx.x];
+    bx = (int)(e % (unsigned)a.tile_ntx);
+    by = (int)((e / (unsigned)a.tile_ntx) % (unsigned)a.tile_nty);
+    map = (int)(e / ((unsigned)a.tile_ntx * (unsigned)a.tile_nty));
+  }
+  const size_t mo = (size_t)map * g.rows * g.cols;
+  const int i0 = bx * MX, j0 = by * MY;
   if (a.blocked_count && threadIdx.x == 0 && threadIdx.y == 0 && blockIdx.x == 0 && blockIdx.y == 0 && blockIdx.z == 0)
     a.blocked_count[0] = a.blocked_count[1] = a.blocked_count[4] = 0u;
   const bool q5 = a.step_disc.Q == 5 && a.step_disc.n_ties == 0;
-  bool flat = false;
-  if (a.face_flags != nullptr && q5 && a.whatif == 0)
-    flat = face_tile_clear(a.face_flags, g.rows, g.cols, a.map >= 0 ? a.map : (int)blockIdx.z, i0, j0, MY) &&
-           !(a.edge_fail != 0 && face_tile_near_failing_border(g.rows, g.cols, a.edge_fail, i0, j0, MX, MY));
+  bool flat = mask_tile_flat(g, a, map, i0, j0, MY);
   flat = __builtin_amdgcn_readfirstlane(flat ? 1 : 0) != 0;
-  uint8_t* const my_flags = a.untrav_flags + ((size_t)(a.map >= 0 ? a.map : (int)blockIdx.z) * a.flag_nfy) * a.flag_ntx + (i0 >> 6);
+  uint8_t* const my_flags = a.untrav_flags + ((size_t)map * a.flag_nfy) * a.flag_ntx + (i0 >> 6);
   {
     constexpr int NF = MY / 4;
     const int t = threadIdx.y * MX + threadIdx.x;
@@ -463,20 +507,15 @@
       near_bad_edge = ((a.edge_fail & 1) && i <= 2) || ((a.edge_fail & 2) && i >= g.rows - 3) || ((a.edge_fail & 4) && j <= 2) ||
                       ((a.edge_fail & 8) && j >= g.cols - 3);
     const bool step_fast = !(c_step == 0.0f) || (q5 && ((screen_mask >> c) & 1u) != 0 && !near_bad_edge);
-    const bool slow = (c_slope == 0.0f) || !step_fast || (a.check_rough && c_rough == 0.0f);
+    const bool slow = mask_cell_slow(a, c_slope, c_rough, step_fast);
     slow_mask |= (slow && j < g.cols && in_map) ? (1u << c) : 0u;
     if (j < g.cols && in_map) {
       const size_t o = mo + (size_t)j * g.rows + i;
       if (!slow) untrav[o] = 0;
-      if (a.combine) {
-        const float ta = a.w_slope * c_slope, tb = a.w_step * c_step, tc = a.w_rough * c_rough;
-        const float tab = ta + tb;
-        const float tabc = tab + tc;
-        trav[o] = a.w_scale * tabc;
-      }
+      if (a.combine) trav[o] = mask_combine(a, c_slope, c_step, c_rough);
       if (a.write_memo && !slow) {
         slope_fp[o] = qnanf();
-        step_fp[o] = (c_step == 0.0f) ? 1.0f : qnanf();
+        step_fp[o] = mask_fast_step_memo(c_step);
         rough_fp[o] = qnanf();
       }
     }
@@ -655,29 +694,175 @@
     const int ci = i0 + li, j = j0 + lj;
     const size_t o = mo + (size_t)j * g.rows + ci;
     const float c_slope = slope[o], c_step = step[o], c_rough = (a.check_rough || a.combine) ? rough[o] : 1.0f;
-    float m_slope = qnanf(), m_step = qnanf(), m_rough = qnanf();
-    bool ok = true;
-    if (c_slope == 0.0f) {
-      ok = count_zero_ok(g, a.slope_disc, vl, ci, j, a.ncrit_slope);
-      m_slope = ok ? 1.0f : 0.0f;
-    }
-    if (ok && c_step == 0.0f) {
+    const SlowVerdict v = mask_slow_cell(g, a, vl, vr, ci, j, c_slope, c_step, c_rough, [&]() __attribute__((always_inline)) {
       const bool screen_ok = screened;
       const bool near_bad_edge = a.edge_fail && (((a.edge_fail & 1) && ci <= 2) || ((a.edge_fail & 2) && ci >= g.rows - 3) ||
                                                   ((a.edge_fail & 4) && j <= 2) || ((a.edge_fail & 8) && j >= g.cols - 3));
-      ok = flat || (screen_ok && !near_bad_edge) || check_step(g, a.step_disc, ve, vs, ci, j, a.crit_step, a.max_gap, a.edge_fail);
-      m_step = ok ? 1.0f : 0.0f;
-    }
-    if (ok && a.check_rough && c_rough == 0.0f) {
-      ok = count_zero_ok(g, a.slope_disc, vr, ci, j, a.ncrit_rough);
-      m_rough = ok ? 1.0f : 0.0f;
-    }
-    untrav[o] = ok ? 0 : 1;
-    if (!ok) my_flags[(size_t)(j >> 2) * a.flag_ntx] = 1;
+      return flat || (screen_ok && !near_bad_edge) || check_step(g, a.step_disc, ve, vs, ci, j, a.crit_step, a.max_gap, a.edge_fail);
+    });
+    untrav[o] = v.ok ? 0 : 1;
+    if (!v.ok) my_flags[(size_t)(j >> 2) * a.flag_ntx] = 1;
     if (a.write_memo) {
-      slope_fp[o] = m_slope;
-      step_fp[o] = m_step;
-      rough_fp[o] = m_rough;
+      slope_fp[o] = v.m_slope;
+      step_fp[o] = v.m_step;
+      rough_fp[o] = v.m_rough;
+    }
+  }
+}
+
+constexpr int kFlatThreads = 256, kFlatWaves = kFlatThreads / kLanes;
+__device__ __forceinline__ int nth_set_bit(unsigned long long m, int n) {
+  int pos = 0;
+#pragma unroll
+  for (int w = 32; w >= 1; w >>= 1) {
+    const int c = __popcll((m >> pos) & ((1ull << w) - 1ull));
+    if (n >= c) {
+      n -= c;
+      pos += w;
+    }
+  }
+  return pos;
+}
+template <bool VEC>
+__global__ __launch_bounds__(kFlatThreads) void k_fp_mask_flat(Geo g, MaskArgs a, int n_tiles, const float* __restrict__ slope,
+                                                                const float* __restrict__ step, const float* __restrict__ rough,
+                                                                uint8_t* __restrict__ untrav, float* __restrict__ slope_fp,
+                                                                float* __restrict__ step_fp, float* __restrict__ rough_fp,
+                                                                float* __restrict__ trav) {
+  constexpr int NG = kFaceTileRows / kFaceGranJ / kFlatWaves;
+  static_assert(MX == kFaceGranI && NG * kFlatWaves * kFaceGranJ == kFaceTileRows, "k_fp_mask_flat: a wavefront per 64 x 4 granule");
+  const int lane = threadIdx.x & (kLanes - 1), wave = threadIdx.x / kLanes;
+  const int lq = lane & 15, lr = lane >> 4;
+  if (a.blocked_count && threadIdx.x == 0 && blockIdx.x == 0) a.blocked_count[0] = a.blocked_count[1] = a.blocked_count[4] = 0u;
+  const bool need_rough = a.check_rough || a.combine;
+  for (int t = blockIdx.x; t < n_tiles; t += gridDim.x) {
+    const int ti = t % a.tile_ntx, tj = (t / a.tile_ntx) % a.tile_nty, map = t / (a.tile_ntx * a.tile_nty);
+    const int i0 = ti * MX, j0 = tj * kFaceTileRows;
+    if (__builtin_amdgcn_readfirstlane(mask_tile_flat(g, a, map, i0, j0, kFaceTileRows) ? 1 : 0) == 0) continue;
+    const size_t mo = (size_t)map * g.rows * g.cols;
+    uint8_t* const my_flags = a.untrav_flags + ((size_t)map * a.flag_nfy) * a.flag_ntx + ti;
+    const TileView vl = {nullptr, slope + mo, i0, j0, g.rows, 0}, vr = {nullptr, rough + mo, i0, j0, g.rows, 0};
+    const int i = i0 + 4 * lq;
+    float c_slope[NG][4], c_step[NG][4], c_rough[NG][4];
+#pragma unroll
+    for (int h = 0; h < NG; ++h) {
+      int j = j0 + kFaceGranJ * (wave + kFlatWaves * h) + lr;
+      j = j < g.cols ? j : g.cols - 1;
+      if (VEC) {
+        const size_t o = mo + (size_t)j * g.rows + (i + 3 < g.rows ? i : g.rows - 4);
+        const float4 vs = *reinterpret_cast<const float4*>(slope + o), vt = *reinterpret_cast<const float4*>(step + o);
+        float4 vo = make_float4(1.0f, 1.0f, 1.0f, 1.0f);
+        if (need_rough) vo = *reinterpret_cast<const float4*>(rough + o);
+        c_slope[h][0] = vs.x, c_slope[h][1] = vs.y, c_slope[h][2] = vs.z, c_slope[h][3] = vs.w;
+        c_step[h][0] = vt.x, c_step[h][1] = vt.y, c_step[h][2] = vt.z, c_step[h][3] = vt.w;
+        c_rough[h][0] = vo.x, c_rough[h][1] = vo.y, c_rough[h][2] = vo.z, c_rough[h][3] = vo.w;
+      } else {
+#pragma unroll
+        for (int c = 0; c < 4; ++c) {
+          const size_t o = mo + (size_t)j * g.rows + (i + c < g.rows ? i + c : g.rows - 1);
+          c_slope[h][c] = slope[o];
+          c_step[h][c] = step[o];
+          c_rough[h][c] = need_rough ? rough[o] : 1.0f;
+        }
+      }
+    }
+#pragma unroll
+    for (int h = 0; h < NG; ++h) {
+      const int gq = wave + kFlatWaves * h, fj = (j0 >> 2) + gq;
+      if (fj >= a.flag_nfy) continue;
+      const int j = j0 + kFaceGranJ * gq + lr;
+      const bool row_in = j < g.cols;
+      const size_t o0 = mo + (size_t)j * g.rows + i;
+      unsigned in_mask = 0, slow_mask = 0;
+      float tr[4];
+#pragma unroll
+      for (int c = 0; c < 4; ++c) {
+        const bool in = row_in && i + c < g.rows;
+        in_mask |= in ? (1u << c) : 0u;
+        slow_mask |= (in && mask_cell_slow(a, c_slope[h][c], c_rough[h][c], true)) ? (1u << c) : 0u;
+        tr[c] = mask_combine(a, c_slope[h][c], c_step[h][c], c_rough[h][c]);
+      }
+      if (a.combine) {
+        if (VEC) {
+          if (in_mask) *reinterpret_cast<float4*>(trav + o0) = make_float4(tr[0], tr[1], tr[2], tr[3]);
+        } else {
+#pragma unroll
+          for (int c = 0; c < 4; ++c)
+            if ((in_mask >> c) & 1u) trav[o0 + c] = tr[c];
+        }
+      }
+      bool bad = false;
+      if (__ballot(slow_mask != 0u) == 0ull) {
+        if (VEC) {
+          if (in_mask) {
+            *reinterpret_cast<unsigned*>(untrav + o0) = 0u;
+            if (a.write_memo) {
+              const float n = qnanf();
+              *reinterpret_cast<float4*>(slope_fp + o0) = make_float4(n, n, n, n);
+              *reinterpret_cast<float4*>(step_fp + o0) = make_float4(mask_fast_step_memo(c_step[h][0]), mask_fast_step_memo(c_step[h][1]),
+                                                                     mask_fast_step_memo(c_step[h][2]), mask_fast_step_memo(c_step[h][3]));
+              *reinterpret_cast<float4*>(rough_fp + o0) = make_float4(n, n, n, n);
+            }
+          }
+        } else {
+#pragma unroll
+          for (int c = 0; c < 4; ++c)
+            if ((in_mask >> c) & 1u) {
+              untrav[o0 + c] = 0;
+              if (a.write_memo) {
+                slope_fp[o0 + c] = qnanf();
+                step_fp[o0 + c] = mask_fast_step_memo(c_step[h][c]);
+                rough_fp[o0 + c] = qnanf();
+              }
+            }
+        }
+      } else {
+#pragma unroll
+        for (int c = 0; c < 4; ++c)
+          if (((in_mask & ~slow_mask) >> c) & 1u) {
+            untrav[o0 + c] = 0;
+            if (a.write_memo) {
+              slope_fp[o0 + c] = qnanf();
+              step_fp[o0 + c] = mask_fast_step_memo(c_step[h][c]);
+              rough_fp[o0 + c] = qnanf();
+            }
+          }
+        unsigned long long bm[4];
+        int total = 0;
+#pragma unroll
+        for (int c = 0; c < 4; ++c) {
+          bm[c] = __ballot(((slow_mask >> c) & 1u) != 0u);
+          total += __popcll(bm[c]);
+        }
+#pragma unroll 1
+        for (int k = lane; k < total; k += kLanes) {
+          int n = k, c = 0;
+          unsigned long long m = bm[0];
+#pragma unroll
+          for (int cc = 0; cc < 3; ++cc) {
+            const int pc = __popcll(bm[cc]);
+            if (c == cc && n >= pc) {
+              n -= pc;
+              c = cc + 1;
+              m = bm[cc + 1];
+            }
+          }
+          const int src = nth_set_bit(m, n);
+          const int ci = i0 + 4 * (src & 15) + c, cj = j0 + kFaceGranJ * gq + (src >> 4);
+          const size_t o = mo + (size_t)cj * g.rows + ci;
+          const float s_slope = slope[o], s_step = step[o], s_rough = need_rough ? rough[o] : 1.0f;
+          const SlowVerdict v = mask_slow_cell(g, a, vl, vr, ci, cj, s_slope, s_step, s_rough, []() { return true; });
+          untrav[o] = v.ok ? 0 : 1;
+          bad |= !v.ok;
+          if (a.write_memo) {
+            slope_fp[o] = v.m_slope;
+            step_fp[o] = v.m_step;
+            rough_fp[o] = v.m_rough;
+          }
+        }
+      }
+      const bool any_bad = __ballot(bad) != 0ull;
+      if (lane == 0) my_flags[(size_t)fj * a.flag_ntx] = any_bad ? 1 : 0;
     }
   }
 }
@@ -1063,7 +1248,7 @@
   }
 }
 
-void launch_mask_pass(const Geo& g, const FootprintParams& p, const Layers& L, const uint8_t* face_flags, bool write_memo, const ChainParams* combine,
+void launch_mask_pass(const Geo& g, const FootprintParams& p, const Layers& L, const FaceInfo& face, bool write_memo, const ChainParams* combine,
                       hipStream_t stream, const Region* region, Region* rf_out) {
   MaskArgs m;
   m.slope_disc = p.slope_disc;
@@ -1084,7 +1269,10 @@
   m.map = -1;
   m.blocked_count = L.fp_blocked_count;
   m.untrav_flags = L.untrav_flags;
-  m.face_flags = face_flags;
+  m.face_flags = face.flags;
+  m.tile_list = nullptr;
+  m.tile_ntx = face_flag_ntx(g.rows);
+  m.tile_nty = face_tile_nty(g.cols);
   m.flag_ntx = untrav_flag_ntx(g.rows);
   m.flag_nfy = untrav_flag_nfy(g.cols);
   static const int mask_whatif = lab_int("TE_MASK_WHATIF", 0);
@@ -1125,7 +1313,24 @@
       hipLaunchKernelGGL(k_fp_mask<32>, grid, dim3(MX, MBY), 0, st, g, m, L.elev, L.slope, L.step, L.rough, L.untrav, L.slope_fp, L.step_fp, L.rough_fp, L.trav);
   };
   const int t_lo = rm.j0 / my, t_hi = (rm.j1 - 1) / my + 1;
-  {
+  if (mask_whatif == 0 && small_env < 0 && tile_env == 0 && footprint_mask_lean(g, p, face, region != nullptr)) {
+    TraceRange tr(combine ? "footprint: isTraversableForFilters mask (lean) + weighted combine" : "footprint: isTraversableForFilters mask (lean)");
+    const int n_tiles = (int)face_tile_total(g.rows, g.cols, g.batch > 0 ? g.batch : 1);
+    const int resident = device_cus() * 8;
+    const dim3 fgrid((unsigned)(n_tiles < resident ? n_tiles : resident));
+    auto aligned = [](const void* q, size_t n) { return ((uintptr_t)q & (n - 1)) == 0; };
+    const bool vec = g.rows % 4 == 0 && g.rows >= 4 && aligned(L.slope, 16) && aligned(L.step, 16) && aligned(L.rough, 16) && aligned(L.trav, 16) &&
+                     aligned(L.slope_fp, 16) && aligned(L.step_fp, 16) && aligned(L.rough_fp, 16) && aligned(L.untrav, 4);
+    if (vec)
+      hipLaunchKernelGGL(k_fp_mask_flat<true>, fgrid, dim3(kFlatThreads), 0, stream, g, m, n_tiles, L.slope, L.step, L.rough, L.untrav, L.slope_fp, L.step_fp, L.rough_fp, L.trav);
+    else
+      hipLaunchKernelGGL(k_fp_mask_flat<false>, fgrid, dim3(kFlatThreads), 0, stream, g, m, n_tiles, L.slope, L.step, L.rough, L.untrav, L.slope_fp, L.step_fp, L.rough_fp, L.trav);
+    if (face.n_tiles > 0) {
+      m.blocked_count = nullptr;
+      m.tile_list = face.tiles;
+      hipLaunchKernelGGL(k_fp_mask<32>, dim3(face.n_tiles), dim3(MX, MBY), 0, stream, g, m, L.elev, L.slope, L.step, L.rough, L.untrav, L.slope_fp, L.step_fp, L.rough_fp, L.trav);
+    }
+  } else {
     TraceRange tr(combine ? "footprint: isTraversableForFilters mask + weighted combine" : "footprint: isTraversableForFilters mask");
     launch_mask(t_lo, t_hi, stream);
   }
@@ -1134,18 +1339,26 @@
 
 }
 
-hipError_t launch_footprint_mask(const Geo& g, const FootprintParams& p, const Layers& L, const uint8_t* face_flags, const ChainParams* combine,
+int footprint_edge_failures(const Geo& g) { return submap_edge_failures(g); }
+
+bool footprint_mask_lean(const Geo& g, const FootprintParams& p, const FaceInfo& face, bool region) {
+  const bool q5 = p.step_disc.Q == 5 && p.step_disc.n_ties == 0;
+  if (!mask_route_lean(face.flags != nullptr, face.tiles != nullptr, region, q5, face.lean, g.rows, g.cols, g.batch)) return false;
+  return face.lean >= 2 || 4 * (size_t)face.n_tiles <= face_tile_total(g.rows, g.cols, g.batch > 0 ? g.batch : 1);
+}
+
+hipError_t launch_footprint_mask(const Geo& g, const FootprintParams& p, const Layers& L, const FaceInfo& face, const ChainParams* combine,
                                  hipStream_t stream) {
   Region rf;
-  launch_mask_pass(g, p, L, face_flags, false, combine, stream, nullptr, &rf);
+  launch_mask_pass(g, p, L, face, false, combine, stream, nullptr, &rf);
   return hipGetLastError();
 }
 
-hipError_t launch_footprint(const Geo& g, const FootprintParams& p, const Layers& L, const uint8_t* face_flags, const unsigned* ptab,
+hipError_t launch_footprint(const Geo& g, const FootprintParams& p, const Layers& L, const FaceInfo& face, const unsigned* ptab,
                             const int* clip_table, bool write_memo, const ChainParams* combine, double trav_cap, hipStream_t stream,
                             const Region* region) {
   Region rf;
-  launch_mask_pass(g, p, L, face_flags, write_memo, combine, stream, region, &rf);
+  launch_mask_pass(g, p, L, face, write_memo, combine, stream, region, &rf);
   TraceRange tr_sum("footprint: disc sums (+ blocked discs)");
   const Region* rfp = region ? &rf : nullptr;
   const Disc& d = p.fp_disc;
diff --git a/traversability_estimation_amd/csrc/te_internal.h b/traversability_estimation_amd/csrc/te_internal.h
--- a/traversability_estimation_amd/csrc/te_internal.h
+++ b/traversability_estimation_amd/csrc/te_internal.h
@@ -253,7 +253,15 @@
                          hipStream_t stream);
 hipError_t launch_chain(const Geo& g, const ChainParams& p, const Layers& L, const Region& r, unsigned flags,
                         hipStream_t stream);
-hipError_t launch_footprint(const Geo& g, const FootprintParams& p, const Layers& L, const uint8_t* face_flags, const unsigned* ptab,
+struct FaceInfo {
+  const uint8_t* flags = nullptr;
+  const unsigned* tiles = nullptr;
+  unsigned n_tiles = 0;
+  int lean = 0;
+};
+int footprint_edge_failures(const Geo& g);
+bool footprint_mask_lean(const Geo& g, const FootprintParams& p, const FaceInfo& face, bool region);
+hipError_t launch_footprint(const Geo& g, const FootprintParams& p, const Layers& L, const FaceInfo& face, const unsigned* ptab,
                             const int* clip_table, bool write_memo, const ChainParams* combine, double trav_cap, hipStream_t stream,
                             const Region* region = nullptr);
 hipError_t launch_footprint_any(const Geo& g, const FootprintParams& p, const Layers& L, const Region* rf, hipStream_t s);
@@ -284,7 +292,7 @@
 hipError_t launch_path_discs(const Geo& g, const PathDiscScratch& s, const PathDiscClass* classes, const float* trav, const uint8_t* untrav,
                              double fp_default, const float* robot_slope, int n_paths, const int* pose_offset, const double* pose_xy,
                              const int* path_class, unsigned char* is_safe, double* traversability, int* status, hipStream_t stream);
-hipError_t launch_footprint_mask(const Geo& g, const FootprintParams& p, const Layers& L, const uint8_t* face_flags, const ChainParams* combine,
+hipError_t launch_footprint_mask(const Geo& g, const FootprintParams& p, const Layers& L, const FaceInfo& face, const ChainParams* combine,
                                  hipStream_t stream);
 
 namespace any {
diff --git a/traversability_estimation_amd/csrc/te_paths_api.hip b/traversability_estimation_amd/csrc/te_paths_api.hip
--- a/traversability_estimation_amd/csrc/te_paths_api.hip
+++ b/traversability_estimation_amd/csrc/te_paths_api.hip
@@ -133,7 +133,7 @@
   if (e == hipSuccess) e = hipMemsetAsync(s.keys, 0xFF, p_keys.bytes(), c->stream);
   if (e == hipSuccess) e = hipMemsetAsync(s.counters, 0, p_cnt.bytes(), c->stream);
   if (e == hipSuccess && !c->mask_done) {
-    e = launch_footprint_mask(g, c->fp, c->L, usable_face_flags(c), c->combine_deferred ? &c->cp : nullptr, c->stream);
+    e = launch_footprint_mask(g, c->fp, c->L, usable_face_info(c), c->combine_deferred ? &c->cp : nullptr, c->stream);
     if (e == hipSuccess) {
       c->combine_deferred = false;
       c->mask_done = true;
diff --git a/traversability_estimation_amd/csrc/te_shim.hip b/traversability_estimation_amd/csrc/te_shim.hip
--- a/traversability_estimation_amd/csrc/te_shim.hip
+++ b/traversability_estimation_amd/csrc/te_shim.hip
@@ -136,7 +136,8 @@
 static_assert(kCfX == te::kFaceGranI && kCfY % te::kFaceGranJ == 0 && kCfT <= 64 && kCfY / te::kFaceGranJ <= 64, "k_count_invalid: tile shape");
 }
 __global__ __launch_bounds__(64 * kCfWaves) void k_count_invalid(const float* __restrict__ v, int rows, int cols, double crit_step,
-                                                                 uint8_t* __restrict__ flags, unsigned long long* __restrict__ out) {
+                                                                 uint8_t* __restrict__ flags, unsigned long long* __restrict__ out,
+                                                                 unsigned* __restrict__ tile_list, int edge_fail) {
   const int lane = threadIdx.x & 63, wave = threadIdx.x >> 6;
   const int ti = (int)blockIdx.x * kCfWaves + wave;
   if (ti >= te::face_flag_ntx(rows)) return;
@@ -199,12 +200,22 @@
     atomicAdd(out, (unsigned long long)cnt);
     if (runs) atomicAdd(out + 1, (unsigned long long)runs);
   }
+  bool my_flag = false;
   if (flags != nullptr && lane < kCfY / te::kFaceGranJ) {
     const int fj = j0 / te::kFaceGranJ + lane;
     if (fj < te::face_flag_nfy(cols)) {
       const unsigned long long span = (1ull << (te::kFaceGranJ + 2 * te::kFaceDilate)) - 1ull;
       const bool any = ((step_any >> (kCfH - te::kFaceDilate + te::kFaceGranJ * lane)) & span) != 0ull;
       flags[((size_t)map * (size_t)te::face_flag_nfy(cols) + (size_t)fj) * (size_t)te::face_flag_ntx(rows) + (size_t)ti] = any ? 1 : 0;
+      my_flag = any;
+    }
+  }
+  if (flags != nullptr && tile_list != nullptr) {
+    static_assert(kCfY == te::kFaceTileRows, "k_count_invalid: a wavefront per face tile");
+    const bool flat = __ballot(my_flag) == 0ull && !(edge_fail != 0 && te::face_tile_near_failing_border(rows, cols, edge_fail, i0, j0, kCfX, kCfY));
+    if (!flat && lane == 0) {
+      const unsigned long long slot = atomicAdd(out + 2, 1ull);
+      tile_list[slot] = (unsigned)(((size_t)map * (size_t)te::face_tile_nty(cols) + (size_t)blockIdx.y) * (size_t)te::face_flag_ntx(rows) + (size_t)ti);
     }
   }
 }
@@ -266,21 +277,29 @@
 int count_invalid_elevation(te_ctx* c) {
   c->invalid_cells = -1;
   c->face_crit = __builtin_nan("");
-  HIP_TRY(c->cmem.count.once(2 * sizeof(unsigned long long)));
+  c->face_tiles_known = false;
+  HIP_TRY(c->cmem.count.once(3 * sizeof(unsigned long long)));
   unsigned long long* const d_count = c->cmem.count.as<unsigned long long>();
-  HIP_TRY(hipMemsetAsync(d_count, 0, 2 * sizeof(unsigned long long), c->stream));
+  HIP_TRY(hipMemsetAsync(d_count, 0, 3 * sizeof(unsigned long long), c->stream));
   const bool with_flags = c->face_flags != nullptr;
   const double crit = c->params.fp_critical_step;
+  unsigned* const tile_list = with_flags ? c->lmem.face_tiles.as<unsigned>() : nullptr;
+  const int edge_fail = footprint_edge_failures(c->geo);
   const dim3 grid((unsigned)((face_flag_ntx(c->geo.rows) + kCfWaves - 1) / kCfWaves), (unsigned)((c->geo.cols + kCfY - 1) / kCfY), (unsigned)c->geo.batch);
   if (grid.y > 65535u || grid.z > 65535u) return fail(TE_ERR_UNSUPPORTED, "elevation layer of %d columns x %d maps: too many for one pass", c->geo.cols, c->geo.batch);
-  hipLaunchKernelGGL(k_count_invalid, grid, dim3(64 * kCfWaves), 0, c->stream, c->L.elev, c->geo.rows, c->geo.cols, crit, c->face_flags, d_count);
+  hipLaunchKernelGGL(k_count_invalid, grid, dim3(64 * kCfWaves), 0, c->stream, c->L.elev, c->geo.rows, c->geo.cols, crit, c->face_flags, d_count, tile_list, edge_fail);
   HIP_TRY(hipGetLastError());
-  unsigned long long h[2] = {0, 0};
+  unsigned long long h[3] = {0, 0, 0};
   HIP_TRY(hipMemcpyAsync(h, d_count, sizeof(h), hipMemcpyDeviceToHost, c->stream));
   HIP_TRY(hipStreamSynchronize(c->stream));
   c->invalid_cells = (long long)h[0];
   c->invalid_runs = (long long)h[1];
   if (with_flags) c->face_crit = crit;
+  if (tile_list != nullptr && h[2] <= face_tile_total(c->geo.rows, c->geo.cols, c->geo.batch)) {
+    c->face_tiles_known = true;
+    c->face_tile_count = (unsigned)h[2];
+    c->face_tiles_edge_fail = edge_fail;
+  }
   return TE_OK;
 }
 
@@ -288,6 +307,17 @@
   return (c->opt_face_flags && c->face_flags && !c->elev_ptr_out && c->face_crit == c->fp.crit_step && c->face_crit == c->params.fp_critical_step)
              ? c->face_flags
              : nullptr;
+}
+
+FaceInfo usable_face_info(const te_ctx* c) {
+  FaceInfo f;
+  f.flags = usable_face_flags(c);
+  f.lean = c->opt_mask_lean;
+  if (f.flags && c->face_tiles_known && c->lmem.face_tiles.p && c->face_tiles_edge_fail == footprint_edge_failures(c->geo)) {
+    f.tiles = c->lmem.face_tiles.as<unsigned>();
+    f.n_tiles = c->face_tile_count;
+  }
+  return f;
 }
 
 HoleCounts hole_counts(const te_ctx* c) { return HoleCounts{(long long)c->layer_elems, c->invalid_cells, c->invalid_runs}; }
@@ -564,6 +594,7 @@
   c->poly_rot = nullptr;
   clear_fp_any_ptrs(c);
   c->face_crit = __builtin_nan("");
+  c->face_tiles_known = false;
   c->elev_ptr_out = false;
   guard_cache_generation().fetch_add(1, std::memory_order_acq_rel);
   c->layers_written = 0;
@@ -660,7 +691,7 @@
   const ChainParams& q = c->cp;
   const bool bounded = !c->trav_external && (fresh || !c->trav_ptr_out) && q.w_scale >= 0.0f && q.w_slope >= 0.0f && q.w_step >= 0.0f && q.w_rough >= 0.0f;
   const double trav_cap = bounded ? (double)q.w_scale * ((double)q.w_slope + (double)q.w_step + (double)q.w_rough) : -1.0;
-  HIP_TRY(launch_footprint(c->geo, c->fp, c->L, usable_face_flags(c), c->cmem.spiral.as<unsigned>(), c->cmem.fp_clip_table.as<int>(), (flags & TE_RUN_FOOTPRINT_MEMO) != 0,
+  HIP_TRY(launch_footprint(c->geo, c->fp, c->L, usable_face_info(c), c->cmem.spiral.as<unsigned>(), c->cmem.fp_clip_table.as<int>(), (flags & TE_RUN_FOOTPRINT_MEMO) != 0,
                            c->combine_deferred ? &c->cp : nullptr, trav_cap, c->stream));
   c->combine_deferred = false;
   c->footprint_done = true;
@@ -686,8 +717,11 @@
     int slot = -1;
     ensure_tie_scratch(c);
     const unsigned key = flags | (((flags & TE_RUN_FOOTPRINT) && usable_face_flags(c)) ? 0x08000000u : 0u) | (sparse_holes(c) && ensure_hole_queue(c) ? 0x80000000u : 0u) | (c->invalid_cells == 0 ? 0x40000000u : 0u) | (skip_clean_march(c) ? 0x20000000u : 0u) | (short_strips(c) ? 0x10000000u : 0u);
+    const FaceInfo face = usable_face_info(c);
+    const bool lean = (flags & TE_RUN_FOOTPRINT) && c->fp_tables_ready && footprint_mask_lean(c->geo, c->fp, face, false);
+    const unsigned key_tiles = lean ? face.n_tiles + 1u : 0u;
     for (int k = 0; k < te_ctx::kGraphs; ++k)
-      if (c->graph_exec[k] && c->graph_flags[k] == key) slot = k;
+      if (c->graph_exec[k] && c->graph_flags[k] == key && c->graph_tiles[k] == key_tiles) slot = k;
     if (slot < 0) {
       slot = c->graph_next;
       c->graph_next = (c->graph_next + 1) % te_ctx::kGraphs;
@@ -710,6 +744,7 @@
         slot = -1;
       } else {
         c->graph_flags[slot] = key;
+        c->graph_tiles[slot] = key_tiles;
       }
     }
     if (slot >= 0) {
@@ -966,6 +1001,11 @@
       if (value < 0 || value > 1) return fail(TE_ERR_INVALID_ARG, "te_set_option: TE_OPT_FACE_FLAGS takes 0 (never passed to the mask kernel) or 1 (passed when known)");
       c->opt_face_flags = value;
       break;
+    case TE_OPT_MASK_LEAN:
+      if (value < 0 || value > 2)
+        return fail(TE_ERR_INVALID_ARG, "te_set_option: TE_OPT_MASK_LEAN takes 0 (one mask kernel over every tile), 1 (the lean route on maps of 64 x 32 tiles) or 2 (on every map)");
+      c->opt_mask_lean = value;
+      break;
     case TE_OPT_NORMALS_RANK_RULE:
       c->opt_rank_rule = value != 0;
       c->chain_done = false;
@@ -989,6 +1029,27 @@
   HIP_TRY(hipSetDevice(c->device));
   HIP_TRY(hipMemcpyAsync(out, f, n, hipMemcpyDeviceToHost, c->stream));
   HIP_TRY(hipStreamSynchronize(c->stream));
+  return TE_OK;
+}
+
+int te_download_mask_state(te_ctx* c, unsigned char* mask, size_t mask_bytes, unsigned char* tile_flags, size_t flag_bytes, unsigned* face_tiles,
+                           size_t tile_capacity, long long* n_face_tiles, int* lean_route) {
+  if (!c) return fail(TE_ERR_INVALID_ARG, "te_download_mask_state: NULL ctx");
+  CtxLock lk(c);
+  if (!c->have_geo) return fail(TE_ERR_NOT_READY, "te_download_mask_state: geometry not set");
+  const size_t nm = (size_t)c->geo.rows * c->geo.cols * c->geo.batch, nf = untrav_flag_bytes(c->geo.rows, c->geo.cols, c->geo.batch);
+  if ((mask && mask_bytes != nm) || (tile_flags && flag_bytes != nf))
+    return fail(TE_ERR_INVALID_ARG, "te_download_mask_state: the mask is %zu bytes, its tile flags are %zu", nm, nf);
+  if ((mask || tile_flags) && !c->mask_done) return fail(TE_ERR_NOT_READY, "te_download_mask_state: no footprint pass has built the mask");
+  const FaceInfo f = c->have_elev ? usable_face_info(c) : FaceInfo();
+  if (face_tiles && f.tiles && tile_capacity < f.n_tiles) return fail(TE_ERR_INVALID_ARG, "te_download_mask_state: %u face tiles, room for %zu", f.n_tiles, tile_capacity);
+  HIP_TRY(hipSetDevice(c->device));
+  if (mask) HIP_TRY(hipMemcpyAsync(mask, c->L.untrav, nm, hipMemcpyDeviceToHost, c->stream));
+  if (tile_flags) HIP_TRY(hipMemcpyAsync(tile_flags, c->L.untrav_flags, nf, hipMemcpyDeviceToHost, c->stream));
+  if (face_tiles && f.tiles && f.n_tiles) HIP_TRY(hipMemcpyAsync(face_tiles, f.tiles, (size_t)f.n_tiles * sizeof(unsigned), hipMemcpyDeviceToHost, c->stream));
+  HIP_TRY(hipStreamSynchronize(c->stream));
+  if (n_face_tiles) *n_face_tiles = f.tiles ? (long long)f.n_tiles : -1;
+  if (lean_route) *lean_route = (c->fp_tables_ready && footprint_mask_lean(c->geo, c->fp, f, false)) ? 1 : 0;
   return TE_OK;
 }
 
@@ -1031,6 +1092,9 @@
     c->L.fp_scratch = have_list ? (unsigned*)(slab + sp.sum_scratch.off) : nullptr;
     c->face_flags = (uint8_t*)(slab + sp.face_flags.off);
     c->face_crit = __builtin_nan("");
+    c->face_tiles_known = false;
+    const size_t n_face_tiles = face_tile_total(rows, cols, batch);
+    if (n_face_tiles < ((size_t)1 << 31)) (void)c->lmem.face_tiles.once(n_face_tiles * sizeof(unsigned));
     c->layer_elems = elems;
     HIP_TRY(hipMemsetAsync(slab, 0xFF, sp.list.off, c->stream));
     HIP_TRY(hipMemsetAsync(slab + sp.back_guard.off, 0xFF, sp.back_guard.bytes, c->stream));
@@ -1121,7 +1185,7 @@
   const ChainParams& q = c->cp;
   const bool bounded = !c->trav_external && !c->trav_ptr_out && q.w_scale >= 0.0f && q.w_slope >= 0.0f && q.w_step >= 0.0f && q.w_rough >= 0.0f;
   const double trav_cap = bounded ? (double)q.w_scale * ((double)q.w_slope + (double)q.w_step + (double)q.w_rough) : -1.0;
-  HIP_TRY(launch_footprint(c->geo, c->fp, c->L, usable_face_flags(c), c->cmem.spiral.as<unsigned>(), c->cmem.fp_clip_table.as<int>(), (flags & TE_RUN_FOOTPRINT_MEMO) != 0, nullptr, trav_cap,
+  HIP_TRY(launch_footprint(c->geo, c->fp, c->L, usable_face_info(c), c->cmem.spiral.as<unsigned>(), c->cmem.fp_clip_table.as<int>(), (flags & TE_RUN_FOOTPRINT_MEMO) != 0, nullptr, trav_cap,
                            c->stream, &changed));
   c->footprint_done = true;
   c->mask_done = mask_was_done;
```

After: 50.59 billion cells/s, median of 6. About the same (+0.9%).
